# treangenlab/komb

Measured on AMD Instinct MI355X. Metric: peeled edges/sec (k-truss), higher is better.
Workload: dtype int32

## Files before the change

### komb_amd/csrc/common.h

```cpp
#pragma once

#include <hip/hip_runtime.h>

#include <chrono>
#include <cstddef>
#include <cstdint>
#include <cstdio>
#include <cstdlib>
#include <cstring>
#include <map>
#include <string>
#include <vector>

#include "komb_accel.h"

#include <roctracer/roctx.h>

namespace komb {

struct Range {
    explicit Range(const char *name) { (void)roctxRangePushA(name); }
    ~Range() { (void)roctxRangePop(); }
    void next(const char *name) { (void)roctxRangePop(); (void)roctxRangePushA(name); }
    Range(const Range &) = delete;
    Range &operator=(const Range &) = delete;
};

constexpr int kBlock = 256;
constexpr int kWave = 64;
constexpr int32_t kAlive = 0x7FFFFFFF;
constexpr int32_t kAliveMin = 0x40000000;

__device__ __forceinline__ uint32_t wave_sum(uint32_t v)
{
    for (int o = kWave / 2; o > 0; o >>= 1) v += (uint32_t)__shfl_xor((int32_t)v, o);
    return v;
}
__device__ __forceinline__ uint32_t wave_max(uint32_t v)
{
    for (int o = kWave / 2; o > 0; o >>= 1) { const uint32_t other = (uint32_t)__shfl_xor((int32_t)v, o); v = other > v ? other : v; }
    return v;
}

struct PeelCtrl {
    int32_t  mode;
    int32_t  level;
    int32_t  round;
    int32_t  done;
    uint32_t cur_light;
    uint32_t cur_heavy;
    int32_t  cur_sel;
    uint32_t remaining;
    int32_t  n_levels;
    int32_t  n_rounds;
    int32_t  n_scans;
    int32_t  max_level;
    uint32_t live_count;
    int32_t  live_sel;
    int32_t  live_mode;
    int32_t  seq;
    uint32_t tail_l[2];
    uint32_t tail_h[2];
    int32_t  next_min;
    uint32_t live_tail;
    int32_t  last_retire;
    uint32_t tail_limit;
    uint32_t pad1[7];
    int32_t  max_retire_gap;
};
static_assert(offsetof(PeelCtrl, seq) == 60 && offsetof(PeelCtrl, tail_l) == 64, "PeelCtrl: the entry state is one 64-byte line");
static_assert(sizeof(PeelCtrl) == 128, "PeelCtrl layout");

struct LocalCtrl {
    int32_t  done;
    int32_t  iters;
    uint32_t spare[3];
    uint32_t bad;
    int32_t  max_val;
    uint32_t levels;
    uint32_t evals;
    uint32_t n_light, n_heavy;
    uint32_t n_giant;
    uint32_t n_chunk;
    uint32_t pad0;
    unsigned long long key_sum;
};
static_assert(sizeof(LocalCtrl) == 64, "LocalCtrl layout");

enum FinishMode : int { FIN_LOCAL = 0, FIN_LDS = 1, FIN_NONE = 2 };

struct Timer {
    hipEvent_t a = nullptr, b = nullptr;
    bool init() { return hipEventCreate(&a) == hipSuccess && hipEventCreate(&b) == hipSuccess; }
    void start(hipStream_t s) { (void)hipEventRecord(a, s); }
    double stop(hipStream_t s)
    {
        (void)hipEventRecord(b, s);
        (void)hipEventSynchronize(b);
        float ms = 0.f;
        (void)hipEventElapsedTime(&ms, a, b);
        return (double)ms;
    }
    void destroy() { if (a) (void)hipEventDestroy(a); if (b) (void)hipEventDestroy(b); a = b = nullptr; }
};

struct EventSet {
    std::vector<hipEvent_t> v;
    EventSet() = default;
    EventSet(const EventSet &) = delete;
    EventSet &operator=(const EventSet &) = delete;
    hipError_t make(hipEvent_t *out, unsigned flags = 0)
    {
        hipEvent_t e = nullptr;
        const hipError_t rc = flags ? hipEventCreateWithFlags(&e, flags) : hipEventCreate(&e);
        if (rc == hipSuccess) { v.push_back(e); *out = e; }
        return rc;
    }
    ~EventSet() { for (hipEvent_t e : v) if (e) (void)hipEventDestroy(e); }
};

}

struct AllocHook {
    bool armed = false;
    int64_t requests = 0, fail_at = 0, trim_at = 0;
    int32_t fired = 0;
    enum Act { PASS, FAIL, TRIM };
    Act step()
    {
        ++requests;
        if (fail_at && requests == fail_at) { fail_at = 0; fired = 1; return FAIL; }
        if (trim_at && requests == trim_at) { trim_at = 0; return TRIM; }
        return PASS;
    }
};

struct Poison {
    bool on = false;
    uint32_t word = 0;
    hipStream_t stream = nullptr;
    AllocHook *hook = nullptr;
    hipError_t fill(void *p, size_t bytes) const
    {
        if (!on || !p || !bytes) return hipSuccess;
        const size_t words = bytes / 4, rest = bytes % 4;
        hipError_t e = hipSuccess;
        if (words) e = hipMemsetD32Async((hipDeviceptr_t)p, (int)word, words, stream);
        if (e == hipSuccess && rest) e = hipMemsetAsync((char *)p + 4 * words, (int)(word & 0xFFu), rest, stream);
        return e == hipSuccess ? hipStreamSynchronize(stream) : e;
    }
    hipError_t malloc(void **out, size_t bytes) const
    {
        if (hook && hook->armed && hook->step() == AllocHook::FAIL) return hipErrorOutOfMemory;
        void *q = nullptr;
        hipError_t e = hipMalloc(&q, bytes);
        if (e != hipSuccess) return e;
        e = fill(q, bytes);
        if (e != hipSuccess) { (void)hipFree(q); return e; }
        *out = q;
        return hipSuccess;
    }
};

struct DevPool {
    struct Block { void *p; size_t bytes; bool used; };
    std::vector<Block> blocks;
    size_t n_malloc = 0, n_trim = 0;
    double ms_malloc = 0.0;
    Poison poison;
    AllocHook hook;
    DevPool() { poison.hook = &hook; }
    DevPool(const DevPool &) = delete;
    DevPool &operator=(const DevPool &) = delete;
    hipError_t get(void **out, size_t bytes)
    {
        if (hook.armed) {
            const AllocHook::Act a = hook.step();
            if (a == AllocHook::FAIL) return hipErrorOutOfMemory;
            if (a == AllocHook::TRIM) { ++n_trim; trim(); }
        }
        if (bytes == 0) bytes = 16;
        int best = -1;
        for (int i = 0; i < (int)blocks.size(); ++i)
            if (!blocks[i].used && blocks[i].bytes >= bytes && blocks[i].bytes <= bytes + bytes / 4 + 4096 &&
                (best < 0 || blocks[i].bytes < blocks[best].bytes)) best = i;
        if (best >= 0) {
            if (poison.on) { const hipError_t e = poison.fill(blocks[best].p, blocks[best].bytes); if (e != hipSuccess) return e; }
            blocks[best].used = true; *out = blocks[best].p; return hipSuccess;
        }
        void *q = nullptr;
        ++n_malloc;
        const auto t0 = std::chrono::steady_clock::now();
        hipError_t e = hipMalloc(&q, bytes);
        ms_malloc += std::chrono::duration<double, std::milli>(std::chrono::steady_clock::now() - t0).count();
        if (e != hipSuccess) {
            ++n_trim;
            trim();
            e = hipMalloc(&q, bytes);
            if (e != hipSuccess) return e;
        }
        blocks.push_back({q, bytes, true});
        if (poison.on) { e = poison.fill(q, bytes); if (e != hipSuccess) { put(q); return e; } }
        *out = q;
        return hipSuccess;
// ... 512 lines not shown
```

### komb_amd/csrc/kcore.hip

```cpp
#include "peel_dev.h"
#include "core_tail.h"
#include "local_dev.h"
#include "shard_dev.h"

#include <cstdlib>

namespace komb {

namespace {

__global__ __launch_bounds__(kBlock) void k_core_init(const uint32_t *__restrict__ rowptr, int64_t nv,
                                                      int32_t *__restrict__ deg, int32_t *__restrict__ degw,
                                                      int32_t *__restrict__ core, uint32_t *__restrict__ init)
{
    uint32_t zeros = 0;
    int32_t lmin = 0x7FFFFFFF;
    for (int64_t v = (int64_t)blockIdx.x * kBlock + threadIdx.x; v < nv; v += (int64_t)gridDim.x * kBlock) {
        const int32_t d = (int32_t)(rowptr[v + 1] - rowptr[v]);
        deg[v] = d; degw[v] = d;
        if (d == 0) { core[v] = 0; ++zeros; }
        else { core[v] = alive_marker((uint32_t)d); lmin = min(lmin, d); }
    }
    block_add_min(zeros, lmin, &init[0], (int32_t *)&init[1]);
}
// ... 112 lines not shown
    const uint32_t *nbr;
    __device__ __forceinline__ void ids(uint32_t pos, uint32_t (&id)[1]) const { id[0] = nbr[pos]; }
};

__global__ void k_live_bits(const int32_t *__restrict__ gid, uint32_t n, unsigned long long *__restrict__ bits)
{
    for (uint32_t i = blockIdx.x * blockDim.x + threadIdx.x; i < n; i += gridDim.x * blockDim.x) {
        const uint32_t v = (uint32_t)gid[i];
        atomicOr(&bits[v >> 6], 1ull << (v & 63u));
    }
}

__global__ void k_collect_ctrl(PeelCtrl *c2, const PeelCtrl *from)
{
    if (threadIdx.x == 0) {
        PeelCtrl c{};
        c.mode = MODE_SCAN; c.round = 1; c.level = 0x3FFFFFFF; c.seq = 1;
        c.remaining = from->remaining;
        c.live_mode = from->live_mode; c.live_sel = from->live_sel; c.live_count = from->live_count;
        c.next_min = 0x7FFFFFFF;
        *c2 = c;
    }
}

__global__ void k_ctrl_pre(uint32_t *grp_done)
{
    for (int i = threadIdx.x; i < kInitOff; i += blockDim.x) grp_done[i] = 0u;
    if (threadIdx.x == 0) { grp_done[kInitOff] = 0u; grp_done[kInitOff + 1] = 0x7FFFFFFFu; grp_done[kInitOff + 2] = 0u; grp_done[kInitOff + 3] = 0u; }
}
__global__ void k_ctrl_init(PeelCtrl *ctrl, const uint32_t *grp_done, uint32_t units, uint32_t tail_limit)
{
    if (threadIdx.x == 0) {
        const uint32_t peeled = grp_done[kInitOff];
        const int32_t first = (int32_t)grp_done[kInitOff + 1];
        const uint32_t front = grp_done[kInitOff + 2];
        PeelCtrl c{};
        c.mode = MODE_SCAN; c.round = 1; c.seq = 1;
        c.last_retire = 1;
        c.remaining = units - peeled;
        c.done = (c.remaining == 0) ? 1 : 0;
        c.level = c.remaining ? first : 0;
        c.n_levels = peeled ? 1 : 0;
        c.next_min = 0x7FFFFFFF;
        c.tail_limit = tail_limit;
        if (front) {
            c.mode = MODE_PROCESS; c.cur_light = front; c.cur_heavy = 0; c.cur_sel = 0;
            c.remaining -= front;
            c.n_levels += 1; c.max_level = first;
        }
        *ctrl = c;
    }
}

}

void peel_ctrl_pre(hipStream_t s, uint32_t *d_grp_done) { k_ctrl_pre<<<1, 128, 0, s>>>(d_grp_done); }
void peel_collect_ctrl(hipStream_t s, PeelCtrl *d_collect, const PeelCtrl *d_from) { k_collect_ctrl<<<1, 64, 0, s>>>(d_collect, d_from); }

void peel_ctrl_init(hipStream_t s, PeelCtrl *d_ctrl, uint32_t *d_grp_done, uint32_t units, uint32_t tail_limit)
{
    k_ctrl_init<<<1, 64, 0, s>>>(d_ctrl, d_grp_done, units, tail_limit);
}

int peel_grid(int64_t units)
{
    int64_t g = (units + kPeelBlock - 1) / kPeelBlock;
    if (g < 1) g = 1;
    if (g > 256 * kPeelPerCu) g = 256 * kPeelPerCu;
    return (int)g;
}

int core_run(komb_ctx *ctx, int rank, int world, komb_allreduce_fn fn, void *user, bool sharded)
{
    if (ctx->nv < 0) KOMB_FAIL(ctx, KOMB_ERR_STATE, "komb_core_run: no graph loaded");
    const int64_t nv = ctx->nv;
    hipStream_t s = ctx->stream;
    ctx->core_done = false;
    if (!ctx->d_deg) {
        const size_t bytes = (size_t)(nv > 0 ? nv : 1) * sizeof(int32_t);
        KOMB_HIP(ctx, dev_malloc_pair(ctx, &ctx->d_deg, bytes, &ctx->d_core, bytes));
    }
    komb_stats &stt = ctx->stats;
    stt.core_levels = stt.core_subrounds = stt.core_launches = 0;
    stt.max_coreness = 0; stt.ms_core = 0.0;
    stt.core_local_units = 0; stt.core_local_sweeps = 0; stt.core_local_items = 0; stt.ms_core_local = 0.0;
    if (ctx_flag(ctx, "SHARD_ENGINE")) sharded = true;
    stt.shard_exchanges = 0; stt.ms_exchange = 0.0; stt.exchange_words = 0;
    stt.engine_flags = sharded ? KOMB_ENGINE_SHARD_PEEL : 0;
    if (nv == 0) { ctx->core_done = true; return KOMB_OK; }

    Range r_all("komb_core_run");
    DevBufs bufs(ctx);
    const size_t heavy_cap = (size_t)(2 * ctx->ne) / 32 + 64;
    int32_t *d_degw = nullptr; PeelCtrl *d_ctrl = nullptr; uint32_t *d_grp = nullptr;
    CoreTailBufs T{};
    PeelQueues Q{nullptr, {nullptr, nullptr}, {nullptr, nullptr}, {nullptr, nullptr}, 0};
    KOMB_HIP(ctx, bufs.alloc(&d_degw, (size_t)nv));
    for (int i = 0; i < 2; ++i) {
        KOMB_HIP(ctx, bufs.alloc(&Q.light[i], (size_t)nv));
        KOMB_HIP(ctx, bufs.alloc(&Q.heavy[i], heavy_cap));
        KOMB_HIP(ctx, bufs.alloc(&Q.live[i], (size_t)nv / 2 + 64));
    }
    KOMB_HIP(ctx, bufs.alloc(&Q.code, (size_t)nv));
    KOMB_HIP(ctx, bufs.alloc(&d_ctrl, 1));
    KOMB_HIP(ctx, bufs.alloc(&d_grp, (size_t)kInitOff + 4));
    const FinishMode fin = finish_mode(ctx, FIN_LOCAL);
    uint32_t tail_limit = 0;
    const size_t live_words = ((size_t)nv + 63) / 64;
    unsigned long long *d_livebits = nullptr;
    if (fin == FIN_LDS) {
        tail_limit = kCoreTailV;
        if (const char *tl = ctx_opt(ctx, "CORE_TAIL")) tail_limit = (uint32_t)strtoul(tl, nullptr, 10);
        if (tail_limit > kCoreTailV) tail_limit = kCoreTailV;
        if (tail_limit) {
            KOMB_HIP(ctx, bufs.alloc(&T.livebits, live_words));
            KOMB_HIP(ctx, bufs.alloc(&T.vnum, (size_t)nv));
            KOMB_HIP(ctx, bufs.alloc(&T.cnt, 4));
            KOMB_HIP(ctx, bufs.alloc(&T.vlist, (size_t)kCoreTailV));
            KOMB_HIP(ctx, bufs.alloc(&T.rows, (size_t)kCoreTailV * kCoreTailWords));
        }
    } else if (fin == FIN_LOCAL) {
        tail_limit = local_limit(ctx, (uint64_t)nv, 16);
        if (tail_limit) KOMB_HIP(ctx, bufs.alloc(&d_livebits, live_words));
    }

    int64_t g = (nv + kBlock - 1) / kBlock;
    const int grid_init = (int)(g > 1024 ? 1024 : g);
    const int grid = peel_grid(nv);
    CoreProblem P{(uint32_t)nv, ctx->d_o_rowptr, ctx->d_o_col, d_degw, ctx->d_core};
    ctx->timer.start(s);
    peel_ctrl_pre(s, d_grp);
    k_core_init<<<grid_init, kBlock, 0, s>>>(ctx->d_o_rowptr, nv, ctx->d_deg, d_degw, ctx->d_core, d_grp + kInitOff);
    peel_ctrl_init(s, d_ctrl, d_grp, (uint32_t)nv, tail_limit);
    auto run_tail = [&](const int32_t *list, uint32_t n_in) -> int {
        KOMB_HIP(ctx, hipMemsetAsync(T.livebits, 0, live_words * sizeof(unsigned long long), s));
        KOMB_HIP(ctx, hipMemsetAsync(T.cnt, 0, 4 * sizeof(uint32_t), s));
        KOMB_HIP(ctx, hipMemsetAsync(T.rows, 0, (size_t)kCoreTailV * kCoreTailWords * sizeof(unsigned long long), s));
        int64_t gm = ((int64_t)n_in + kBlock - 1) / kBlock;
        k_ctail_mark<<<(int)(gm < 1 ? 1 : (gm > 1024 ? 1024 : gm)), kBlock, 0, s>>>(list, n_in, ctx->d_core, T);
        k_ctail_rows<<<dim3(kCoreTailV, 8), kBlock, 0, s>>>(ctx->d_o_rowptr, ctx->d_o_col, T);
        k_core_tail<false><<<1, 1024, 0, s>>>(d_ctrl, T, d_degw, ctx->d_core, nullptr);
        KOMB_HIP(ctx, d2h(ctx, &ctx->h_ctrl[0], d_ctrl, sizeof(PeelCtrl)));
        return KOMB_OK;
    };
    auto run_local = [&]() -> int {
        const PeelCtrl hc = ctx->h_ctrl[0];
        Range r_local("core: local finish");
        EventSet evs;
        hipEvent_t ev[2] = {nullptr, nullptr};
        for (auto &e : ev) KOMB_HIP(ctx, evs.make(&e));
        (void)hipEventRecord(ev[0], s);
        KOMB_HIP(ctx, hipMemsetAsync(d_livebits, 0, live_words * sizeof(unsigned long long), s));
        LocalStats ls;
        const int rc = local_finish(ctx, bufs, hc, d_ctrl, (uint32_t)nv, ctx->d_core, d_degw, Q.live[hc.live_sel],
            (uint32_t)kWave * CoreLocal::kU, sizeof(uint32_t), local_item_limit(ctx, std::max<uint64_t>(kCoreLocalItems, (uint64_t)ctx->ne / 3)), 0u, false, 0, ctx->d_core,
            [&](const LocalGraph &lg, const int32_t *num, void *items, PeelCtrl *d_cctrl, int32_t launch) {
                CoreCollect C{(uint32_t)nv, ctx->d_o_rowptr, ctx->d_o_col, ctx->d_core, d_livebits, num, lg.off, lg.cur, (uint32_t *)items};
                k_peel_step<CoreCollect><<<grid, kPeelBlock, 0, s>>>(d_cctrl, d_grp, Q, C, launch);
            },
            [&](const LocalGraph &lg, void *items, uint64_t total, LocalCtrl *d_lctrl, uint32_t *d_cnt, int *launches) -> int {
                return local_fixpoint(ctx, d_lctrl, d_cnt, lg, CoreLocal{(const uint32_t *)items}, total, launches);
            },
            &ls,
            [&](const LocalGraph &lg) { k_live_bits<<<(int)((lg.n + 255) / 256 > 1024 ? 1024 : (lg.n + 255) / 256), 256, 0, s>>>(lg.gid, lg.n, d_livebits); });
        (void)hipEventRecord(ev[1], s);
        (void)hipEventSynchronize(ev[1]);
        float ms = 0.f;
        (void)hipEventElapsedTime(&ms, ev[0], ev[1]);
        KOMB_TRY(rc);
        if (ls.refused) { ctx->h_ctrl[0].done = 0; ctx->h_ctrl[0].tail_limit = ls.new_limit; return KOMB_OK; }
        stt.core_local_units = (int32_t)ls.units; stt.core_local_sweeps = ls.sweeps; stt.core_local_items = (int64_t)ls.items;
        stt.ms_core_local = (double)ms;
        PeelCtrl done = hc;
        done.done = 1; done.remaining = 0;
        done.n_levels += (int32_t)ls.levels;
        done.max_level = ls.max_val > done.max_level ? ls.max_val : done.max_level;
        ctx->h_ctrl[0] = done;
        return KOMB_OK;
    };
    int launches = 0, st = KOMB_OK;
    if (sharded) {
        uint32_t iw[2] = {0u, 0u};
        KOMB_HIP(ctx, d2h(ctx, iw, d_grp + kInitOff, sizeof(iw)));
        ShardCore SP{(uint32_t)nv, ctx->d_o_rowptr, ctx->d_o_col, d_degw, ctx->d_core, 0u, 0u};
        shard_bounds((uint64_t)nv, rank, world, &SP.lo, &SP.hi);
        ShardStats ss;
        st = shard_peel(ctx, bufs, SP, d_degw, (uint32_t)nv, iw[0], (int32_t)iw[1], rank, world, fn, user, Q, d_ctrl,
                        [&](int32_t launch) { k_peel_step<ShardCore><<<grid, kPeelBlock, 0, s>>>(d_ctrl, d_grp, Q, SP, launch); },
                        fin == FIN_LOCAL ? tail_limit : 0u, [&]() -> int { return run_local(); }, &ss);
        stt.shard_exchanges = (int32_t)ss.exchanges; stt.ms_exchange = ss.ms_exchange; stt.exchange_words = ss.words;
        launches = ss.launches;
        PeelCtrl fc{};
        fc.done = st == KOMB_OK ? 1 : 2; fc.n_levels = ss.levels; fc.n_rounds = ss.rounds; fc.n_scans = ss.scans; fc.max_level = ss.max_level;
        ctx->h_ctrl[0] = fc;
    } else if (tail_limit && (uint64_t)nv <= tail_limit) {
        st = d2h(ctx, &ctx->h_ctrl[0], d_ctrl, sizeof(PeelCtrl)) == hipSuccess ? KOMB_OK : KOMB_ERR_DEVICE;
        if (st == KOMB_OK && !ctx->h_ctrl[0].done) st = (fin == FIN_LOCAL) ? run_local() : run_tail(nullptr, (uint32_t)nv);
    } else {
        ctx->h_ctrl[0].done = 0;
    }
    for (int guard = 0; st == KOMB_OK && ctx->h_ctrl[0].done != 1 && ctx->h_ctrl[0].done != 2 && guard < 64; ++guard) {
        if (ctx->h_ctrl[0].done == 3) {
            const PeelCtrl &c = ctx->h_ctrl[0];
            if (fin == FIN_LOCAL) st = run_local();
            else st = c.live_mode ? run_tail(Q.live[c.live_sel], c.live_count) : run_tail(nullptr, (uint32_t)nv);
            continue;
        }
        int batch = 0;
        st = drive_peel(ctx, d_ctrl, nv, [&](int32_t launch) {
            k_peel_step<CoreProblem><<<grid, kPeelBlock, 0, s>>>(d_ctrl, d_grp, Q, P, launch);
        }, &batch);
        launches += batch;
    }
    stt.ms_core = ctx->timer.stop(s);
#ifdef KOMB_STEP_TIMERS
    {
        const PeelCtrl &c = ctx->h_ctrl[0];
        const double n = c.pad1[6] ? (double)c.pad1[6] : 1.0;
        fprintf(stderr, "komb core step timers (block 0, %u small multi-workgroup PROCESS steps), us per step: ctrl %.2f queue+slice %.2f items %.2f flush %.2f barrier %.2f ticket %.2f\n",
                c.pad1[6], c.pad1[0] / n / 100.0, c.pad1[1] / n / 100.0, c.pad1[2] / n / 100.0, c.pad1[3] / n / 100.0, c.pad1[4] / n / 100.0, c.pad1[5] / n / 100.0);
    }
#endif
    KOMB_TRY(st);
    if (ctx->h_ctrl[0].done != 1) KOMB_FAIL(ctx, KOMB_ERR_DEVICE, "k-core peel ended in an inconsistent state");
    if (stt.core_local_units) stt.engine_flags |= KOMB_ENGINE_LOCAL_FINISH;
    else if (fin == FIN_LDS && tail_limit) stt.engine_flags |= KOMB_ENGINE_LDS_TAIL;
    stt.core_levels = ctx->h_ctrl[0].n_levels;
    stt.core_subrounds = ctx->h_ctrl[0].n_rounds;
    stt.core_launches = launches;
    stt.max_coreness = ctx->h_ctrl[0].max_level;
    ctx->core_done = true;
    return KOMB_OK;
}

}
```

### komb_amd/csrc/ktruss.hip

```cpp
#include "peel_dev.h"
#include "truss_tail.h"
#include "local_dev.h"
#include "shard_dev.h"

#include <algorithm>
#include <cstdlib>
#include <cstring>

#include "truss_line.h"
#include "truss_tri.h"
#include "truss_wedge.h"
#include "truss_index.h"
#include "truss_gather.h"

namespace komb {

namespace {

struct TrussProblem {
    static constexpr bool kChain = false;
    static constexpr bool kSingleStep = false;
    uint32_t units;
    const uint2 *off2;
    const int2 *inc;
    int32_t *sup;
    int32_t *stamp;
    uint8_t *st8;
    static constexpr int32_t kRetireEvery = komb::kRetireEvery;
    int32_t retire_every;
#ifdef KOMB_DEBUG_SWITCHES
    int ablate;
#endif

    __device__ __forceinline__ void retire(const CtrlView &cv, uint32_t block, uint32_t nblocks) const
    {
        const uint32_t n16 = (units + 15u) / 16u;
        uint4 *v = reinterpret_cast<uint4 *>(st8);
        for (uint32_t i = block * (uint32_t)kPeelBlock + threadIdx.x; i < n16; i += nblocks * (uint32_t)kPeelBlock) {
            uint4 q = v[i];
            uint32_t *w = &q.x;
            bool changed = false;
#pragma unroll
            for (int k = 0; k < 4; ++k) {
                uint32_t out = w[k];
#pragma unroll
                for (int b = 0; b < 4; ++b) {
                    const uint32_t c = (w[k] >> (8 * b)) & 0xFFu;
                    if (c > ST_GONE && state_rel(c, cv.round) == REL_GONE) out = (out & ~(0xFFu << (8 * b))) | ((uint32_t)ST_GONE << (8 * b));
                }
                changed |= out != w[k];
                w[k] = out;
            }
            if (changed) v[i] = q;
        }
    }

    __device__ __forceinline__ const int32_t *scan_marker() const { return stamp; }
    __device__ __forceinline__ const uint8_t *scan_state() const { return st8; }
    __device__ __forceinline__ const int32_t *scan_key() const { return sup; }
    __device__ __forceinline__ void mark_scanned(uint32_t e, const CtrlView &cv) const { stamp[e] = cv.round; st8[e] = state_of_round(cv.round); }
    __device__ __forceinline__ void slice(uint32_t e, uint32_t &b, uint32_t &len) const
    {
        const uint2 o = off2[e];
        b = o.x;
        len = o.y;
    }
    struct Loaded { int32_t me, x, y; uint32_t cx, cy; };
    __device__ __forceinline__ Loaded item_load(int32_t me, uint32_t pos, const CtrlView &) const
    {
        Loaded ld;
#ifdef KOMB_DEBUG_SWITCHES
        if (ablate & 6) {
            int2 p = make_int2((int)(((uint32_t)me * 2654435761u) % units), (int)(((uint32_t)me * 40503u + pos) % units));
            if (!(ablate & 4)) { const unsigned long long pq = __builtin_nontemporal_load(reinterpret_cast<const unsigned long long *>(inc) + pos); p = make_int2((int)(uint32_t)pq, (int)(uint32_t)(pq >> 32)); }
            ld.me = me; ld.x = p.x; ld.y = p.y;
            ld.cx = (ablate & 2) ? 0u : st8[p.x]; ld.cy = (ablate & 2) ? 0u : st8[p.y];
            return ld;
        }
#endif
        const unsigned long long pq = __builtin_nontemporal_load(reinterpret_cast<const unsigned long long *>(inc) + pos);
        const int2 p = make_int2((int)(uint32_t)pq, (int)(uint32_t)(pq >> 32));
        ld.me = me; ld.x = p.x; ld.y = p.y;
        ld.cx = st8[p.x]; ld.cy = st8[p.y];
        return ld;
    }
    __device__ __forceinline__ void item_apply(const Loaded &ld, const CtrlView &cv, int32_t &t0, int32_t &t1, uint32_t &c0, uint32_t &c1) const
    {
        const int32_t r = cv.round, L = cv.level;
        const int rx = state_rel(ld.cx, r), ry = state_rel(ld.cy, r);
        if (rx == REL_GONE || ry == REL_GONE) return;
        const bool xin = (rx == REL_NOW), yin = (ry == REL_NOW);
        bool decx = !xin && (!yin || ld.me < ld.y);
        bool decy = !yin && (!xin || ld.me < ld.x);
#ifdef KOMB_DEBUG_SWITCHES
        if (ablate & 1) { decx = false; decy = false; }
#endif
        if (decx && atomicSub(&sup[ld.x], 1) == L + 1) {
            c0 = ld.cx == ST_ALIVE_HEAVY ? marker_chunks(stamp[ld.x]) : 0u;
            stamp[ld.x] = r + 1; st8[ld.x] = state_of_round(r + 1); t0 = ld.x;
        }
        if (decy && atomicSub(&sup[ld.y], 1) == L + 1) {
            c1 = ld.cy == ST_ALIVE_HEAVY ? marker_chunks(stamp[ld.y]) : 0u;
            stamp[ld.y] = r + 1; st8[ld.y] = state_of_round(r + 1); t1 = ld.y;
        }
    }
};

struct ShardTruss {
    static constexpr bool kChain = false;
    static constexpr bool kSingleStep = true;
    uint32_t units;
    const uint2 *off2;
    const int2 *inc;
    int32_t *sup;
    int32_t *stamp;
    uint32_t lo, hi;

    __device__ __forceinline__ const int32_t *scan_marker() const { return stamp; }
    __device__ __forceinline__ const int32_t *scan_key() const { return sup; }
    __device__ __forceinline__ void mark_scanned(uint32_t e, const CtrlView &cv) const { stamp[e] = cv.round; }
    __device__ __forceinline__ void slice(uint32_t e, uint32_t &b, uint32_t &len) const
    {
        const uint2 o = off2[e];
        b = o.x;
        len = o.y;
    }
    __device__ __forceinline__ bool mine(int32_t e) const { return (uint32_t)e - lo < hi - lo; }
    struct Loaded { int32_t me, x, y, sx, sy; };
    __device__ __forceinline__ Loaded item_load(int32_t me, uint32_t pos, const CtrlView &) const
    {
        Loaded ld;
        const int2 p = inc[pos];
        ld.me = me; ld.x = p.x; ld.y = p.y;
        ld.sx = stamp[p.x]; ld.sy = stamp[p.y];
        return ld;
    }
    __device__ __forceinline__ void item_apply(const Loaded &ld, const CtrlView &cv, int32_t &t0, int32_t &t1, uint32_t &, uint32_t &) const
    {
        const int32_t r = cv.round, L = cv.level;
        if (ld.sx < r || ld.sy < r) return;
        const bool xin = (ld.sx == r), yin = (ld.sy == r);
        const bool decx = !xin && (!yin || ld.me < ld.y) && mine(ld.x);
        const bool decy = !yin && (!xin || ld.me < ld.x) && mine(ld.y);
        if (decx && atomicSub(&sup[ld.x], 1) == L + 1) { stamp[ld.x] = r + 1; t0 = ld.x; }
        if (decy && atomicSub(&sup[ld.y], 1) == L + 1) { stamp[ld.y] = r + 1; t1 = ld.y; }
    }
};

struct TrussCollect {
    static constexpr bool kChain = false;
    static constexpr bool kSingleStep = false;
    uint32_t units;
    const uint2 *off2;
    const int2 *inc;
    const int32_t *stamp;
    const int32_t *num;
    const uint32_t *coff;
    uint32_t *cur;
    uint2 *cpair;

    __device__ __forceinline__ const int32_t *scan_marker() const { return stamp; }
    __device__ __forceinline__ const int32_t *scan_key() const { return nullptr; }
    __device__ __forceinline__ void mark_scanned(uint32_t, const CtrlView &) const {}
    __device__ __forceinline__ void slice(uint32_t e, uint32_t &b, uint32_t &len) const
    {
        const uint2 o = off2[e];
        b = o.x;
        len = o.y;
    }
    struct Loaded { int32_t me, x, y, sx, sy; };
    __device__ __forceinline__ Loaded item_load(int32_t me, uint32_t pos, const CtrlView &) const
    {
        Loaded ld;
        const int2 p = inc[pos];
        ld.me = me; ld.x = p.x; ld.y = p.y;
        ld.sx = stamp[p.x]; ld.sy = stamp[p.y];
        return ld;
    }
    __device__ __forceinline__ void item_apply(const Loaded &ld, const CtrlView &, int32_t &, int32_t &, uint32_t &, uint32_t &) const
    {
        if (!marker_alive(ld.sx) || !marker_alive(ld.sy)) return;
        const uint32_t id = (uint32_t)num[ld.me];
        const uint32_t b0 = coff[id], k = local_slot(id, cur);
        if (k < coff[id + 1] - b0) cpair[b0 + k] = make_uint2((uint32_t)num[ld.x], (uint32_t)num[ld.y]);
    }
};

constexpr uint64_t kTrussLocalItems = 32ull << 20;
constexpr uint32_t kTrussLocalDensity = 160;
struct TrussLocal {
    static constexpr int kU = 8;
#ifndef KOMB_TRUSS_GROUPS
#define KOMB_TRUSS_GROUPS 8
#endif
    static constexpr int kGroups = KOMB_TRUSS_GROUPS;
    static constexpr int kN = 2;
    const uint2 *cpair;
    __device__ __forceinline__ void ids(uint32_t pos, uint32_t (&id)[2]) const
    {
        const uint2 p = cpair[pos];
        id[0] = p.x; id[1] = p.y;
    }
};

}

void truss_free(komb_ctx *ctx)
{
    communities_drop(ctx);
    community_hierarchy_drop(ctx);
    biconnected_drop(ctx);
    structural_drop(ctx);
    nucleus_drop(ctx);
    max_clique_drop(ctx);
    clique_census_drop(ctx);
    maximal_cliques_drop(ctx);
    if (ctx->t_own_edges) { ctx->pool.put(ctx->d_t_eu); ctx->pool.put(ctx->d_t_ev); }
    ctx->pool.put(ctx->d_t_truss);
    ctx->pool.put(ctx->d_t_sup);
    ctx->pool.put(ctx->d_t_slice);
    ctx->d_t_eu = ctx->d_t_ev = ctx->d_t_truss = ctx->d_t_sup = nullptr;
    ctx->d_t_slice = nullptr;
    ctx->t_sup_ready = false;
    ctx->t_own_edges = false;
    ctx->t_ne = -1; ctx->truss_done = false;
}

int truss_edges_canonical(komb_ctx *ctx)
{
    if (ctx->t_own_edges || ctx->t_ne <= 0) return KOMB_OK;
    if (!ctx->d_ceu) {
        int32_t *eu = nullptr, *ev = nullptr;
        hipError_t e = ctx->pool.get((void **)&eu, (size_t)ctx->ne * sizeof(int32_t));
        if (e == hipSuccess) e = ctx->pool.get((void **)&ev, (size_t)ctx->ne * sizeof(int32_t));
        const int rc = e == hipSuccess ? edge_list(ctx, ctx->d_o_rowptr, ctx->d_o_col, ctx->nv, nullptr, eu, ev) : KOMB_ERR_NOMEM;
        if (rc != KOMB_OK) {
            ctx->pool.put(eu); ctx->pool.put(ev);
            if (e != hipSuccess) KOMB_FAIL(ctx, KOMB_ERR_NOMEM, "komb_truss_fetch: no memory for the canonical edge list (%s)", hipGetErrorString(e));
            return rc;
        }
        ctx->d_ceu = eu; ctx->d_cev = ev;
    }
    ctx->d_t_eu = ctx->d_ceu; ctx->d_t_ev = ctx->d_cev;
    return KOMB_OK;
}

int truss_support_canonical(komb_ctx *ctx)
{
    if (ctx->t_sup_ready) return KOMB_OK;
    if (!ctx->truss_done || !ctx->d_t_slice || !ctx->prep.valid || ctx->prep.ne != ctx->t_ne)
        KOMB_FAIL(ctx, KOMB_ERR_STATE, "komb_truss_fetch_support: no k-truss result to take the supports from");
    hipStream_t s = ctx->stream;
    const int64_t m = ctx->t_ne;
    if (!ctx->d_t_sup) KOMB_HIP(ctx, ctx->pool.get((void **)&ctx->d_t_sup, (size_t)m * sizeof(int32_t)));
#ifndef KOMB_TEST_SKIP_SLICE_ZERO
    if (ctx->t_k_lo) KOMB_HIP(ctx, hipMemsetAsync(ctx->d_t_sup, 0, (size_t)ctx->t_k_lo * sizeof(int32_t), s));
    if (ctx->t_k_hi < (uint32_t)m) KOMB_HIP(ctx, hipMemsetAsync(ctx->d_t_sup + ctx->t_k_hi, 0, ((size_t)m - ctx->t_k_hi) * sizeof(int32_t), s));
#endif
    k_scatter_len<<<grid_for(m), kBlock, 0, s>>>(ctx->d_t_slice, ctx->prep.e2k, m, ctx->t_k_lo, ctx->t_k_hi, ctx->d_t_sup);
    KOMB_HIP(ctx, hipStreamSynchronize(s));
    ctx->t_sup_ready = true;
    return KOMB_OK;
}

namespace {
int truss_run_body(komb_ctx *ctx, const uint8_t *vmask_host, int rank, int world, komb_allreduce_fn fn, void *user)
{
    if (world < 1 || rank < 0 || rank >= world || (world > 1 && !fn))
        KOMB_FAIL(ctx, KOMB_ERR_ARG, "komb_truss_run_sharded: bad rank %d / world %d / callback", rank, world);
    if (ctx->nv < 0) KOMB_FAIL(ctx, KOMB_ERR_STATE, "komb_truss_run: no graph loaded");
    truss_free(ctx);
    hipStream_t s = ctx->stream;
    komb_stats &st = ctx->stats;
    st.triangles = 0; st.truss_levels = st.truss_subrounds = st.truss_launches = 0;
    st.max_trussness = 0; st.ms_support = st.ms_peel = st.ms_orient = st.ms_tri_count = st.ms_tri_fill = st.ms_gather = st.ms_allreduce = st.ms_compact = 0.0;
    st.truss_scans = 0; st.ms_prepare = 0.0; st.truss_prepared = 0; st.ms_prep_vertex = st.ms_prep_edges = st.ms_prep_rows = 0.0;
    auto empty_result = [&]() -> int {
        void *q[4] = {nullptr, nullptr, nullptr, nullptr};
        hipError_t e = hipSuccess;
        for (int i = 0; i < 4 && e == hipSuccess; ++i) e = ctx->pool.get(&q[i], 4);
        if (e != hipSuccess) {
            for (void *p : q) ctx->pool.put(p);
            KOMB_HIP(ctx, e);
        }
        ctx->d_t_eu = (int32_t *)q[0]; ctx->d_t_ev = (int32_t *)q[1]; ctx->d_t_truss = (int32_t *)q[2]; ctx->d_t_sup = (int32_t *)q[3];
        ctx->t_own_edges = true; ctx->t_ne = 0; ctx->truss_done = true; ctx->t_sup_ready = true;
        return KOMB_OK;
    };
    if (ctx->nv == 0 || ctx->ne == 0) return empty_result();
    Range r_all("komb_truss_run");
    DevBufs bufs(ctx);

    Range phase("truss: preparation");
    InducedCsr sub;
    TrussPrep sub_prep;
    struct SubGuard { komb_ctx *c; InducedCsr *g; TrussPrep *p; ~SubGuard() { prep_free(c, p); induced_free(c, g); } } sub_guard{ctx, &sub, &sub_prep};
    TrussPrep *tp = &ctx->prep;
    if (vmask_host) {
        ctx->timer.start(s);
        KOMB_TRY(induce_csr(ctx, vmask_host, &sub));
        st.ms_orient = ctx->timer.stop(s);
        if (sub.ns == 0) return empty_result();
        KOMB_TRY(prep_build(ctx, sub.rowptr, sub.col, sub.nv, sub.ns, &sub_prep));
        st.ms_prepare = sub_prep.ms; st.truss_prepared = 1;
        st.ms_prep_vertex = sub_prep.ms_part[0]; st.ms_prep_edges = sub_prep.ms_part[1]; st.ms_prep_rows = sub_prep.ms_part[2];
        tp = &sub_prep;
    } else if (!ctx->prep.valid) {
        KOMB_TRY(prep_ensure(ctx));
        st.ms_prepare = ctx->prep.ms; st.truss_prepared = 1;
        st.ms_prep_vertex = ctx->prep.ms_part[0]; st.ms_prep_edges = ctx->prep.ms_part[1]; st.ms_prep_rows = ctx->prep.ms_part[2];
    }
    const int64_t nv = tp->nv;
    const int64_t m = tp->ne;
    const uint32_t *d_orow = tp->orow;
    const int32_t *d_ocol = tp->ocol;
    const uint4 *d_line = tp->vline;
    const uint2 *d_wtasks = (const uint2 *)tp->wtasks;
    const int64_t n_wtasks = tp->n_wtasks;
    const int gw = grid_for(n_wtasks, kTriWaves);
    phase.next("truss: triangles + incidence index");

    const int ge = grid_for(m);
    const int tri_tv = (int)std::max<int64_t>(1, std::min<int64_t>(kTriV, nv / (256 * KOMB_TRI_EU * kTriWaves * 4)));
    const int64_t ntasks = (nv + tri_tv - 1) / tri_tv;
    const int gt = grid_for(ntasks, kTriWaves);
    uint32_t *d_own = nullptr, *d_other = nullptr, *d_cnt = nullptr, *d_off = nullptr;
    uint2 *d_off2 = nullptr;
    KOMB_HIP(ctx, bufs.alloc(&d_own, 2 * ((size_t)m + 1)));
    d_other = d_own + ((size_t)m + 1);
    KOMB_HIP(ctx, bufs.alloc(&d_cnt, (size_t)m + 1));
    KOMB_HIP(ctx, bufs.alloc(&d_off2, (size_t)m + 4));
    unsigned long long *d_mom = nullptr;
    KOMB_HIP(ctx, bufs.alloc(&d_mom, 12));
    KOMB_HIP(ctx, hipMemsetAsync(d_mom, 0, 12 * sizeof(unsigned long long), s));
// ... 36 lines not shown
    st.ms_sort = 0.0; st.tri_records = 0; st.ms_compact = 0.0; st.ms_tri_count = 0.0; st.ms_tri_fill = 0.0; st.stream_retries = 0;
    st.index_layout = layout;
    auto zero_counts = [&]() -> hipError_t { return hipMemsetAsync(d_own, 0, 2 * ((size_t)m + 1) * sizeof(uint32_t), s); };
    if (!(world == 1 && layout == IDX_STREAM)) KOMB_HIP(ctx, zero_counts());
    bool have_counts = false;
    if (world > 1) {
        const int64_t task_lo = n_wtasks * rank / world, task_hi = n_wtasks * (rank + 1) / world;
        ctx->timer.start(s);
        k_wedges<TRI_COUNT><<<gw, kBlock, 0, s>>>(d_orow, d_ocol, d_line, d_wtasks, task_lo, task_hi, d_own, d_other, nullptr, nullptr, 0ull, nullptr, no_stream, nullptr, ablate);
        st.ms_tri_count = ctx->timer.stop(s);
        k_sum_counts<<<ge, kBlock, 0, s>>>(d_own, d_other, nullptr, m + 1, d_cnt, d_mom + 5);
        ctx->timer.start(s);
        KOMB_HIP(ctx, hipStreamSynchronize(s));
        if (fn(user, d_cnt, (int64_t)m + 1) != 0)
            KOMB_FAIL(ctx, KOMB_ERR_DEVICE, "komb_truss_run_sharded: all-reduce callback failed");
        st.ms_allreduce = ctx->timer.stop(s);
        KOMB_HIP(ctx, hipMemsetAsync(d_mom + 5, 0, sizeof(unsigned long long), s));
        k_total_u32<<<ge, kBlock, 0, s>>>(d_cnt, m + 1, d_mom + 5);
        have_counts = true;
        if (layout != IDX_TWO_PASS) {
            KOMB_HIP(ctx, bufs.alloc(&d_cnt_ref, (size_t)m + 1));
            KOMB_HIP(ctx, hipMemcpyAsync(d_cnt_ref, d_cnt, ((size_t)m + 1) * sizeof(uint32_t), hipMemcpyDeviceToDevice, s));
            KOMB_HIP(ctx, zero_counts());
        }
    }

    if (layout == IDX_STREAM) {
        const unsigned long long bound = (unsigned long long)tp->own_bound;
        const int gws = std::min(gw, 256 * KOMB_WEDGE_EU);
        const unsigned long long slack = (unsigned long long)gws * kTriWaves * kRecChunk + kRecChunk;
        const unsigned long long own_slack = (unsigned long long)gws * kTriWaves * kOwnChunk + kOwnChunk;
        const unsigned long long t_bound = bound / 2;
        const unsigned long long own_full = bound + bound / 8 + own_slack, rec_full = 3 * t_bound + (3 * t_bound) / 14 + slack;
        unsigned long long own_cap = std::min(own_full, 4ull * (unsigned long long)m + own_slack);
        unsigned long long rec_cap = std::min(rec_full, 2ull * (unsigned long long)m + slack);
        bool fixed_caps = false;
        if (const char *oc = ctx_opt(ctx, "OWN_DENSE_CAP")) { own_cap = strtoull(oc, nullptr, 10) + 1; rec_cap = rec_full; fixed_caps = true; }
        if (ctx_flag(ctx, "NO_OWN_DENSE")) { own_cap = 1; rec_cap = rec_full; fixed_caps = true; }
        if (const char *rc = ctx_opt(ctx, "REC_CAP")) { rec_cap = strtoull(rc, nullptr, 10) + 1; fixed_caps = true; }
        if (ctx_flag(ctx, "FULL_CAPS")) { own_cap = own_full; rec_cap = rec_full; }
        if (!fixed_caps && ctx->cap_hint.nv == nv && ctx->cap_hint.m == m) {
            own_cap = std::min(own_full, std::max(own_cap, ctx->cap_hint.own_cap));
            rec_cap = std::min(rec_full, std::max(rec_cap, ctx->cap_hint.rec_cap));
        }
        const uint32_t sentinel = geom.sentinel_base();
        uint32_t *d_key = nullptr; int2 *d_val = nullptr;
        unsigned long long n_claimed = 0;
        bool ok = false;
        st.ms_tri_fill = 0.0;
        for (int attempt = 0; attempt < 2; ++attempt) {
            size_t free_b = 0, total_b = 0;
            (void)hipMemGetInfo(&free_b, &total_b);
            const unsigned long long budget = (unsigned long long)((free_b + ctx->pool.unused_bytes()) * 0.7);
            if (own_cap * sizeof(int2) > budget / 2) own_cap = budget / 2 / sizeof(int2);
            if (rec_cap * 12ull > budget / 2) rec_cap = budget / 2 / 12ull;
            if (rec_cap > 0xFFFFFFF0ull) rec_cap = 0xFFFFFFF0ull;
            ok = bufs.alloc(&d_key, (size_t)rec_cap) == hipSuccess && bufs.alloc(&d_val, (size_t)rec_cap) == hipSuccess &&
                 bufs.alloc(&d_owndense, (size_t)own_cap) == hipSuccess &&
                 (d_ownoff || bufs.alloc(&d_ownoff, (size_t)m + 1) == hipSuccess) && (d_dcur || bufs.alloc(&d_dcur, 4) == hipSuccess);
            uint2 *d_scratch = nullptr;
            if (ok && !ctx_flag(ctx, "NO_REC_SCRATCH") && bufs.alloc(&d_scratch, (size_t)gws * kTriWaves * kScratchRec) != hipSuccess) { (void)hipGetLastError(); d_scratch = nullptr; }
            if (!ok) { (void)hipGetLastError(); break; }
            KOMB_HIP(ctx, hipMemsetAsync(d_dcur, 0, 4 * sizeof(unsigned long long), s));
            const TriStream ts{d_key, d_val, d_dcur + 2, rec_cap, sentinel, geom.nb - 1u, kChunkBits};
            ctx->timer.start(s);
            k_wedges<TRI_SINGLE><<<gws, kBlock, 0, s>>>(d_orow, d_ocol, d_line, d_wtasks, 0, n_wtasks, d_own, d_other, d_owndense, d_dcur, own_cap, d_ownoff, ts, d_scratch, ablate);
            st.ms_tri_fill += ctx->timer.stop(s);
            unsigned long long dc[4] = {0, 0, 0, 0};
            KOMB_HIP(ctx, d2h(ctx, dc, d_dcur, sizeof(dc)));
            n_claimed = dc[2];
            bufs.release(d_scratch);
            if (ctx_flag(ctx, "TRI_DEBUG"))
                fprintf(stderr, "komb triangles: stream build (attempt %d): %llu record positions claimed of %llu, dense own-role region %llu entries claimed of %llu, %llu task ranges overflowed their record buffer\n",
                        attempt, dc[2], rec_cap, dc[0], own_cap, dc[1]);
            if (n_claimed <= rec_cap) {
                if (!fixed_caps) { ctx->cap_hint.nv = nv; ctx->cap_hint.m = m; ctx->cap_hint.own_cap = own_cap; ctx->cap_hint.rec_cap = rec_cap; }
                break;
            }
            ok = false;
            if (attempt == 1 || fixed_caps) break;
            bufs.release(d_key); bufs.release(d_val); bufs.release(d_owndense);
            d_key = nullptr; d_val = nullptr; d_owndense = nullptr;
            own_cap = std::min(own_full, std::max(own_cap, dc[0] + own_slack));
            rec_cap = std::min(rec_full, n_claimed + slack);
            st.stream_retries += 1;
        }
        uint32_t *d_skey = nullptr;
        if (ok) {
            uint32_t *d_key2 = nullptr; unsigned long long *d_val2 = nullptr;
            ok = bufs.alloc(&d_key2, (size_t)n_claimed + 1) == hipSuccess && bufs.alloc(&d_val2, (size_t)n_claimed + 1) == hipSuccess;
            if (ok) {
                ctx->timer.start(s);
                unsigned long long *sv = nullptr;
                if (geom.nb_bits > 0) KOMB_TRY(prim_sort_pairs_u32_u64(ctx, d_key, d_key2, (unsigned long long *)d_val, d_val2, (int64_t)n_claimed, kChunkBits, kChunkBits + geom.nb_bits, &d_skey, &sv));
                else { d_skey = d_key; sv = (unsigned long long *)d_val; }
                st.ms_sort = ctx->timer.stop(s);
                d_recval = (int2 *)sv;
                if (d_skey == d_key) { bufs.release(d_key2); bufs.release(d_val2); } else { bufs.release(d_key); bufs.release(d_val); }
                d_reckey = d_skey;
                KOMB_HIP(ctx, bufs.alloc(&d_toff, (size_t)n_bins + 2));
                KOMB_HIP(ctx, bufs.alloc(&d_bintot, (size_t)n_bins + 2));
                KOMB_HIP(ctx, bufs.alloc(&d_grp, (size_t)kInitOff + 4));
                if (!whole_peel_finish && !shard_peel_on && !ctx_flag(ctx, "NO_FIRST_QUEUE")) KOMB_HIP(ctx, bufs.alloc(&d_light0, (size_t)m));
                ctx->timer.start(s);
                peel_ctrl_pre(s, d_grp);
                KOMB_HIP(ctx, hipMemsetAsync(d_mom + 5, 0, sizeof(unsigned long long), s));
                k_bin_offsets<<<grid_for(n_bins + 1), kBlock, 0, s>>>(d_skey, (int64_t)n_claimed, geom, d_toff);
                k_bin_count<<<grid_for(n_bins, 1, 256 * 8), kBlock, 0, s>>>(d_skey, d_toff, geom, d_own, m, d_cnt, d_bintot, d_mom + 5, (int32_t *)(d_grp + kInitOff + 1));
                st.ms_compact = ctx->timer.stop(s);
                st.tri_records = (int64_t)n_claimed;
            } else (void)hipGetLastError();
        }
        if (!ok) {
            bufs.release(d_key); bufs.release(d_val); bufs.release(d_owndense); bufs.release(d_ownoff); bufs.release(d_dcur);
            bufs.release(d_grp); bufs.release(d_light0); d_grp = nullptr; d_light0 = nullptr;
            d_owndense = nullptr; d_ownoff = nullptr; d_dcur = nullptr;
            KOMB_HIP(ctx, zero_counts());
            KOMB_HIP(ctx, hipMemsetAsync(d_mom + 5, 0, sizeof(unsigned long long), s));
            st.ms_tri_fill = 0.0;
            layout = IDX_TWO_PASS;
        }
    }
    if (layout != IDX_TWO_PASS && d_cnt_ref) {
        k_count_mismatch<<<ge, kBlock, 0, s>>>(d_cnt, d_cnt_ref, m + 1, d_mom + 8);
    }
    if (layout == IDX_TWO_PASS) {
        if (d_cnt_ref) {
            KOMB_HIP(ctx, hipMemcpyAsync(d_cnt, d_cnt_ref, ((size_t)m + 1) * sizeof(uint32_t), hipMemcpyDeviceToDevice, s));
            KOMB_HIP(ctx, hipMemsetAsync(d_mom + 5, 0, sizeof(unsigned long long), s));
            k_total_u32<<<ge, kBlock, 0, s>>>(d_cnt, m + 1, d_mom + 5);
        } else if (!have_counts) {
            ctx->timer.start(s);
            k_triangles<TRI_COUNT><<<gt, kBlock, 0, s>>>(d_orow, d_ocol, nv, 0, ntasks, d_own, d_other, nullptr, nullptr, ablate, tri_tv);
            st.ms_tri_count = ctx->timer.stop(s);
            k_sum_counts<<<ge, kBlock, 0, s>>>(d_own, d_other, nullptr, m + 1, d_cnt, d_mom + 5);
        }
    }
    st.index_layout = layout;
    {
        unsigned long long mom[9];
        KOMB_HIP(ctx, d2h(ctx, mom, d_mom, sizeof(mom)));
        st.triangles = (int64_t)(mom[5] / 3);
        bufs.release(d_mom);
        if (mom[8] != 0)
            KOMB_FAIL(ctx, KOMB_ERR_DEVICE, "komb_truss_run_sharded: %llu edges whose all-reduced support differs from the support of the index build", mom[8]);
        if (mom[5] > 0xFFFFFFF0ull)
            KOMB_FAIL(ctx, KOMB_ERR_LIMIT, "graph has %llu triangles; the incidence index is limited to 2^32-16 entries (3 per triangle)",
                      mom[5] / 3);
    }
    bufs.release(d_cnt_ref);
    uint32_t total = 0;
    const uint32_t sum_supports = (uint32_t)st.triangles * 3u;
    int2 *d_inc = nullptr;
    int32_t *d_sup = nullptr, *d_stamp = nullptr, *d_truss = nullptr;
    uint8_t *d_st8 = nullptr;
    bool peel_inited = false;
    if (layout == IDX_STREAM) {
        KOMB_TRY(prim_exclusive_sum_u32(ctx, d_bintot, d_bintot, n_bins + 1));
        total = sum_supports;
        KOMB_HIP(ctx, bufs.alloc(&d_inc, (size_t)total));
        KOMB_HIP(ctx, bufs.alloc(&d_sup, (size_t)m));
        KOMB_HIP(ctx, bufs.alloc(&d_stamp, (size_t)m));
        KOMB_HIP(ctx, bufs.alloc(&d_st8, (size_t)m + 16));
        KOMB_HIP(ctx, bufs.alloc(&d_truss, (size_t)m));
        ctx->timer.start(s);
        k_bin_finish<<<grid_for(n_bins, 1, 256 * kFinPerCu), kFinBlock, 0, s>>>(d_reckey, d_recval, d_toff, geom, d_own, d_cnt, d_bintot, d_owndense, d_ownoff, d_inc, m,
                                                                      d_off2, d_sup, d_stamp, d_st8, d_grp + kInitOff, d_light0);
        st.ms_compact += ctx->timer.stop(s);
        peel_inited = true;
        bufs.release(d_toff); bufs.release(d_bintot); bufs.release((void *)d_recval); bufs.release(d_reckey);
        bufs.release(d_owndense); bufs.release(d_ownoff); bufs.release(d_dcur);
    } else {
        KOMB_HIP(ctx, bufs.alloc(&d_off, (size_t)m + 1));
        KOMB_TRY(prim_exclusive_sum_u32(ctx, d_cnt, d_off, m + 1));
        KOMB_HIP(ctx, d2h(ctx, &total, d_off + m, sizeof(uint32_t)));
        KOMB_HIP(ctx, bufs.alloc(&d_inc, (size_t)total));
        ctx->timer.start(s);
        KOMB_HIP(ctx, zero_counts());
        k_back_cursors<<<ge, kBlock, 0, s>>>(d_off, m, d_other);
        k_triangles<TRI_SINGLE><<<gt, kBlock, 0, s>>>(d_orow, d_ocol, nv, 0, ntasks, d_own, d_other, d_off, d_inc, ablate, tri_tv);
        st.ms_tri_fill = ctx->timer.stop(s);
    }
    st.ms_support = st.ms_tri_count + st.ms_tri_fill + st.ms_sort + st.ms_compact;
    bufs.release(d_cnt); bufs.release(d_own);

    phase.next("truss: peel");
    PeelCtrl *d_ctrl = nullptr;
    PeelQueues Q{nullptr, {nullptr, nullptr}, {nullptr, nullptr}, {nullptr, nullptr}, 0};
    const size_t heavy_cap = (size_t)total / 32 + 64;
    if (!peel_inited) {
        KOMB_HIP(ctx, bufs.alloc(&d_sup, (size_t)m));
        KOMB_HIP(ctx, bufs.alloc(&d_stamp, (size_t)m));
        KOMB_HIP(ctx, bufs.alloc(&d_st8, (size_t)m + 16));
        KOMB_HIP(ctx, bufs.alloc(&d_truss, (size_t)m));
        KOMB_HIP(ctx, bufs.alloc(&d_grp, (size_t)kInitOff + 4));
    }
    for (int i = 0; i < 2; ++i) {
        if (i == 0 && d_light0) Q.light[0] = d_light0;
        else KOMB_HIP(ctx, bufs.alloc(&Q.light[i], (size_t)m));
        KOMB_HIP(ctx, bufs.alloc(&Q.heavy[i], heavy_cap));
        KOMB_HIP(ctx, bufs.alloc(&Q.live[i], (size_t)m / 2 + 64));
    }
    KOMB_HIP(ctx, bufs.alloc(&d_ctrl, 1));
    KOMB_HIP(ctx, bufs.alloc(&Q.code, (size_t)m));
    KOMB_HIP(ctx, bufs.alloc(&Q.rlevel, (size_t)m + 2));
    KOMB_HIP(ctx, hipMemsetAsync(Q.rlevel, 0, 2 * sizeof(int32_t), s));
    int32_t retire_every = kRetireEvery;
    if (const char *e = ctx_opt(ctx, "RETIRE_EVERY")) retire_every = std::max(1, std::min((int)kRetireEvery, atoi(e)));
#ifdef KOMB_DEBUG_SWITCHES
    TrussProblem P{(uint32_t)m, d_off2, d_inc, d_sup, d_stamp, d_st8, retire_every, getenv("KOMB_PEEL_ABLATE") ? atoi(getenv("KOMB_PEEL_ABLATE")) : 0};
#else
    TrussProblem P{(uint32_t)m, d_off2, d_inc, d_sup, d_stamp, d_st8, retire_every};
#endif
    TailBufs T{};
    if (fin == FIN_LDS && tail_limit) {
        KOMB_HIP(ctx, bufs.alloc(&T.vmap, (size_t)nv));
        KOMB_HIP(ctx, bufs.alloc(&T.cnt, 64));
        KOMB_HIP(ctx, bufs.alloc(&T.vlist, (size_t)kTailMaxV));
        KOMB_HIP(ctx, bufs.alloc(&T.rows, (size_t)kTailMaxV * kTailRowWords));
        KOMB_HIP(ctx, bufs.alloc(&T.pair, (size_t)tail_limit));
        KOMB_HIP(ctx, bufs.alloc(&T.sup, (size_t)tail_limit));
        KOMB_HIP(ctx, bufs.alloc(&T.gid, (size_t)tail_limit));
        KOMB_HIP(ctx, bufs.alloc(&T.gid_by_rank, (size_t)tail_limit));
        KOMB_HIP(ctx, bufs.alloc(&T.pair_by_rank, (size_t)tail_limit));
        KOMB_HIP(ctx, bufs.alloc(&T.truss_by_rank, (size_t)tail_limit));
        KOMB_HIP(ctx, bufs.alloc(&T.spill[0], (size_t)tail_limit));
        KOMB_HIP(ctx, bufs.alloc(&T.spill[1], (size_t)tail_limit));
        T.max_edges = tail_limit;
    }
    auto run_tail = [&](const int32_t *list, uint32_t n_in) -> int {
        KOMB_HIP(ctx, hipMemsetAsync(T.vmap, 0, (size_t)nv * sizeof(int32_t), s));
        KOMB_HIP(ctx, hipMemsetAsync(T.cnt, 0, 64 * sizeof(uint32_t), s));
        KOMB_HIP(ctx, hipMemsetAsync(T.rows, 0, (size_t)kTailMaxV * kTailRowWords * sizeof(unsigned long long), s));
        const int g = grid_for(n_in, kBlock, 256);
        const bool dbg = ctx_flag(ctx, "TAIL_DEBUG");
        hipEvent_t ev[3] = {nullptr, nullptr, nullptr};
        for (auto &e : ev) (void)hipEventCreate(&e);
        (void)hipEventRecord(ev[0], s);
        k_tail_mark<<<g, kBlock, 0, s>>>(list, n_in, d_sup, d_stamp, d_osrc, d_ocol, T);
        k_tail_number<<<1, kTailMaxV, 0, s>>>(T);
        k_tail_rows<<<g, kBlock, 0, s>>>(list, n_in, d_sup, d_stamp, d_osrc, d_ocol, T);
        (void)hipEventRecord(ev[1], s);
        k_truss_tail<<<1, 1024, 0, s>>>(d_ctrl, T, d_truss);
        (void)hipEventRecord(ev[2], s);
        KOMB_HIP(ctx, d2h(ctx, &ctx->h_ctrl[0], d_ctrl, sizeof(PeelCtrl)));
        ++st.truss_tail_runs;
        float m0 = 0, m1 = 0, m2 = 0;
        (void)hipEventElapsedTime(&m0, ctx->timer.a, ev[0]); (void)hipEventElapsedTime(&m1, ev[0], ev[1]); (void)hipEventElapsedTime(&m2, ev[1], ev[2]);
        for (auto &e : ev) (void)hipEventDestroy(e);
        st.ms_tail += (double)m1 + (double)m2;
        if (dbg) {
            uint32_t h[16];
            KOMB_HIP(ctx, d2h(ctx, h, T.cnt, sizeof(h)));
            fprintf(stderr, "komb tail: %u vertices, %u edges, %s; general engine before it %.1f us, setup %.1f us, tail kernel %.1f us\n",
                    h[0], h[1], ctx->h_ctrl[0].done == 1 ? "done" : "refused", m0 * 1000.f, m1 * 1000.f, m2 * 1000.f);
#ifdef KOMB_TAIL_TIMERS
            fprintf(stderr, "komb tail: us in kernel: load %.1f ranks %.1f supports %.1f scan %.1f mark %.1f triangles %.1f retire %.1f results %.1f\n",
                    h[14] / 100.0, h[15] / 100.0, h[8] / 100.0, h[9] / 100.0, h[10] / 100.0, h[11] / 100.0, h[12] / 100.0, h[13] / 100.0);
#endif
        }
        return KOMB_OK;
    };
    const int gp = peel_grid(m);
    auto run_local = [&]() -> int {
        const PeelCtrl hc = ctx->h_ctrl[0];
        EventSet evs;
        hipEvent_t ev[2] = {nullptr, nullptr};
        for (auto &e : ev) KOMB_HIP(ctx, evs.make(&e));
        (void)hipEventRecord(ev[0], s);
        LocalStats ls;
        const int lrc = local_finish(ctx, bufs, hc, d_ctrl, (uint32_t)m, d_stamp, d_sup, Q.live[hc.live_sel],
            (uint32_t)kWave * TrussLocal::kU, sizeof(uint2), local_item_limit(ctx, kTrussLocalItems), local_density_limit(ctx, kTrussLocalDensity), true, 2, d_truss,
            [&](const LocalGraph &lg, const int32_t *num, void *items, PeelCtrl *d_cctrl, int32_t launch) {
                TrussCollect C{(uint32_t)m, d_off2, d_inc, d_stamp, num, lg.off, lg.cur, (uint2 *)items};
                PeelQueues Qc = Q;
                Qc.rlevel = nullptr;
                k_peel_step<TrussCollect><<<gp, kPeelBlock, 0, s>>>(d_cctrl, d_grp, Qc, C, launch);
            },
            [&](const LocalGraph &lg, void *items, uint64_t total_items, LocalCtrl *d_lctrl, uint32_t *d_cnt, int *nl) -> int {
                return local_fixpoint(ctx, d_lctrl, d_cnt, lg, TrussLocal{(const uint2 *)items}, total_items, nl);
            },
            &ls, [](const LocalGraph &) {});
        (void)hipEventRecord(ev[1], s);
        (void)hipEventSynchronize(ev[1]);
        float ms = 0.f;
        (void)hipEventElapsedTime(&ms, ev[0], ev[1]);
        KOMB_TRY(lrc);
        if (ls.refused) { ctx->h_ctrl[0].done = 0; ctx->h_ctrl[0].tail_limit = ls.new_limit; return KOMB_OK; }
        st.truss_local_units = (int32_t)ls.units; st.truss_local_sweeps = ls.sweeps; st.truss_local_items = (int64_t)ls.items;
        st.ms_truss_local = (double)ms;
        PeelCtrl fin_c = hc;
        fin_c.done = 1; fin_c.remaining = 0;
        fin_c.n_levels += (int32_t)ls.levels;
        fin_c.max_level = ls.max_val > fin_c.max_level ? ls.max_val : fin_c.max_level;
        ctx->h_ctrl[0] = fin_c;
        return KOMB_OK;
    };
    ctx->timer.start(s);
    if (!peel_inited) {
        peel_ctrl_pre(s, d_grp);
        k_peel_init<<<grid_for(m, kBlock, 1024), kBlock, 0, s>>>(m, d_off, d_off2, d_sup, d_stamp, d_st8, d_grp + kInitOff);
    }
    peel_ctrl_init(s, d_ctrl, d_grp, (uint32_t)m, tail_limit);
    int launches = 0, rc = KOMB_OK;
    st.truss_tail_runs = 0; st.ms_tail = 0.0;
    st.truss_local_units = 0; st.truss_local_sweeps = 0; st.truss_local_items = 0; st.ms_truss_local = 0.0;
    st.shard_exchanges = 0; st.ms_exchange = 0.0; st.exchange_words = 0;
    if (shard_peel_on) {
        uint32_t iw[2] = {0u, 0u};
        KOMB_HIP(ctx, d2h(ctx, iw, d_grp + kInitOff, sizeof(iw)));
        ShardTruss SP{(uint32_t)m, d_off2, d_inc, d_sup, d_stamp, 0u, 0u};
        shard_bounds((uint64_t)m, rank, world, &SP.lo, &SP.hi);
        ShardStats ss;
        rc = shard_peel(ctx, bufs, SP, d_sup, (uint32_t)m, iw[0], (int32_t)iw[1], rank, world, fn, user, Q, d_ctrl,
                        [&](int32_t launch) { k_peel_step<ShardTruss><<<gp, kPeelBlock, 0, s>>>(d_ctrl, d_grp, Q, SP, launch); },
                        fin == FIN_LOCAL ? tail_limit : 0u, [&]() -> int { return run_local(); }, &ss);
        st.shard_exchanges = (int32_t)ss.exchanges; st.ms_exchange = ss.ms_exchange; st.exchange_words = ss.words;
        launches = ss.launches;
        PeelCtrl fc{};
        fc.done = rc == KOMB_OK ? 1 : 2; fc.n_levels = ss.levels; fc.n_rounds = ss.rounds; fc.n_scans = ss.scans; fc.max_level = ss.max_level;
        ctx->h_ctrl[0] = fc;
    } else if (whole_peel_finish) {
        rc = d2h(ctx, &ctx->h_ctrl[0], d_ctrl, sizeof(PeelCtrl)) == hipSuccess ? KOMB_OK : KOMB_ERR_DEVICE;
        if (rc == KOMB_OK && !ctx->h_ctrl[0].done) rc = (fin == FIN_LOCAL) ? run_local() : run_tail(nullptr, (uint32_t)m);
    } else {
        ctx->h_ctrl[0].done = 0;
    }
    for (int guard = 0; rc == KOMB_OK && ctx->h_ctrl[0].done != 1 && ctx->h_ctrl[0].done != 2 && guard < 64; ++guard) {
        if (ctx->h_ctrl[0].done == 3) {
            const PeelCtrl &c = ctx->h_ctrl[0];
            if (fin == FIN_LOCAL) rc = run_local();
            else rc = c.live_mode ? run_tail(Q.live[c.live_sel], c.live_count) : run_tail(nullptr, (uint32_t)m);
            continue;
        }
        int batch = 0;
        rc = drive_peel(ctx, d_ctrl, m, [&](int32_t launch) {
            k_peel_step<TrussProblem><<<gp, kPeelBlock, 0, s>>>(d_ctrl, d_grp, Q, P, launch);
        }, &batch);
        launches += batch;
    }
    st.ms_peel = ctx->timer.stop(s);
    KOMB_TRY(rc);
#ifdef KOMB_STEP_TIMERS
    {
        const PeelCtrl &c = ctx->h_ctrl[0];
        const double n = c.pad1[6] ? (double)c.pad1[6] : 1.0;
        fprintf(stderr, "komb step timers (block 0, %u small multi-workgroup PROCESS steps), us per step: ctrl %.2f queue+slice %.2f items %.2f flush %.2f barrier %.2f ticket %.2f\n",
                c.pad1[6], c.pad1[0] / n / 100.0, c.pad1[1] / n / 100.0, c.pad1[2] / n / 100.0, c.pad1[3] / n / 100.0, c.pad1[4] / n / 100.0, c.pad1[5] / n / 100.0);
    }
#endif
    if (ctx->h_ctrl[0].done != 1) KOMB_FAIL(ctx, KOMB_ERR_DEVICE, "k-truss peel ended in an inconsistent state");
    if (ctx->h_ctrl[0].max_retire_gap > retire_every)
        KOMB_FAIL(ctx, KOMB_ERR_DEVICE, "k-truss peel: %d sub-rounds passed without a RETIRE step (period %d): edge state codes may have wrapped",
                  ctx->h_ctrl[0].max_retire_gap, retire_every);
    st.engine_flags = (layout == IDX_TWO_PASS ? KOMB_ENGINE_TWO_PASS : 0) | (shard_peel_on ? KOMB_ENGINE_SHARD_PEEL : 0) |
                      (st.truss_local_units ? KOMB_ENGINE_LOCAL_FINISH : 0) | (st.truss_tail_runs ? KOMB_ENGINE_LDS_TAIL : 0);
    st.truss_levels = ctx->h_ctrl[0].n_levels;
    st.truss_subrounds = ctx->h_ctrl[0].n_rounds;
    st.truss_launches = launches;
    st.truss_scans = ctx->h_ctrl[0].n_scans;
    st.max_trussness = ctx->h_ctrl[0].max_level + 2;
    for (int i = 0; i < 2; ++i) { bufs.release(Q.light[i]); bufs.release(Q.heavy[i]); bufs.release(Q.live[i]); }
    bufs.release(Q.code);
    bufs.release(d_sup); bufs.release(d_inc);

    phase.next("truss: canonical gather");
    ctx->timer.start(s);
    KOMB_HIP(ctx, ctx->pool.get((void **)&ctx->d_t_truss, (size_t)m * sizeof(int32_t)));
    uint32_t k_lo = 0, k_hi = (uint32_t)m;
    if (!vmask_host) {
        ctx->d_t_eu = ctx->d_ceu; ctx->d_t_ev = ctx->d_cev;
        ctx->t_own_edges = false;
        if (ctx->slice_world > 1) {
            shard_bounds((uint64_t)m, ctx->slice_rank, ctx->slice_world, &k_lo, &k_hi);
#ifndef KOMB_TEST_SKIP_SLICE_ZERO
            if (k_lo) KOMB_HIP(ctx, hipMemsetAsync(ctx->d_t_truss, 0, (size_t)k_lo * sizeof(int32_t), s));
            if (k_hi < (uint32_t)m) KOMB_HIP(ctx, hipMemsetAsync(ctx->d_t_truss + k_hi, 0, ((size_t)m - k_hi) * sizeof(int32_t), s));
#endif
        }
    } else {
        ctx->t_own_edges = true;
        KOMB_HIP(ctx, ctx->pool.get((void **)&ctx->d_t_eu, (size_t)m * sizeof(int32_t)));
        KOMB_HIP(ctx, ctx->pool.get((void **)&ctx->d_t_ev, (size_t)m * sizeof(int32_t)));
        KOMB_TRY(edge_list(ctx, sub.rowptr, sub.col, sub.nv, sub.vold, ctx->d_t_eu, ctx->d_t_ev));
    }
    ctx->t_k_lo = k_lo; ctx->t_k_hi = k_hi;
    k_truss_results<<<grid_for(m), kBlock, 0, s>>>(d_stamp, Q.rlevel, d_truss, tp->e2k, m, k_lo, k_hi, ctx->d_t_truss);
    ctx->d_t_slice = d_off2;
    bufs.detach(d_off2);
    ctx->t_sup_ready = false;
    if (vmask_host) {
        KOMB_HIP(ctx, ctx->pool.get((void **)&ctx->d_t_sup, (size_t)m * sizeof(int32_t)));
        k_scatter_len<<<grid_for(m), kBlock, 0, s>>>(ctx->d_t_slice, tp->e2k, m, 0u, (uint32_t)m, ctx->d_t_sup);
        ctx->t_sup_ready = true;
    }
    st.ms_gather = ctx->timer.stop(s);
    if (ctx_flag(ctx, "POOL_DEBUG")) {
        size_t held = 0;
        for (const auto &b : ctx->pool.blocks) held += b.bytes;
        fprintf(stderr, "komb pool: %zu blocks, %.2f GB held, %zu hipMalloc calls so far (%.1f ms inside them), %zu trims\n", ctx->pool.blocks.size(), held / 1e9, ctx->pool.n_malloc, ctx->pool.ms_malloc, ctx->pool.n_trim);
    }
    if (vmask_host) KOMB_HIP(ctx, hipStreamSynchronize(s));
    ctx->t_ne = m;
    ctx->truss_done = true;
    return KOMB_OK;
}
}

int truss_run(komb_ctx *ctx, const uint8_t *vmask_host, int rank, int world, komb_allreduce_fn fn, void *user)
{
    const int rc = truss_run_body(ctx, vmask_host, rank, world, fn, user);
    if (rc != KOMB_OK && !ctx->truss_done) truss_free(ctx);
    return rc;
}

}
```

### komb_amd/csrc/local_dev.h

```cpp
#pragma once

#include "peel_dev.h"

namespace komb {

constexpr int kLocBlock = 512;
constexpr int kLocWaves = kLocBlock / kWave;
constexpr int kLocHB = 4096;
constexpr int kLocBins = kLocHB / kLocBlock;
constexpr int kCntWays = 8;
constexpr int kCntWords = (5 * kCntWays + 5) * 32;
constexpr int kCntTimerWords = 6 * 12 * 2;
constexpr int kHvU = 8;
constexpr uint32_t kKeyBins = 4096;
constexpr uint32_t kMedMax = 2048;
constexpr int kGiantWin = 8;
constexpr uint32_t kGiantChunk = 8192;
constexpr int kLocBatch = 6;


struct LocalGraph {
    uint32_t n, nh;
    uint32_t *off;
    int32_t *val;
    int32_t *mark[2];
    int32_t *gid;
    uint32_t *len;
    uint32_t *cur;
    uint4 *giant;
    uint32_t ng;
    uint4 *gchunk;
    uint32_t nchunk;
    unsigned long long *gacc;
    uint32_t *gwin;
    int4 *gnote;
    uint32_t *khist;
    uint32_t *list;
    uint32_t flags;
};
constexpr uint32_t kLocUseList = 1u, kLocDeferNotify = 2u;
constexpr uint32_t kLocDeferChunks = 256;

constexpr int kNumBlock = 1024;
static __global__ __launch_bounds__(kNumBlock) void k_local_number(const int32_t *__restrict__ list, uint32_t n_in, uint32_t n_live,
                                                         const int32_t *__restrict__ marker, const int32_t *__restrict__ key,
                                                         uint32_t light_max, int32_t *__restrict__ num, LocalGraph g, LocalCtrl *ctrl)
{
    __shared__ uint32_t sh_cnt[kNumBlock / kWave][2];
    __shared__ uint32_t sh_base[2];
    __shared__ uint32_t sh_kh[kKeyBins];
    __shared__ unsigned long long sh_ks;
    unsigned long long ks = 0ull;
    if (threadIdx.x == 0) sh_ks = 0ull;
    for (uint32_t i = threadIdx.x; i < kKeyBins; i += kNumBlock) sh_kh[i] = 0u;
    const int lane = lane_id(), w = (int)(threadIdx.x >> 6);
    for (uint32_t i0 = blockIdx.x * kNumBlock; i0 < n_in; i0 += gridDim.x * kNumBlock) {
        const uint32_t i = i0 + threadIdx.x;
        int32_t u = -1, k = 0;
        if (i < n_in) {
            u = list ? list[i] : (int32_t)i;
            if (!marker_alive(marker[u])) u = -1; else k = key[u];
        }
        const bool heavy = u >= 0 && (uint32_t)k > light_max, light = u >= 0 && !heavy;
        const uint64_t mh = __ballot(heavy), ml = __ballot(light);
        __syncthreads();
        if (lane == 0) { sh_cnt[w][0] = (uint32_t)__popcll(mh); sh_cnt[w][1] = (uint32_t)__popcll(ml); }
        __syncthreads();
        uint32_t bh = 0, bl = 0, th = 0, tl = 0;
#pragma unroll
        for (int x = 0; x < kNumBlock / kWave; ++x) {
            const uint32_t a = sh_cnt[x][0], b = sh_cnt[x][1];
            if (x < w) { bh += a; bl += b; }
            th += a; tl += b;
        }
        if (threadIdx.x == 0) {
            sh_base[0] = th ? atomicAdd(&ctrl->n_heavy, th) : 0u;
            sh_base[1] = tl ? atomicAdd(&ctrl->n_light, tl) : 0u;
        }
        __syncthreads();
        if (u < 0) continue;
        ks += (unsigned long long)(uint32_t)k;
        const uint32_t id = heavy ? sh_base[0] + bh + (uint32_t)__popcll(mh & lanemask_lt())
                                  : n_live - 1u - (sh_base[1] + bl + (uint32_t)__popcll(ml & lanemask_lt()));
        if (id >= n_live) { atomicAdd(&ctrl->bad, 1u); continue; }
        num[u] = (int32_t)id;
        g.gid[id] = u; g.len[id] = (uint32_t)k; g.val[id] = k; g.mark[1][id] = 1; g.mark[0][id] = 0; g.cur[id] = 0u;
        atomicAdd(&sh_kh[min((uint32_t)k, kKeyBins - 1u)], 1u);
        if ((uint32_t)k > kMedMax) {
            const uint32_t nch = ((uint32_t)k + kGiantChunk - 1u) / kGiantChunk;
            g.giant[atomicAdd(&ctrl->n_giant, 1u)] = make_uint4(id, atomicAdd(&ctrl->n_chunk, nch), nch, 0u);
        }
    }
    for (int o = 32; o > 0; o >>= 1) ks += __shfl_xor(ks, o);
    if (lane == 0 && ks) atomicAdd(&sh_ks, ks);
    __syncthreads();
    for (uint32_t i = threadIdx.x; i < kKeyBins; i += kNumBlock) if (sh_kh[i]) atomicAdd(&g.khist[i], sh_kh[i]);
    if (threadIdx.x == 0 && sh_ks) atomicAdd(&ctrl->key_sum, sh_ks);
}

static __global__ __launch_bounds__(kBlock) void k_local_chunks(LocalGraph g)
{
    for (uint32_t gi = blockIdx.x; gi < g.ng; gi += gridDim.x) {
        const uint4 u = g.giant[gi];
        for (uint32_t j = threadIdx.x; j < u.z; j += kBlock) g.gchunk[u.y + j] = make_uint4(u.x, gi, j, u.z);
        if (threadIdx.x == 0) { g.gacc[gi] = 0ull; g.gnote[gi] = make_int4(0, 0, 0, 0); }
        if (threadIdx.x < (uint32_t)kGiantWin) g.gwin[gi * kGiantWin + threadIdx.x] = 0u;
    }
}

static __global__ __launch_bounds__(kBlock) void k_local_clamp(LocalGraph g, int32_t K)
{
    for (uint32_t id = blockIdx.x * kBlock + threadIdx.x; id < g.n; id += gridDim.x * kBlock)
        if (g.val[id] > K) g.val[id] = K;
}

__device__ __forceinline__ uint32_t local_slot(uint32_t id, uint32_t *cur)
{
    const int lane = lane_id();
    uint64_t todo = __ballot(true);
    uint32_t pos = 0;
    while (todo) {
        const int leader = __ffsll((long long)todo) - 1;
        const uint32_t lid = (uint32_t)__shfl((int)id, leader);
        const uint64_t grp = __ballot(id == lid) & todo;
        uint32_t base = 0;
        if (lane == leader) base = atomicAdd(&cur[lid], (uint32_t)__popcll(grp));
        base = (uint32_t)__shfl((int)base, leader);
        if ((grp >> lane) & 1ull) pos = base + (uint32_t)__popcll(grp & lanemask_lt());
        todo &= ~grp;
    }
    return pos;
}

static __global__ __launch_bounds__(kBlock) void k_local_check(LocalGraph g, LocalCtrl *ctrl)
{
    uint32_t bad = 0;
    for (uint32_t id = blockIdx.x * kBlock + threadIdx.x; id < g.n; id += gridDim.x * kBlock)
        bad += (g.cur[id] != g.off[id + 1] - g.off[id]) ? 1u : 0u;
    bad = wave_sum(bad);
    if (lane_id() == 0 && bad) atomicAdd(&ctrl->bad, bad);
    if (blockIdx.x == 0 && threadIdx.x == 0 && (ctrl->n_heavy != g.nh || ctrl->n_heavy + ctrl->n_light != g.n)) atomicAdd(&ctrl->bad, 1u);
}

constexpr int kListBlock = 1024;
static __global__ __launch_bounds__(kListBlock) void k_local_list(const LocalCtrl *ctrl, uint32_t *cnt, LocalGraph g, int32_t k)
{
    if (ctrl->done) return;
    __shared__ uint32_t sh_n[kListBlock / kWave];
    __shared__ uint32_t sh_base;
    const int32_t *mark_cur = g.mark[k & 1];
    const int lane = lane_id(), w = (int)(threadIdx.x >> 6);
    uint32_t *tail = cnt + (5 * kCntWays + 3 + (k & 1)) * 32;
    const uint32_t nlight = g.n - g.nh;
    for (uint32_t i0 = blockIdx.x * kListBlock; i0 < nlight; i0 += gridDim.x * kListBlock) {
        const uint32_t i = i0 + threadIdx.x;
        const bool m = i < nlight && mark_cur[g.nh + i] == k;
        const uint64_t bm = __ballot(m);
        __syncthreads();
        if (lane == 0) sh_n[w] = (uint32_t)__popcll(bm);
        __syncthreads();
        uint32_t before = 0, total = 0;
#pragma unroll
        for (int x = 0; x < kListBlock / kWave; ++x) { const uint32_t c = sh_n[x]; if (x < w) before += c; total += c; }
        if (threadIdx.x == 0) sh_base = total ? atomicAdd(tail, total) : 0u;
        __syncthreads();
        if (m) g.list[sh_base + before + (uint32_t)__popcll(bm & lanemask_lt())] = g.nh + i;
    }
}

template <class P>
__device__ __forceinline__ int32_t local_value(const P &p, uint32_t pos, const int32_t *val)
{
    uint32_t id[P::kN];
    p.ids(pos, id);
    int32_t v = val[id[0]];
#pragma unroll
    for (int i = 1; i < P::kN; ++i) v = min(v, val[id[i]]);
    return v;
}
template <class P>
struct LocalNotify {
    uint32_t id[P::kN];
    bool hit[P::kN];
    __device__ __forceinline__ void load(const P &p, uint32_t pos, const int32_t *val, const int32_t *mark_cur, int32_t h, int32_t a, int32_t k, bool active, bool all)
    {
#pragma unroll
        for (int i = 0; i < P::kN; ++i) hit[i] = false;
        if (!active) return;
        p.ids(pos, id);
        int32_t v[P::kN];
#pragma unroll
        for (int i = 0; i < P::kN; ++i) v[i] = val[id[i]];
#pragma unroll
        for (int i = 0; i < P::kN; ++i) hit[i] = v[i] > h && (all || v[i] <= a || mark_cur[id[i]] == k);
    }
    __device__ __forceinline__ void load_known(const P &p, uint32_t pos, int32_t v0, const int32_t *mark_cur, int32_t h, int32_t a, int32_t k, bool active, bool all)
    {
        static_assert(P::kN == 1, "one unit per item");
        hit[0] = false;
        if (!active || v0 <= h) return;
        p.ids(pos, id);
        hit[0] = all || v0 <= a || mark_cur[id[0]] == k;
    }
    __device__ __forceinline__ void store(int32_t *mark_next, int32_t k) const
    {
#pragma unroll
        for (int i = 0; i < P::kN; ++i) if (hit[i]) mark_next[id[i]] = k + 1;
    }
};

template <class P>
__global__ __launch_bounds__(kLocBlock) void k_local_step(LocalCtrl *ctrl, uint32_t *cnt, LocalGraph g, P p, int32_t k, uint32_t full_thr)
{
    constexpr int kU = P::kU;
// ... 390 lines not shown
    if (lane == 0 && (k == 1 || k == 4 || k == 8 || k == 12 || k == 16 || k == 20)) {
        const int slot = k == 1 ? 0 : k / 4;
        unsigned long long *tm = reinterpret_cast<unsigned long long *>(cnt + kCntWords) + slot * 12;
        for (int i = 0; i < 9; ++i) atomicAdd(&tm[i], tmv[i]);
        atomicMax(&tm[9], wall_clock64() - tstart);
        atomicAdd(&tm[10], 1ull);
    }
#endif
    __syncthreads();
    if (lane == 0) { sh_end[w][0] = n_changed; sh_end[w][1] = n_evals; }
    __syncthreads();
    if (tid == 0) {
        uint32_t c = 0, e = 0;
        for (int i = 0; i < kLocWaves; ++i) { c += sh_end[i][0]; e += sh_end[i][1]; }
        uint32_t *mine = cnt + ((k & 3) * kCntWays + (blockIdx.x % kCntWays)) * 32;
        if (c) atomicAdd(mine, c);
        if (e) atomicAdd(cnt + (4 * kCntWays + (blockIdx.x % kCntWays)) * 32, e);
    }
}

template <class P>
__global__ __launch_bounds__(kLocBlock) void k_local_giant_notify(const LocalCtrl *ctrl, LocalGraph g, P p, int32_t k)
{
    if (ctrl->done) return;
    const int32_t *mark_cur = g.mark[k & 1];
    int32_t *mark_next = g.mark[(k + 1) & 1];
    for (uint32_t c = blockIdx.x; c < g.nchunk; c += gridDim.x) {
        const uint4 ch = g.gchunk[c];
        const int4 nt4 = g.gnote[ch.y];
        if (nt4.w != k) continue;
        const uint32_t beg = g.off[ch.x], len = g.off[ch.x + 1] - beg;
        const uint32_t c_end = min(len, (ch.z + 1u) * kGiantChunk);
        for (uint32_t j0 = ch.z * kGiantChunk + threadIdx.x; j0 < c_end; j0 += kHvU * kLocBlock) {
            LocalNotify<P> nt[kHvU];
#pragma unroll
            for (int x = 0; x < kHvU; ++x) { const uint32_t j = j0 + (uint32_t)x * kLocBlock; nt[x].load(p, beg + j, g.val, mark_cur, nt4.x, nt4.y, k, j < c_end, nt4.z != 0); }
#pragma unroll
            for (int x = 0; x < kHvU; ++x) nt[x].store(mark_next, k);
        }
    }
}

constexpr uint32_t kFinWords = 2048;
static __global__ __launch_bounds__(kBlock) void k_local_finish(LocalGraph g, int32_t add, int32_t *__restrict__ out,
                                                         uint32_t *present, LocalCtrl *ctrl)
{
    __shared__ uint32_t sh_bits[kFinWords];
    for (uint32_t i = threadIdx.x; i < kFinWords; i += kBlock) sh_bits[i] = 0u;
    __syncthreads();
    int32_t mx = 0;
    for (uint32_t id = blockIdx.x * kBlock + threadIdx.x; id < g.n; id += gridDim.x * kBlock) {
        const int32_t v = g.val[id];
        out[g.gid[id]] = v + add;
        mx = max(mx, v);
        const uint32_t wd = (uint32_t)v >> 5, bit = 1u << ((uint32_t)v & 31u);
        if (wd < kFinWords) { if (!(sh_bits[wd] & bit)) atomicOr(&sh_bits[wd], bit); }
        else atomicOr(&present[wd], bit);
    }
    __shared__ int32_t sh_mx;
    if (threadIdx.x == 0) sh_mx = 0;
    __syncthreads();
    for (uint32_t i = threadIdx.x; i < kFinWords; i += kBlock) if (sh_bits[i]) atomicOr(&present[i], sh_bits[i]);
    for (int o = 32; o > 0; o >>= 1) mx = max(mx, __shfl_xor(mx, o));
    if (lane_id() == 0 && mx) atomicMax(&sh_mx, mx);
    __syncthreads();
    if (threadIdx.x == 0 && sh_mx) atomicMax(&ctrl->max_val, sh_mx);
}
static __global__ __launch_bounds__(kBlock) void k_local_levels(const uint32_t *__restrict__ present, uint32_t words, const uint32_t *__restrict__ cnt, LocalCtrl *ctrl)
{
    if (blockIdx.x == 0 && threadIdx.x == 0) { uint32_t e = 0; for (int i = 0; i < kCntWays; ++i) e += cnt[(4 * kCntWays + i) * 32]; ctrl->evals = e; }
    uint32_t c = 0;
    for (uint32_t i = blockIdx.x * kBlock + threadIdx.x; i < words; i += gridDim.x * kBlock) c += (uint32_t)__popc(present[i]);
    c = wave_sum(c);
    if (lane_id() == 0 && c) atomicAdd(&ctrl->levels, c);
}

template <class P>
int local_fixpoint(komb_ctx *ctx, LocalCtrl *d_ctrl, uint32_t *d_cnt, const LocalGraph &g, const P &p, uint64_t total_items, int *launches_out)
{
    hipStream_t s = ctx->stream;
    const int grid = 512;
    const uint32_t nlight_all = g.n - g.nh;
    const int list_grid = (int)std::min<uint32_t>(256u, (nlight_all + kListBlock - 1) / kListBlock ? (nlight_all + kListBlock - 1) / kListBlock : 1u);
    EventSet evs;
    hipEvent_t ev[2] = {nullptr, nullptr};
    KOMB_HIP(ctx, evs.make(&ev[0], hipEventDisableTiming));
    KOMB_HIP(ctx, evs.make(&ev[1], hipEventDisableTiming));
    LocalCtrl *h = ctx->h_local;
    const uint64_t max_launches = total_items + (uint64_t)g.n + 64u;
    int launches = 0, slot = 0, status = KOMB_OK;
    bool have_prev = false, finished = false, stuck = false;
    int32_t k = 0, seen_iters = -1;
    uint32_t full_thr = g.n / 8u + 1u;
#ifdef KOMB_DEBUG_SWITCHES
    if (const char *e = getenv("KOMB_LOCAL_FULL")) { const long d = atol(e); full_thr = d > 0 ? g.n / (uint32_t)d + 1u : 0xFFFFFFFFu; }
#endif
    const char *dbg_env = ctx_opt(ctx, "LOCAL_DEBUG");
    const bool per_sweep = dbg_env && atoi(dbg_env) >= 2;
    std::vector<hipEvent_t> sw;
    if (per_sweep) { sw.resize(1); if (evs.make(&sw[0]) == hipSuccess) (void)hipEventRecord(sw[0], s); }
    while (!finished && (uint64_t)launches < max_launches && k < 0x3FFFFFF0) {
        for (int i = 0; i < kLocBatch; ++i) {
            ++k;
            if (g.flags & kLocUseList) k_local_list<<<list_grid, kListBlock, 0, s>>>(d_ctrl, d_cnt, g, k);
            k_local_step<P><<<grid, kLocBlock, 0, s>>>(d_ctrl, d_cnt, g, p, k, full_thr); ++launches;
            if (g.nchunk && (g.flags & kLocDeferNotify)) k_local_giant_notify<P><<<(int)std::min<uint32_t>(g.nchunk, 1024u), kLocBlock, 0, s>>>(d_ctrl, g, p, k);
            if (per_sweep && sw.size() < 600) { hipEvent_t e2 = nullptr; if (evs.make(&e2) == hipSuccess) { (void)hipEventRecord(e2, s); sw.push_back(e2); } }
        }
        if (hipMemcpyAsync(&h[slot], d_ctrl, sizeof(LocalCtrl), hipMemcpyDeviceToHost, s) != hipSuccess ||
            hipEventRecord(ev[slot], s) != hipSuccess) { status = KOMB_ERR_DEVICE; break; }
        if (have_prev) {
            if (hipEventSynchronize(ev[slot ^ 1]) != hipSuccess) { status = KOMB_ERR_DEVICE; break; }
            if (h[slot ^ 1].done) finished = true;
            else if ((int32_t)h[slot ^ 1].spare[0] == seen_iters) { stuck = true; finished = true; }
            seen_iters = (int32_t)h[slot ^ 1].spare[0];
        }
        have_prev = true;
        slot ^= 1;
    }
    hipError_t e = hipStreamSynchronize(s);
    if (per_sweep) {
        fprintf(stderr, "komb local sweeps (us):");
        for (size_t i = 1; i < sw.size(); ++i) { float ms = 0.f; (void)hipEventElapsedTime(&ms, sw[i - 1], sw[i]); fprintf(stderr, " %.0f", ms * 1e3f); }
        fprintf(stderr, "\n");
    }
    if (launches_out) *launches_out = launches;
    if (status != KOMB_OK || e != hipSuccess)
        KOMB_FAIL(ctx, KOMB_ERR_DEVICE, "local fixed point: HIP failure (%s)", hipGetErrorString(e));
    if (stuck) KOMB_FAIL(ctx, KOMB_ERR_DEVICE, "local fixed point: the sweeps make no progress (sweep %d)", (int)seen_iters);
    return KOMB_OK;
}

static __global__ __launch_bounds__(kBlock) void k_local_zero(uint32_t *a, uint32_t na, uint32_t *b, uint32_t nb, uint32_t *c, uint32_t nc,
                                                       uint32_t *d, uint32_t nd, uint32_t *e, uint32_t ne)
{
    const uint32_t t = blockIdx.x * kBlock + threadIdx.x, step = gridDim.x * kBlock;
    for (uint32_t i = t; i < na; i += step) a[i] = 0u;
    for (uint32_t i = t; i < nb; i += step) b[i] = 0u;
    for (uint32_t i = t; i < nc; i += step) c[i] = 0u;
    for (uint32_t i = t; i < nd; i += step) d[i] = 0u;
    for (uint32_t i = t; i < ne; i += step) e[i] = 0u;
}

struct LocalStats {
    uint32_t units = 0, heavy = 0, levels = 0;
    int32_t max_val = 0;
    int sweeps = 0, launches = 0;
    uint64_t items = 0, evals = 0;
    bool refused = false;
    uint32_t new_limit = 0;
};

template <class LaunchCollect, class RunFix, class AfterNumber>
int local_finish(komb_ctx *ctx, DevBufs &bufs, const PeelCtrl &hc, PeelCtrl *d_ctrl, uint32_t units, const int32_t *marker,
                 const int32_t *key, const int32_t *live_list, uint32_t light_max, size_t item_bytes, uint64_t item_limit, uint32_t max_density, bool use_list, int32_t add, int32_t *out,
                 LaunchCollect &&launch_collect, RunFix &&run_fix, LocalStats *ls, AfterNumber &&after_number)
{
    hipStream_t s = ctx->stream;
    const uint32_t n = hc.remaining;
    if (n == 0) KOMB_FAIL(ctx, KOMB_ERR_STATE, "local finish: nothing left to hand over");
    const bool dbg = ctx_opt(ctx, "LOCAL_DEBUG") != nullptr;
    EventSet evs;
    hipEvent_t ev[5] = {nullptr, nullptr, nullptr, nullptr, nullptr};
    if (dbg) for (auto &e : ev) (void)evs.make(&e);
    auto stamp = [&](int i) { if (dbg) (void)hipEventRecord(ev[i], s); };
    stamp(0);
    const int32_t *list = hc.live_mode ? live_list : nullptr;
    const uint32_t n_in = hc.live_mode ? hc.live_count : units;
    LocalGraph g{};
    int32_t *d_num = nullptr;
    LocalCtrl *d_lctrl = nullptr;
    PeelCtrl *d_cctrl = nullptr;
    uint32_t *d_present = nullptr;
    const size_t present_words = ((size_t)units >> 5) + 2 > kFinWords ? ((size_t)units >> 5) + 2 : (size_t)kFinWords;
    KOMB_HIP(ctx, bufs.alloc(&d_num, (size_t)units));
    KOMB_HIP(ctx, bufs.alloc(&g.off, (size_t)n + 1));
    KOMB_HIP(ctx, bufs.alloc(&g.len, (size_t)n + 1));
    KOMB_HIP(ctx, bufs.alloc(&g.val, (size_t)n));
    KOMB_HIP(ctx, bufs.alloc(&g.mark[0], (size_t)n));
    KOMB_HIP(ctx, bufs.alloc(&g.mark[1], (size_t)n));
    KOMB_HIP(ctx, bufs.alloc(&g.gid, (size_t)n));
    KOMB_HIP(ctx, bufs.alloc(&g.cur, (size_t)n));
    KOMB_HIP(ctx, bufs.alloc(&g.list, (size_t)n));
    KOMB_HIP(ctx, bufs.alloc(&g.giant, (size_t)n));
    KOMB_HIP(ctx, bufs.alloc(&g.khist, (size_t)kKeyBins));
    KOMB_HIP(ctx, bufs.alloc(&d_lctrl, 1));
    uint32_t *d_cnt = nullptr;
    KOMB_HIP(ctx, bufs.alloc(&d_cnt, (size_t)kCntWords + kCntTimerWords));
    KOMB_HIP(ctx, bufs.alloc(&d_cctrl, 1));
    KOMB_HIP(ctx, bufs.alloc(&d_present, present_words));
    static_assert(sizeof(LocalCtrl) % sizeof(uint32_t) == 0, "LocalCtrl is zeroed word by word");
    if (present_words > 0xFFFFFFFFull) KOMB_FAIL(ctx, KOMB_ERR_LIMIT, "local finish: %zu presence words", present_words);
    k_local_zero<<<64, kBlock, 0, s>>>(g.khist, kKeyBins, d_cnt, (uint32_t)(kCntWords + kCntTimerWords), (uint32_t *)d_lctrl, (uint32_t)(sizeof(LocalCtrl) / sizeof(uint32_t)),
                                       g.len + n, 1u, d_present, (uint32_t)present_words);
    void *d_items = nullptr;
    auto release_all = [&]() {
        bufs.release(d_items); bufs.release(d_num); bufs.release(g.off); bufs.release(g.len); bufs.release(g.val);
        bufs.release(g.mark[0]); bufs.release(g.mark[1]); bufs.release(g.gid); bufs.release(g.list); bufs.release(g.giant); bufs.release(g.gchunk); bufs.release(g.gacc); bufs.release(g.gwin); bufs.release(g.gnote);
        bufs.release(g.khist); bufs.release(g.cur); bufs.release(d_lctrl); bufs.release(d_cnt); bufs.release(d_cctrl); bufs.release(d_present);
    };
    g.n = n; g.nh = 0; g.ng = 0; g.nchunk = 0;
    int64_t gb = ((int64_t)n_in + kNumBlock - 1) / kNumBlock;
    k_local_number<<<(int)(gb < 1 ? 1 : (gb > 1024 ? 1024 : gb)), kNumBlock, 0, s>>>(list, n_in, n, marker, key, light_max, d_num, g, d_lctrl);
    LocalCtrl hl{};
    std::vector<uint32_t> kh(kKeyBins);
    if (ctx->h_stage && sizeof(LocalCtrl) + kKeyBins * sizeof(uint32_t) <= kStageBytes) {
        char *st8 = (char *)ctx->h_stage;
        KOMB_HIP(ctx, hipMemcpyAsync(st8, d_lctrl, sizeof(LocalCtrl), hipMemcpyDeviceToHost, s));
        KOMB_HIP(ctx, hipMemcpyAsync(st8 + sizeof(LocalCtrl), g.khist, kKeyBins * sizeof(uint32_t), hipMemcpyDeviceToHost, s));
        KOMB_HIP(ctx, hipStreamSynchronize(s));
        memcpy(&hl, st8, sizeof(LocalCtrl));
        memcpy(kh.data(), st8 + sizeof(LocalCtrl), kKeyBins * sizeof(uint32_t));
    } else {
        KOMB_HIP(ctx, d2h(ctx, &hl, d_lctrl, sizeof(LocalCtrl)));
        KOMB_HIP(ctx, d2h(ctx, kh.data(), g.khist, kKeyBins * sizeof(uint32_t)));
    }
    if (hl.bad || hl.n_heavy + hl.n_light != n)
        KOMB_FAIL(ctx, KOMB_ERR_DEVICE, "local finish: %u live units numbered, the peel counted %u", hl.n_heavy + hl.n_light, n);
    const bool too_dense = max_density && hl.key_sum > (unsigned long long)max_density * n;
    if (hl.key_sum > item_limit || hl.key_sum >= 0xFFFFFFFFull || too_dense) {
        const uint64_t lim = item_limit < 0xFFFFFFFFull ? item_limit : 0xFFFFFFFFull;
        uint64_t nl = (uint64_t)((double)n * ((double)lim / (double)hl.key_sum) * 0.5);
        if (nl >= n) nl = n / 2;
        if (too_dense) nl = 0;
        const uint32_t patch[2] = {(uint32_t)nl, 0u};
        KOMB_HIP(ctx, hipMemcpy(&d_ctrl->tail_limit, &patch[0], sizeof(uint32_t), hipMemcpyHostToDevice));
        KOMB_HIP(ctx, hipMemcpy(&d_ctrl->done, &patch[1], sizeof(uint32_t), hipMemcpyHostToDevice));
        if (dbg) fprintf(stderr, "komb local finish: refused %u units with %llu items (limit %llu); next offer at <= %u units\n", n, (unsigned long long)hl.key_sum, (unsigned long long)item_limit, (uint32_t)nl);
        if (ls) { ls->refused = true; ls->new_limit = (uint32_t)nl; }
        release_all();
        return KOMB_OK;
    }
    KOMB_TRY(prim_exclusive_sum_u32(ctx, g.len, g.off, (int64_t)n + 1));
    const uint32_t total = (uint32_t)hl.key_sum;
    g.nh = hl.n_heavy;
    g.ng = hl.n_giant;
    g.nchunk = hl.n_chunk;
    uint32_t defer_chunks = kLocDeferChunks;
    if (const char *e = ctx_opt(ctx, "LOCAL_DEFER_CHUNKS")) defer_chunks = (uint32_t)strtoul(e, nullptr, 10);
    g.flags = (use_list ? kLocUseList : 0u) | (g.nchunk >= defer_chunks && g.nchunk > 0 ? kLocDeferNotify : 0u);
#ifdef KOMB_DEBUG_SWITCHES
    if (const char *e = getenv("KOMB_LOCAL_MODE")) g.flags = (uint32_t)atoi(e);
#endif
    if (g.ng) {
        KOMB_HIP(ctx, bufs.alloc(&g.gchunk, (size_t)g.nchunk));
        KOMB_HIP(ctx, bufs.alloc(&g.gacc, (size_t)g.ng));
        KOMB_HIP(ctx, bufs.alloc(&g.gwin, (size_t)g.ng * kGiantWin));
        KOMB_HIP(ctx, bufs.alloc(&g.gnote, (size_t)g.ng));
        k_local_chunks<<<(int)(g.ng > 1024u ? 1024u : g.ng), kBlock, 0, s>>>(g);
    }
    int32_t K = 0x7FFFFFFF;
    {
        uint64_t ge = 0;
        for (int32_t k = (int32_t)kKeyBins - 1; k >= 0; --k) {
            ge += kh[(size_t)k];
            if (ge >= (uint64_t)k) { if (k < (int32_t)kKeyBins - 1) K = k; break; }
        }
    }
    stamp(1);
    after_number(g);
    KOMB_HIP(ctx, bufs.alloc((unsigned char **)&d_items, (size_t)total * item_bytes));

    peel_collect_ctrl(s, d_cctrl, d_ctrl);
    PeelCtrl hcc{};
    int32_t cl = 1;
    for (int guard = 0; guard < 16 && hcc.done == 0; ++guard) {
        for (int i = 0; i < 3; ++i) launch_collect(g, d_num, d_items, d_cctrl, cl++);
        KOMB_HIP(ctx, d2h(ctx, &hcc, d_cctrl, sizeof(PeelCtrl)));
        cl = hcc.seq;
    }
    if (hcc.done != 1) KOMB_FAIL(ctx, KOMB_ERR_DEVICE, "local finish: collect pass did not complete (state %d)", hcc.done);
    int64_t gn = ((int64_t)n + kBlock - 1) / kBlock;
    const int grid_n = (int)(gn > 1024 ? 1024 : gn);
    k_local_check<<<grid_n, kBlock, 0, s>>>(g, d_lctrl);
    if (K != 0x7FFFFFFF) k_local_clamp<<<grid_n, kBlock, 0, s>>>(g, K);
    stamp(2);

    int launches = 0;
    KOMB_TRY(run_fix(g, d_items, (uint64_t)total, d_lctrl, d_cnt, &launches));
    stamp(3);
    k_local_finish<<<grid_n, kBlock, 0, s>>>(g, add, out, d_present, d_lctrl);
    k_local_levels<<<(int)(present_words / kBlock + 1 > 256 ? 256 : present_words / kBlock + 1), kBlock, 0, s>>>(d_present, (uint32_t)present_words, d_cnt, d_lctrl);
    stamp(4);
    KOMB_HIP(ctx, d2h(ctx, &hl, d_lctrl, sizeof(LocalCtrl)));
    if (dbg) {
        float t[4] = {0, 0, 0, 0};
        for (int i = 0; i < 4; ++i) (void)hipEventElapsedTime(&t[i], ev[i], ev[i + 1]);
        fprintf(stderr, "komb local finish: %u units (%u heavy, %u of them long; bound %d), %u items; number+scan %.1f us, collect %.1f us, %d sweeps (%d launches, %u evaluations) %.1f us, scatter %.1f us\n",
                n, g.nh, g.ng, K == 0x7FFFFFFF ? -1 : K, total, t[0] * 1e3f, t[1] * 1e3f, hl.iters, launches, hl.evals, t[2] * 1e3f, t[3] * 1e3f);
    }
#ifdef KOMB_LOCAL_TIMERS
    {
        unsigned long long tm[72];
        KOMB_HIP(ctx, d2h(ctx, tm, d_cnt + kCntWords, sizeof(tm)));
        for (int sw = 0; sw < 6; ++sw) {
            const unsigned long long *t = tm + sw * 12;
            const double nwv = t[10] ? (double)t[10] : 1.0;
            fprintf(stderr, "komb local timers, sweep %d (%llu waves), us per wave: hscan %.1f medium %.1f workgroup %.1f setup %.1f load+count %.1f search %.1f notify %.1f; "
                            "batches/wave %.2f groups/wave %.2f; slowest wave %.1f us\n",
                    sw == 0 ? 1 : sw * 4, t[10], t[0] / nwv / 100.0, t[1] / nwv / 100.0, t[2] / nwv / 100.0, t[3] / nwv / 100.0, t[4] / nwv / 100.0, t[5] / nwv / 100.0,
                    t[6] / nwv / 100.0, t[7] / nwv, t[8] / nwv, t[9] / 100.0);
        }
    }
#endif
    if (hl.bad) KOMB_FAIL(ctx, KOMB_ERR_DEVICE, "local finish: %u consistency failures in the compact index", hl.bad);
    if (!hl.done) KOMB_FAIL(ctx, KOMB_ERR_DEVICE, "local finish: launch budget exhausted before the fixed point");
    if (ls) {
        ls->units = n; ls->heavy = g.nh; ls->levels = hl.levels; ls->max_val = hl.max_val;
        ls->sweeps = hl.iters; ls->launches = launches; ls->items = total; ls->evals = hl.evals;
    }
    release_all();
    return KOMB_OK;
}

}
```

### komb_amd/csrc/peel_dev.h

```cpp
#pragma once

#include "common.h"

namespace komb {

enum : int32_t { MODE_SCAN = 0, MODE_PROCESS = 1, MODE_RETIRE = 2 };

#ifndef KOMB_PEEL_BLOCK
#define KOMB_PEEL_BLOCK 1024
#endif
#ifndef KOMB_PEEL_PER_CU
#define KOMB_PEEL_PER_CU 1
#endif
constexpr int kPeelBlock = KOMB_PEEL_BLOCK;
constexpr int kPeelPerCu = KOMB_PEEL_PER_CU;
constexpr int kPeelWaves = kPeelBlock / kWave;
constexpr int kLight = 64;
constexpr int kChunk = 128;
constexpr int kScanU = 4;
constexpr int kItemU = 2;
constexpr int kChainBudget = 16;
constexpr int kStage = 192;
constexpr int kGroup = 32;
constexpr int kMaxGroups = 64;
constexpr int kInitOff = 2 * (kMaxGroups + 1);

struct CtrlView {
    int32_t mode, level, round, done, cur_sel;
    uint32_t cur_light, cur_heavy, remaining;
    uint32_t live_count;
    int32_t live_sel, live_mode;
    uint32_t tail_limit;
};

__device__ __forceinline__ int32_t alive_marker(uint32_t len)
{
    return kAlive - (int32_t)(len <= (uint32_t)kLight ? 0u : (len + kChunk - 1) / kChunk);
}
__device__ __forceinline__ bool marker_alive(int32_t m) { return m >= kAliveMin; }
__device__ __forceinline__ uint32_t marker_chunks(int32_t m) { return (uint32_t)(kAlive - m); }

enum : uint32_t { ST_ALIVE_LIGHT = 0, ST_ALIVE_HEAVY = 1, ST_GONE = 2, ST_ROUND0 = 3 };
enum : int { REL_GONE = 0, REL_NOW = 1, REL_LATER = 2 };
constexpr uint32_t kStateWindow = 253;
constexpr int32_t kRetireEvery = 120;
static_assert(2 * kRetireEvery + 2 < (int32_t)kStateWindow, "state codes must not wrap between two RETIRE steps, even if one were late by a whole period");
__device__ __forceinline__ uint8_t state_of_round(int32_t q) { return (uint8_t)(ST_ROUND0 + (uint32_t)q % kStateWindow); }
__device__ __forceinline__ uint8_t state_of_stamp(int32_t stamp)
{
    if (stamp >= kAliveMin) return (uint8_t)(stamp == kAlive ? ST_ALIVE_LIGHT : ST_ALIVE_HEAVY);
    return stamp == 0 ? (uint8_t)ST_GONE : state_of_round(stamp);
}
__device__ __forceinline__ int32_t marker_of_state(uint32_t c)
{
    return c == ST_ALIVE_LIGHT ? kAlive : (c == ST_ALIVE_HEAVY ? kAlive - 1 : 0);
}
__device__ __forceinline__ int state_rel(uint32_t c, int32_t r)
{
    if (c < ST_GONE) return REL_LATER;
    if (c == ST_GONE) return REL_GONE;
    uint32_t d = c - ST_ROUND0 + kStateWindow - (uint32_t)r % kStateWindow;
    d = d >= kStateWindow ? d - kStateWindow : d;
    return d == 0 ? REL_NOW : (d == 1 ? REL_LATER : REL_GONE);
}

__device__ __forceinline__ int lane_id() { return (int)(threadIdx.x & 63); }
__device__ __forceinline__ uint64_t lanemask_lt() { return (1ull << lane_id()) - 1ull; }

__device__ __forceinline__ uint32_t coherent_load(uint32_t *p) { return atomicAdd(p, 0u); }
__device__ __forceinline__ int32_t coherent_load(int32_t *p) { return atomicAdd(p, 0); }

__device__ __forceinline__ int32_t wave_min(int32_t v)
{
    for (int o = 32; o > 0; o >>= 1) v = min(v, __shfl_xor(v, o));
    return v;
}
__device__ __forceinline__ uint32_t wave_incl_scan(uint32_t v)
{
    const int lane = lane_id();
    for (int o = 1; o < kWave; o <<= 1) {
        const uint32_t t = (uint32_t)__shfl_up((int)v, o);
        if (lane >= o) v += t;
    }
    return v;
}

__device__ __forceinline__ void block_add_u64(unsigned long long v, unsigned long long *dst)
{
    __shared__ unsigned long long sh_blk64[16];
    for (int o = 32; o > 0; o >>= 1) v += __shfl_xor(v, o);
    const int w = (int)(threadIdx.x >> 6), nw = (int)((blockDim.x + 63) >> 6);
    __syncthreads();
    if (lane_id() == 0) sh_blk64[w] = v;
    __syncthreads();
    if (threadIdx.x == 0) { unsigned long long t = 0; for (int i = 0; i < nw; ++i) t += sh_blk64[i]; if (t) atomicAdd(dst, t); }
}
__device__ __forceinline__ void block_add_min(uint32_t add, int32_t mn, uint32_t *dst_add, int32_t *dst_min)
{
    __shared__ uint32_t sh_blk_a[16];
    __shared__ int32_t sh_blk_m[16];
    add = wave_sum(add);
    mn = wave_min(mn);
    const int w = (int)(threadIdx.x >> 6), nw = (int)((blockDim.x + 63) >> 6);
    __syncthreads();
    if (lane_id() == 0) { sh_blk_a[w] = add; sh_blk_m[w] = mn; }
    __syncthreads();
    if (threadIdx.x == 0) {
        uint32_t a = 0; int32_t m = 0x7FFFFFFF;
        for (int i = 0; i < nw; ++i) { a += sh_blk_a[i]; m = min(m, sh_blk_m[i]); }
        if (a) atomicAdd(dst_add, a);
        if (m != 0x7FFFFFFF) atomicMin(dst_min, m);
    }
}

enum : uint8_t { SC_NONE = 0, SC_LIGHT = 1, SC_HEAVY = 2, SC_SURVIVOR = 4 };

struct PeelQueues {
    uint8_t *code;
    int32_t *light[2];
    int2 *heavy[2];
    int32_t *live[2];
    int scalar_scan;
    int32_t *rlevel = nullptr;
};


__device__ __forceinline__ void wave_write_ordered(bool pred, int32_t val, int32_t *q, uint32_t base, uint32_t &run)
{
    const uint64_t m = __ballot(pred);
    if (pred) q[base + run + (uint32_t)__popcll(m & lanemask_lt())] = val;
    run += (uint32_t)__popcll(m);
}

__device__ __forceinline__ void wave_write_chunks(bool pred, int32_t unit, uint32_t nchunks, int2 *q, uint32_t base, uint32_t &run)
{
    uint64_t m = __ballot(pred);
    const int lane = lane_id();
    while (m) {
        const int src = __ffsll((long long)m) - 1;
        m &= m - 1;
        const int32_t u = __shfl(unit, src);
        const uint32_t n = (uint32_t)__shfl((int)nchunks, src);
        for (uint32_t c = (uint32_t)lane; c < n; c += kWave) q[base + run + c] = make_int2(u, (int)c);
        run += n;
    }
}

constexpr int kStageH = 64;
struct WaveStage {
    int32_t *buf;
    int2 *hbuf;
    uint32_t n, hn;
};
__device__ __forceinline__ void stage_flush(WaveStage &st, int32_t *ql, uint32_t *tail_l, int2 *qh, uint32_t *tail_h)
{
    if (st.n == 0 && st.hn == 0) return;
    const int lane = lane_id();
    __builtin_amdgcn_wave_barrier();
    const int2 mine = (uint32_t)lane < st.hn ? st.hbuf[lane] : make_int2(0, 0);
    const uint32_t incl = wave_incl_scan((uint32_t)mine.y);
    const uint32_t total_h = (uint32_t)__shfl((int)incl, kWave - 1);
    uint32_t r = 0;
    if (lane == 0 && st.n) r = atomicAdd(tail_l, st.n);
    else if (lane == 1 && total_h) r = atomicAdd(tail_h, total_h);
    const uint32_t base_l = (uint32_t)__shfl((int)r, 0), base_h = (uint32_t)__shfl((int)r, 1);
    for (uint32_t i = (uint32_t)lane; i < st.n; i += kWave) ql[base_l + i] = st.buf[i];
    const uint32_t excl = incl - (uint32_t)mine.y;
    for (uint32_t k = 0; k < st.hn; ++k) {
        const int32_t u = __shfl(mine.x, (int)k);
        const uint32_t n = (uint32_t)__shfl(mine.y, (int)k);
        const uint32_t o = base_h + (uint32_t)__shfl((int)excl, (int)k);
        for (uint32_t c = (uint32_t)lane; c < n; c += kWave) qh[o + c] = make_int2(u, (int)c);
    }
    __builtin_amdgcn_wave_barrier();
    st.n = 0; st.hn = 0;
}
__device__ __forceinline__ void stage_push(WaveStage &st, bool is_light, bool is_heavy, int32_t unit, uint32_t nchunks,
                                           int32_t *ql, uint32_t *tail_l, int2 *qh, uint32_t *tail_h)
{
    const uint64_t ml = __ballot(is_light), mh = __ballot(is_heavy);
    if ((ml | mh) == 0) return;
    const uint32_t cl = (uint32_t)__popcll(ml), ch = (uint32_t)__popcll(mh);
    if (st.n + cl > (uint32_t)kStage || st.hn + ch > (uint32_t)kStageH) stage_flush(st, ql, tail_l, qh, tail_h);
    if (is_light) st.buf[st.n + (uint32_t)__popcll(ml & lanemask_lt())] = unit;
    if (is_heavy) st.hbuf[st.hn + (uint32_t)__popcll(mh & lanemask_lt())] = make_int2(unit, (int)nchunks);
    st.n += cl; st.hn += ch;
}

constexpr uint32_t kSmallScan = 16384;
#ifndef KOMB_SMALL_LIGHT
#define KOMB_SMALL_LIGHT 64
#endif
#ifndef KOMB_SMALL_HEAVY
#define KOMB_SMALL_HEAVY 4
#endif
constexpr uint32_t kSmallLight = KOMB_SMALL_LIGHT;
constexpr uint32_t kSmallHeavy = KOMB_SMALL_HEAVY;
constexpr uint32_t kMaxInKernelSteps = 8192;

__device__ __forceinline__ uint32_t plan_step(const CtrlView &cv, uint32_t grid, uint32_t &bsz)
{
    bsz = kWave;
    const uint64_t grid_waves = (uint64_t)grid * kPeelWaves;
    while (bsz > 2 && (uint64_t)cv.cur_light < grid_waves * (bsz / 2)) bsz >>= 1;
    if (cv.mode & MODE_RETIRE) return grid;
    if (cv.mode == MODE_SCAN) return (cv.live_mode != 0 && cv.live_count <= kSmallScan) ? 1u : grid;
    if (cv.cur_light <= kSmallLight && cv.cur_heavy <= kSmallHeavy) {
        bsz = 4;
        while (bsz < (uint32_t)kWave && bsz * kPeelWaves < cv.cur_light) bsz <<= 1;
        return 1u;
    }
    const uint64_t wave_jobs = ((uint64_t)cv.cur_light + bsz - 1) / bsz + (uint64_t)cv.cur_heavy;
    const uint64_t need = (wave_jobs + kPeelWaves - 1) / kPeelWaves;
    return (uint32_t)(need < 1 ? 1 : (need > grid ? grid : need));
}

__device__ __forceinline__ void finalize_step(PeelCtrl *ctrl, const CtrlView &cv, uint32_t units, CtrlView *out, uint32_t acc, int32_t launch,
                                              int32_t *rlevel, int32_t retire_every)
{
    const int lane = lane_id();
    if (lane == 0) { (void)atomicExch(&ctrl->seq, launch + 1); asm volatile("s_waitcnt vmcnt(0)" ::: "memory"); }
    __builtin_amdgcn_wave_barrier();
    if (cv.mode & MODE_RETIRE) {
        if (lane == 0) { ctrl->mode = cv.mode & ~MODE_RETIRE; ctrl->last_retire = cv.round; *out = cv; out->mode = cv.mode & ~MODE_RETIRE; }
        return;
    }
    const bool scan = cv.mode == MODE_SCAN;
    const int sel = cv.cur_sel;
    const bool emitted = scan && (cv.live_mode != 0 || cv.remaining <= units / 2);
    const int next_q = scan ? sel : (sel ^ 1);
    uint32_t v = 0;
    if (lane == 1) v = coherent_load(&ctrl->tail_l[next_q]);
    else if (lane == 2) v = coherent_load(&ctrl->tail_h[next_q]);
    else if (lane == 3) v = (uint32_t)atomicExch(&ctrl->next_min, 0x7FFFFFFF);
    else if (lane == 4) v = emitted ? atomicExch(&ctrl->live_tail, 0u) : 0u;
    else if (lane == 5) { if (!scan) atomicExch(&ctrl->tail_l[sel], 0u); }
    else if (lane == 6) { if (!scan) atomicExch(&ctrl->tail_h[sel], 0u); }
    else if (lane == 7) atomicAdd(scan ? &ctrl->n_scans : &ctrl->n_rounds, 1);
    const uint32_t cur_l = (uint32_t)__shfl((int)v, 1), cur_h = (uint32_t)__shfl((int)v, 2);
    const int32_t nmin = __shfl((int)v, 3);
    const uint32_t live_n = (uint32_t)__shfl((int)v, 4);
    if (lane != 0) return;
    if (!scan && rlevel) rlevel[cv.round] = cv.level;
    int32_t mode = cv.mode, level = cv.level, round = cv.round, done = 0, nsel = sel;
    int32_t live_sel = cv.live_sel, live_mode = cv.live_mode;
    uint32_t live_count = cv.live_count;
    const uint32_t remaining = cv.remaining - acc;
    if (scan) {
        if (emitted) { live_count = live_n; live_sel ^= 1; live_mode = 1; }
        if (acc > 0) { atomicAdd(&ctrl->n_levels, 1); ctrl->max_level = level; }
        if (cur_l + cur_h > 0) mode = MODE_PROCESS;
        else if (remaining == 0) done = 1;
        else if (acc > 0) level += 1;
        else if (nmin == 0x7FFFFFFF) done = 2;
        else level = nmin;
    } else {
        nsel = sel ^ 1; round += 1;
        const bool retire = retire_every > 0 && round % retire_every == 0;
        if (cur_l + cur_h == 0) {
            if (remaining == 0) done = 1;
            else {
                level += 1; mode = MODE_SCAN;
                if (remaining <= cv.tail_limit) done = 3;
            }
        }
#ifdef KOMB_TEST_OLD_RETIRE_RULE
        if (retire && !done) mode |= MODE_RETIRE;
#else
        if (retire && done != 1 && done != 2) mode |= MODE_RETIRE;
#endif
        if (retire_every > 0) {
            const int32_t gap = round - ctrl->last_retire;
            if (gap > ctrl->max_retire_gap) ctrl->max_retire_gap = gap;
        }
    }
    ctrl->mode = mode; ctrl->level = level; ctrl->round = round; ctrl->done = done;
    ctrl->cur_sel = nsel; ctrl->cur_light = cur_l; ctrl->cur_heavy = cur_h; ctrl->remaining = remaining;
    ctrl->live_count = live_count; ctrl->live_sel = live_sel; ctrl->live_mode = live_mode;
    out->mode = mode; out->level = level; out->round = round; out->done = done;
    out->cur_sel = nsel; out->cur_light = cur_l; out->cur_heavy = cur_h; out->remaining = remaining;
    out->live_count = live_count; out->live_sel = live_sel; out->live_mode = live_mode;
    out->tail_limit = cv.tail_limit;
}

template <class P, class = void> struct PeelRetire { static constexpr int32_t every = 0; };
template <class P> struct PeelRetire<P, decltype((void)P::kRetireEvery)> { static constexpr int32_t every = P::kRetireEvery; };
template <class P> __host__ __device__ constexpr int32_t peel_retire_every() { return PeelRetire<P>::every; }

template <class P>
__global__ __launch_bounds__(kPeelBlock, (kPeelBlock / 64) * kPeelPerCu / 4) void k_peel_step(PeelCtrl *ctrl, uint32_t *grp_done, PeelQueues Q, P p, int32_t launch)
{
    int32_t retire_every = 0;
    if constexpr (peel_retire_every<P>() > 0) retire_every = p.retire_every;
    __shared__ CtrlView sh_cv;
    __shared__ uint32_t sh_w[kPeelWaves][4];
    __shared__ uint32_t sh_base[3];
    __shared__ uint32_t sh_acc;
    __shared__ int32_t sh_min[kPeelWaves];
    __shared__ uint32_t sh_end[kPeelWaves][kWave];
    __shared__ uint32_t sh_beg[kPeelWaves][kWave];
    __shared__ int32_t sh_unit[kPeelWaves][kWave];
    __shared__ int32_t sh_stage[kPeelWaves][kStage];
    __shared__ int2 sh_stage_h[kPeelWaves][kStageH];

#ifdef KOMB_STEP_TIMERS
    unsigned long long tk[8] = {(unsigned long long)wall_clock64(), 0, 0, 0, 0, 0, 0, 0};
#define KOMB_TK(i) do { if (blockIdx.x == 0 && threadIdx.x == 0) tk[i] = wall_clock64(); } while (0)
#else
#define KOMB_TK(i) do { } while (0)
#endif
    __shared__ int32_t sh_raw[16];
    if (threadIdx.x < 16) sh_raw[threadIdx.x] = reinterpret_cast<const int32_t *>(ctrl)[threadIdx.x];
    __syncthreads();
    if (threadIdx.x == 0) {
        const PeelCtrl *c = reinterpret_cast<const PeelCtrl *>(sh_raw);
        sh_cv.mode = c->mode; sh_cv.level = c->level; sh_cv.round = c->round; sh_cv.done = c->done;
        sh_cv.cur_sel = c->cur_sel; sh_cv.cur_light = c->cur_light; sh_cv.cur_heavy = c->cur_heavy;
        sh_cv.remaining = c->remaining; sh_cv.live_count = c->live_count;
        sh_cv.live_sel = c->live_sel; sh_cv.live_mode = c->live_mode;
        sh_cv.tail_limit = ctrl->tail_limit;
        if (c->seq != launch) sh_cv.done = 1;
    }
    __syncthreads();
    CtrlView cv = sh_cv;
    if (cv.done) return;
    KOMB_TK(1);
    const int lane = lane_id();
    const int w = (int)(threadIdx.x >> 6);

    for (uint32_t chained = 0;; ++chained) {
    uint32_t bsz;
    const uint32_t nblk = plan_step(cv, gridDim.x, bsz);
    if (blockIdx.x >= nblk) return;
    const int L = cv.level;
    const int sel = cv.cur_sel;

    if (cv.mode & MODE_RETIRE) {
        if constexpr (peel_retire_every<P>() > 0) p.retire(cv, blockIdx.x, nblk);
        if (threadIdx.x == 0) sh_acc = 0;
    } else if (cv.mode == MODE_SCAN) {
        const bool from_list = cv.live_mode != 0;
        const bool emit = from_list || cv.remaining <= p.units / 2;
        const uint32_t n_in = from_list ? cv.live_count : p.units;
        const int32_t *live_in = Q.live[cv.live_sel];
        int32_t *live_out = Q.live[cv.live_sel ^ 1];
        const bool vec = !from_list && !Q.scalar_scan;
        const int32_t *s_marker = p.scan_marker(), *s_key = p.scan_key();
        constexpr bool byte_marker = peel_retire_every<P>() > 0;
        const uint8_t *s_state = nullptr;
        if constexpr (byte_marker) s_state = p.scan_state();
        uint32_t n_light = 0, n_chunks = 0, n_hits = 0, n_surv = 0;
        int32_t lmin = 0x7FFFFFFF;
        const uint64_t tile = (uint64_t)kPeelBlock * kScanU;
        auto index_of = [&](uint64_t tb, int k) -> uint64_t {
            return vec ? tb + ((uint64_t)w * kWave + (uint64_t)lane) * kScanU + (uint64_t)k
                       : tb + (uint64_t)k * kPeelBlock + (uint64_t)w * kWave + (uint64_t)lane;
        };
        int4 nm4 = make_int4(0, 0, 0, 0), nk4 = make_int4(0, 0, 0, 0);
        auto fetch = [&](uint64_t tb) {
            const uint64_t i0 = index_of(tb, 0);
            if (vec && tb < n_in && i0 + kScanU <= n_in) {
                if constexpr (byte_marker) nm4.x = (int32_t)*reinterpret_cast<const uint32_t *>(s_state + i0);
                else nm4 = *reinterpret_cast<const int4 *>(s_marker + i0);
                if (s_key) nk4 = *reinterpret_cast<const int4 *>(s_key + i0);
            }
        };
        fetch((uint64_t)blockIdx.x * tile);
        for (uint64_t tb = (uint64_t)blockIdx.x * tile; tb < n_in; tb += (uint64_t)nblk * tile) {
            uint8_t code[kScanU];
            int32_t mk[kScanU], ky[kScanU];
            const uint64_t i0 = index_of(tb, 0);
            const bool whole = vec && i0 + kScanU <= n_in;
            if (whole) {
                static_assert(kScanU == 4, "the dense sweep loads int4");
                if constexpr (byte_marker) {
#pragma unroll
                    for (int k = 0; k < kScanU; ++k) mk[k] = marker_of_state(((uint32_t)nm4.x >> (8 * k)) & 0xFFu);
                } else { mk[0] = nm4.x; mk[1] = nm4.y; mk[2] = nm4.z; mk[3] = nm4.w; }
                ky[0] = nk4.x; ky[1] = nk4.y; ky[2] = nk4.z; ky[3] = nk4.w;
            }
            fetch(tb + (uint64_t)nblk * tile);
#pragma unroll
            for (int k = 0; k < kScanU; ++k) {
                const uint64_t idx = index_of(tb, k);
                code[k] = SC_NONE;
                if (idx < n_in) {
                    if (!whole) {
                        const uint32_t u = from_list ? (uint32_t)live_in[idx] : (uint32_t)idx;
                        if constexpr (byte_marker) mk[k] = marker_of_state(s_state[u]);
                        else mk[k] = s_marker[u];
                        ky[k] = s_key ? s_key[u] : 0;
                    }
                    const bool live = marker_alive(mk[k]);
                    uint32_t nch = marker_chunks(mk[k]);
                    if (live && ky[k] <= L) {
                        if constexpr (byte_marker) if (nch) {
                            const uint32_t u = from_list ? (uint32_t)live_in[idx] : (uint32_t)idx;
                            uint32_t b, len; p.slice(u, b, len); nch = (len + kChunk - 1) / kChunk;
                        }
                        if (nch == 0) code[k] = SC_LIGHT;
                        else { n_chunks += nch; code[k] = SC_HEAVY; }
                    } else if (live) { lmin = min(lmin, ky[k]); code[k] = SC_SURVIVOR; }
                }
            }
            if (whole) *reinterpret_cast<uchar4 *>(Q.code + i0) = make_uchar4(code[0], code[1], code[2], code[3]);
#pragma unroll
            for (int k = 0; k < kScanU; ++k) {
                const uint64_t idx = index_of(tb, k);
                if (!whole && idx < n_in) Q.code[idx] = code[k];
                n_light += code[k] == SC_LIGHT ? 1u : 0u;
                n_hits += (code[k] == SC_LIGHT || code[k] == SC_HEAVY) ? 1u : 0u;
                n_surv += (emit && code[k] == SC_SURVIVOR) ? 1u : 0u;
            }
        }
        n_light = wave_sum(n_light); n_hits = wave_sum(n_hits); n_surv = wave_sum(n_surv);
        n_chunks = wave_sum(n_chunks);
        lmin = wave_min(lmin);
        if (lane == 0) { sh_w[w][0] = n_light; sh_w[w][1] = n_chunks; sh_w[w][2] = n_hits; sh_w[w][3] = n_surv; sh_min[w] = lmin; }
        __syncthreads();
        if (threadIdx.x == 0) {
            uint32_t tl = 0, th = 0, ts = 0, hits = 0;
            int32_t bmin = 0x7FFFFFFF;
            for (int i = 0; i < kPeelWaves; ++i) {
                const uint32_t a = sh_w[i][0], b = sh_w[i][1], c = sh_w[i][3];
                sh_w[i][0] = tl; sh_w[i][1] = th; sh_w[i][3] = ts;
                tl += a; th += b; ts += c; hits += sh_w[i][2];
                bmin = min(bmin, sh_min[i]);
            }
            sh_base[0] = tl ? atomicAdd(&ctrl->tail_l[sel], tl) : 0u;
            sh_base[1] = th ? atomicAdd(&ctrl->tail_h[sel], th) : 0u;
            sh_base[2] = ts ? atomicAdd(&ctrl->live_tail, ts) : 0u;
            sh_acc = hits;
            if (bmin != 0x7FFFFFFF) atomicMin(&ctrl->next_min, bmin);
        }
        __syncthreads();
        const uint32_t base_l = sh_base[0] + sh_w[w][0], base_h = sh_base[1] + sh_w[w][1], base_s = sh_base[2] + sh_w[w][3];
        uint32_t run_l = 0, run_h = 0, run_s = 0;
        auto index_b = [&](uint64_t tb, int k) -> uint64_t {
            return vec ? tb + (uint64_t)w * (kWave * kScanU) + (uint64_t)k * kWave + (uint64_t)lane : index_of(tb, k);
        };
        for (uint64_t tb = (uint64_t)blockIdx.x * tile; tb < n_in; tb += (uint64_t)nblk * tile) {
            uint8_t code[kScanU];
            uint32_t u[kScanU];
#pragma unroll
            for (int k = 0; k < kScanU; ++k) {
                const uint64_t idx = index_b(tb, k);
                code[k] = idx < n_in ? Q.code[idx] : (uint8_t)SC_NONE;
            }
#pragma unroll
            for (int k = 0; k < kScanU; ++k) {
                const uint64_t idx = index_b(tb, k);
                u[k] = 0;
                if (code[k] != SC_NONE) u[k] = from_list ? (uint32_t)live_in[idx] : (uint32_t)idx;
            }
#pragma unroll
            for (int k = 0; k < kScanU; ++k) {
                const bool light = code[k] == SC_LIGHT, heavy = code[k] == SC_HEAVY, surv = code[k] == SC_SURVIVOR;
                uint32_t nch = 0;
                if (heavy) { uint32_t b, len; p.slice(u[k], b, len); nch = (len + kChunk - 1) / kChunk; }
                if (code[k] != SC_NONE && !surv) p.mark_scanned(u[k], cv);
                wave_write_ordered(light, (int32_t)u[k], Q.light[sel], base_l, run_l);
                if (__ballot(heavy)) wave_write_chunks(heavy, (int32_t)u[k], nch, Q.heavy[sel], base_h, run_h);
                if (emit) wave_write_ordered(surv, (int32_t)u[k], live_out, base_s, run_s);
            }
        }
    } else {
        int32_t *qn_l = Q.light[sel ^ 1];
        int2 *qn_h = Q.heavy[sel ^ 1];
        uint32_t *tail_nl = &ctrl->tail_l[sel ^ 1], *tail_nh = &ctrl->tail_h[sel ^ 1];
        WaveStage st{sh_stage[w], sh_stage_h[w], 0u, 0u};
        uint32_t n_trig = 0;
        const uint64_t gw = (uint64_t)blockIdx.x * kPeelWaves + (uint64_t)w;
        const uint64_t nw = (uint64_t)nblk * kPeelWaves;

        auto push_trigger = [&](int32_t t, uint32_t nch) {
            const bool trig = t >= 0;
            const uint64_t m = __ballot(trig);
            if (m == 0) return;
            n_trig += (uint32_t)__popcll(m);
            const bool is_light = trig && nch == 0;
            const bool is_heavy = trig && nch != 0;
            stage_push(st, is_light, is_heavy, t, nch, qn_l, tail_nl, qn_h, tail_nh);
        };
        auto run_items = [&](const bool (&active)[kItemU], const int32_t (&unit)[kItemU], const uint32_t (&pos)[kItemU]) {
            typename P::Loaded ld[kItemU];
#pragma unroll
            for (int k = 0; k < kItemU; ++k)
                if (active[k]) ld[k] = p.item_load(unit[k], pos[k], cv);
            int32_t trg[2 * kItemU];
            uint32_t tch[2 * kItemU];
#pragma unroll
            for (int k = 0; k < kItemU; ++k) {
                trg[2 * k] = -1; trg[2 * k + 1] = -1;
                tch[2 * k] = 0; tch[2 * k + 1] = 0;
                if (active[k]) p.item_apply(ld[k], cv, trg[2 * k], trg[2 * k + 1], tch[2 * k], tch[2 * k + 1]);
            }
#pragma unroll
            for (int k = 0; k < 2 * kItemU; ++k) push_trigger(trg[k], tch[k]);
        };

        const uint64_t n_batches = ((uint64_t)cv.cur_light + bsz - 1) / bsz;
        uint32_t *s_end = sh_end[w], *s_beg = sh_beg[w];
        int32_t *s_unit = sh_unit[w];
        auto run_batch = [&](int32_t unit, uint32_t beg, uint32_t len) {
            const uint32_t incl = wave_incl_scan(len);
            const uint32_t total = (uint32_t)__shfl((int)incl, kWave - 1);
            __builtin_amdgcn_wave_barrier();
            s_end[lane] = incl; s_beg[lane] = beg; s_unit[lane] = unit;
            __builtin_amdgcn_wave_barrier();
            for (uint32_t it0 = 0; it0 < total; it0 += kWave * kItemU) {
                bool active[kItemU];
                int32_t me[kItemU];
                uint32_t pos[kItemU];
#pragma unroll
                for (int k = 0; k < kItemU; ++k) {
                    const uint32_t it = it0 + (uint32_t)(k * kWave + lane);
                    active[k] = it < total;
                    me[k] = -1; pos[k] = 0;
                    if (active[k]) {
                        int lo = 0;
#pragma unroll
                        for (int st = kWave / 2; st > 0; st >>= 1) lo += (s_end[lo + st - 1] <= it) ? st : 0;
                        const uint32_t first = lo ? s_end[lo - 1] : 0u;
                        me[k] = s_unit[lo];
                        pos[k] = s_beg[lo] + (it - first);
                    }
                }
                run_items(active, me, pos);
            }
            __builtin_amdgcn_wave_barrier();
        };
        const uint64_t n_jobs = n_batches + (uint64_t)cv.cur_heavy;
        for (uint64_t job = gw; job < n_jobs; job += nw) {
            if (job < n_batches) {
                const uint64_t idx = job * bsz + (uint64_t)lane;
                int32_t unit = -1;
                uint32_t beg = 0, len = 0;
                if ((uint32_t)lane < bsz && idx < cv.cur_light) { unit = Q.light[sel][idx]; p.slice((uint32_t)unit, beg, len); }
#ifdef KOMB_STEP_TIMERS
                if (blockIdx.x == 0 && threadIdx.x == 0 && tk[2] == 0) { asm volatile("s_waitcnt vmcnt(0)" ::: "memory"); tk[2] = wall_clock64(); }
#endif
                run_batch(unit, beg, len);
                continue;
            }
            const int2 ent = Q.heavy[sel][job - n_batches];
            uint32_t beg, len;
            p.slice((uint32_t)ent.x, beg, len);
#ifdef KOMB_STEP_TIMERS
            if (blockIdx.x == 0 && threadIdx.x == 0 && tk[2] == 0) { asm volatile("s_waitcnt vmcnt(0)" ::: "memory"); tk[2] = wall_clock64(); }
#endif
            const uint32_t c0 = (uint32_t)ent.y * kChunk;
            const uint32_t c1 = min(len, c0 + (uint32_t)kChunk);
            for (uint32_t it0 = c0; it0 < c1; it0 += kWave * kItemU) {
                bool active[kItemU];
                int32_t me[kItemU];
                uint32_t pos[kItemU];
#pragma unroll
                for (int k = 0; k < kItemU; ++k) {
                    const uint32_t it = it0 + (uint32_t)(k * kWave + lane);
                    active[k] = it < c1; me[k] = ent.x; pos[k] = beg + it;
                }
                run_items(active, me, pos);
            }
        }
        if (P::kChain) {
            for (int budget = kChainBudget; budget > 0 && st.n > 0; --budget) {
                const uint32_t take = st.n < (uint32_t)kWave ? st.n : (uint32_t)kWave;
                int32_t unit = -1;
                uint32_t beg = 0, len = 0;
                __builtin_amdgcn_wave_barrier();
                if ((uint32_t)lane < take) { unit = st.buf[st.n - take + (uint32_t)lane]; p.slice((uint32_t)unit, beg, len); }
                __builtin_amdgcn_wave_barrier();
                st.n -= take;
                run_batch(unit, beg, len);
            }
        }
        KOMB_TK(3);
        stage_flush(st, qn_l, tail_nl, qn_h, tail_nh);
#ifdef KOMB_STEP_TIMERS
        if (blockIdx.x == 0 && threadIdx.x == 0) { asm volatile("s_waitcnt vmcnt(0)" ::: "memory"); tk[4] = wall_clock64(); }
#endif
        if (lane == 0) sh_w[w][3] = n_trig;
        __syncthreads();
        if (threadIdx.x == 0) {
            uint32_t t = 0;
            for (int i = 0; i < kPeelWaves; ++i) t += sh_w[i][3];
            sh_acc = t;
        }
    }

    __syncthreads();
    KOMB_TK(5);
    if (nblk > 1) {
        if (threadIdx.x >= kWave) return;
        int last = 0;
        uint32_t total = 0;
        if (lane == 0) {
            asm volatile("s_waitcnt vmcnt(0)" ::: "memory");
            unsigned long long *tick = reinterpret_cast<unsigned long long *>(grp_done);
            const uint32_t grp = blockIdx.x / kGroup;
            const uint32_t ngrp = (nblk + kGroup - 1) / kGroup;
            const uint32_t grp_size = (grp == ngrp - 1) ? (nblk - grp * kGroup) : (uint32_t)kGroup;
            const uint32_t mine = sh_acc;
            const unsigned long long old = atomicAdd(&tick[grp], (1ull << 32) | mine);
            if ((uint32_t)(old >> 32) == grp_size - 1) {
                atomicExch(&tick[grp], 0ull);
                const uint32_t grp_acc = (uint32_t)old + mine;
                if (ngrp == 1) { last = 1; total = grp_acc; }
                else {
                    const unsigned long long old2 = atomicAdd(&tick[kMaxGroups], (1ull << 32) | grp_acc);
                    if ((uint32_t)(old2 >> 32) == ngrp - 1) {
                        atomicExch(&tick[kMaxGroups], 0ull);
                        last = 1; total = (uint32_t)old2 + grp_acc;
                    }
                }
            }
        }
#ifdef KOMB_STEP_TIMERS
        if (blockIdx.x == 0 && threadIdx.x == 0 && cv.mode == MODE_PROCESS && cv.cur_light + cv.cur_heavy < 16384 && tk[2] != 0) {
            tk[6] = wall_clock64();
            for (int i = 0; i < 6; ++i) atomicAdd(&ctrl->pad1[i], (uint32_t)(tk[i + 1] - tk[i]));
            atomicAdd(&ctrl->pad1[6], 1u);
        }
#endif
        last = __shfl(last, 0);
        total = (uint32_t)__shfl((int)total, 0);
        if (last) finalize_step(ctrl, cv, p.units, &sh_cv, total, launch, Q.rlevel, retire_every);
        return;
    }
    if (threadIdx.x < kWave) finalize_step(ctrl, cv, p.units, &sh_cv, sh_acc, launch, Q.rlevel, retire_every);
    if (P::kSingleStep) return;
    __syncthreads();
    cv = sh_cv;
    if (cv.done || chained >= kMaxInKernelSteps) return;
    uint32_t next_bsz;
    if (plan_step(cv, gridDim.x, next_bsz) != 1u) return;
    }
}

}
```

### komb_amd/csrc/truss_gather.h

```cpp
#pragma once

#include "peel_dev.h"

namespace komb {

namespace {

__global__ __launch_bounds__(kBlock) void k_truss_results(const int32_t *__restrict__ stamp, const int32_t *__restrict__ rlevel,
                                                         const int32_t *__restrict__ truss,
                                                         const uint32_t *__restrict__ e2k, int64_t m, uint32_t k_lo, uint32_t k_hi,
                                                         int32_t *__restrict__ tr_out)
{
    for (int64_t e = (int64_t)blockIdx.x * kBlock + threadIdx.x; e < m; e += (int64_t)gridDim.x * kBlock) {
        const int32_t s = stamp[e];
        const int32_t t = marker_alive(s) ? truss[e] : rlevel[s] + 2;
        const uint32_t k = e2k[e];
        if (k - k_lo < k_hi - k_lo) tr_out[k] = t;
    }
}

__global__ __launch_bounds__(kBlock) void k_scatter_len(const uint2 *__restrict__ off2, const uint32_t *__restrict__ e2k, int64_t m,
                                                       uint32_t k_lo, uint32_t k_hi, int32_t *__restrict__ out)
{
    for (int64_t e = (int64_t)blockIdx.x * kBlock + threadIdx.x; e < m; e += (int64_t)gridDim.x * kBlock) {
        const uint32_t k = e2k[e];
        if (k - k_lo < k_hi - k_lo) out[k] = (int32_t)off2[e].y;
    }
}

}

}
```

### komb_amd/csrc/truss_index.h

```cpp
#pragma once

#include "peel_dev.h"

namespace komb {

namespace {

constexpr int kBinBits = 11;
constexpr uint32_t kBinEdges = 1u << kBinBits;
#ifndef KOMB_CHUNK_BITS
#define KOMB_CHUNK_BITS 6
#endif
constexpr int kChunkBits = KOMB_CHUNK_BITS;
constexpr uint32_t kChunkMask = (1u << kChunkBits) - 1u;
struct BinGeom {
    int nb_bits;
    uint32_t nb;
    __host__ __device__ uint32_t bin_of(uint32_t e) const { return (e >> kChunkBits) & (nb - 1u); }
    __host__ __device__ uint32_t local_of(uint32_t e) const { return ((e >> (kChunkBits + nb_bits)) << kChunkBits) | (e & kChunkMask); }
    __host__ __device__ uint64_t edge_of(uint32_t b, uint32_t i) const
    {
        return ((((uint64_t)(i >> kChunkBits) << nb_bits) | b) << kChunkBits) | (i & kChunkMask);
    }
    __host__ __device__ uint32_t sentinel_base() const { return (uint32_t)(((uint64_t)kBinEdges >> kChunkBits) << (kChunkBits + nb_bits)); }
};
inline BinGeom bin_geom(int64_t m)
{
    BinGeom g{0, 1u};
    while (((int64_t)g.nb << kBinBits) < m) { ++g.nb_bits; g.nb <<= 1; }
    return g;
}

__global__ __launch_bounds__(kBlock) void k_bin_offsets(const uint32_t *__restrict__ key, int64_t n, BinGeom g, uint32_t *__restrict__ boff)
{
    for (int64_t b = (int64_t)blockIdx.x * kBlock + threadIdx.x; b <= (int64_t)g.nb; b += (int64_t)gridDim.x * kBlock) {
        int64_t lo = 0, hi = n;
        while (lo < hi) {
            const int64_t mid = lo + ((hi - lo) >> 1);
            if ((int64_t)g.bin_of(key[mid]) < b) lo = mid + 1; else hi = mid;
        }
        boff[b] = (uint32_t)lo;
    }
}

__global__ __launch_bounds__(kBlock) void k_count_mismatch(const uint32_t *__restrict__ a, const uint32_t *__restrict__ b, int64_t n,
                                                           unsigned long long *__restrict__ bad)
{
    unsigned long long t = 0;
    for (int64_t e = (int64_t)blockIdx.x * kBlock + threadIdx.x; e < n; e += (int64_t)gridDim.x * kBlock) t += a[e] != b[e] ? 1ull : 0ull;
    block_add_u64(t, bad);
}

constexpr int kCntU = 4;
constexpr int kCntE = (int)(kBinEdges / kBlock);
static_assert(kBlock % (1 << kChunkBits) == 0, "a thread's edges sit at one place in different chunks of the bin");
__global__ __launch_bounds__(kBlock, 8) void k_bin_count(const uint32_t *__restrict__ key, const uint32_t *__restrict__ boff, BinGeom g,
                                                      const uint32_t *__restrict__ own, int64_t m, uint32_t *__restrict__ sum,
                                                      uint32_t *__restrict__ bin_total, unsigned long long *__restrict__ total,
                                                      int32_t *__restrict__ min_pos)
{
    __shared__ uint32_t sh_cnt[kBinEdges];
    __shared__ uint32_t sh_part[kBlock / kWave];
    unsigned long long t = 0;
    int32_t lmin = 0x7FFFFFFF;
    uint32_t n0 = 0, n1 = 0;
    uint32_t kq[kCntU];
    auto first_keys = [&](uint32_t r0, uint32_t r1) {
#pragma unroll
        for (int u = 0; u < kCntU; ++u) {
            const uint64_t r = (uint64_t)r0 + threadIdx.x + (uint64_t)u * kBlock;
            kq[u] = r < r1 ? key[r] : 0xFFFFFFFFu;
        }
    };
    if (blockIdx.x < g.nb) { n0 = boff[blockIdx.x]; n1 = boff[blockIdx.x + 1]; first_keys(n0, n1); }
    for (uint32_t b = blockIdx.x; b < g.nb; b += gridDim.x) {
        const uint32_t r0 = n0, r1 = n1;
        const uint32_t bn = b + gridDim.x;
        const bool more = bn > b && bn < g.nb;
        if (more) { n0 = boff[bn]; n1 = boff[bn + 1]; }
        const uint64_t e_first = g.edge_of(b, threadIdx.x), e_step = (uint64_t)(kBlock >> kChunkBits) << (kChunkBits + g.nb_bits);
        uint32_t ow[kCntE];
#pragma unroll
        for (int u = 0; u < kCntE; ++u) {
            const uint64_t e = e_first + (uint64_t)u * e_step;
            ow[u] = e < (uint64_t)m ? own[e] : 0u;
        }
        for (uint32_t i = threadIdx.x; i < kBinEdges; i += kBlock) sh_cnt[i] = 0u;
        __syncthreads();
        for (uint64_t r = (uint64_t)r0 + threadIdx.x; r < r1; r += (uint64_t)kBlock * kCntU) {
            uint32_t k[kCntU];
            if (r < (uint64_t)r0 + kBlock) {
#pragma unroll
                for (int u = 0; u < kCntU; ++u) k[u] = kq[u];
            } else {
#pragma unroll
                for (int u = 0; u < kCntU; ++u) {
                    const uint64_t rr = r + (uint64_t)u * kBlock;
                    k[u] = rr < r1 ? key[rr] : 0xFFFFFFFFu;
                }
            }
#pragma unroll
            for (int u = 0; u < kCntU; ++u) {
                const uint64_t rr = r + (uint64_t)u * kBlock;
                if (rr < r1 && (int64_t)k[u] < m) atomicAdd(&sh_cnt[g.local_of(k[u])], 1u);
            }
        }
        __syncthreads();
#pragma unroll
        for (int u = 0; u < kCntE; ++u) asm volatile("" : "+v"(ow[u]));
        if (more) first_keys(n0, n1);
        uint32_t tb = 0;
#pragma unroll
        for (int u = 0; u < kCntE; ++u) {
            const uint32_t i = threadIdx.x + (uint32_t)u * kBlock;
            const uint64_t e = e_first + (uint64_t)u * e_step;
            if (e >= (uint64_t)m) continue;
            const uint32_t c = ow[u] + sh_cnt[i];
            sum[e] = c;
            tb += c;
            if (c) lmin = min(lmin, (int32_t)c);
        }
        tb = wave_sum(tb);
        if (lane_id() == 0) sh_part[threadIdx.x >> 6] = tb;
        __syncthreads();
        if (threadIdx.x == 0) {
            uint32_t all = 0;
            for (int i = 0; i < kBlock / kWave; ++i) all += sh_part[i];
            bin_total[b] = all;
            t += all;
        }
        __syncthreads();
    }
    if (blockIdx.x == 0 && threadIdx.x == 0) { sum[m] = 0u; bin_total[g.nb] = 0u; }
    if (threadIdx.x == 0 && t) atomicAdd(total, t);
    lmin = wave_min(lmin);
    if (lane_id() == 0 && lmin != 0x7FFFFFFF) atomicMin(min_pos, lmin);
}

constexpr int kFinBlock = 512;
#ifndef KOMB_FIN_PER_CU
#define KOMB_FIN_PER_CU 2
#endif
#ifndef KOMB_WIN_CAP
#define KOMB_WIN_CAP 7168
#endif
constexpr int kFinPerCu = KOMB_FIN_PER_CU;
constexpr uint32_t kWinCap = KOMB_WIN_CAP;
constexpr int kFinE = (int)(kBinEdges / kFinBlock);
constexpr int kFinU = 4;
static_assert((kWinCap * 8 + 2 * kBinEdges * 4 + 512) * kFinPerCu <= 160 * 1024, "the finishing workgroups of a CU: windows and tables are sized for gfx950's 160 KB of LDS");
static_assert(kWinCap * 8 >= (2 * kBinEdges + 4) * 4 + kBinEdges * 8, "the window buffer doubles as the table of the in-place copy");
static_assert(kFinE == 4 && kFinE <= (1 << kChunkBits), "a thread's edges are 4 consecutive ones of a chunk: their supports and own-role counts are one 16-byte vector each");
__global__ __launch_bounds__(kFinBlock, (kFinBlock / 64) * kFinPerCu / 4) void k_bin_finish(const uint32_t *__restrict__ key, const int2 *__restrict__ val,
                                                         const uint32_t *__restrict__ boff, BinGeom g,
                                                         const uint32_t *__restrict__ own, const uint32_t *__restrict__ cnt,
                                                         const uint32_t *__restrict__ bin_base,
                                                         const int2 *__restrict__ own_dense, const unsigned long long *__restrict__ ownoff,
                                                         int2 *__restrict__ dense, int64_t m,
                                                         uint2 *__restrict__ off2, int32_t *__restrict__ sup, int32_t *__restrict__ stamp, uint8_t *__restrict__ st8,
                                                         uint32_t *__restrict__ init, int32_t *__restrict__ light0)
{
    __shared__ uint32_t sh_off[kBinEdges + 4];
    __shared__ uint32_t sh_cur[kBinEdges];
    __shared__ uint32_t sh_wsum[kFinBlock / kWave];
    __shared__ int2 sh_win[kWinCap];
    __shared__ uint32_t sh_hsum[kFinBlock / kWave];
    __shared__ uint32_t sh_qbase;
    const int lane = lane_id(), w = (int)(threadIdx.x >> 6);
    uint32_t zeros = 0;
    const int32_t L1 = (int32_t)init[1];
    const bool queue_first = light0 != nullptr && L1 <= kLight;
    for (uint32_t b = blockIdx.x; b < g.nb; b += gridDim.x) {
        const uint64_t r0 = boff[b], r1 = boff[b + 1];
        const uint32_t base = bin_base[b];
        const uint32_t i0 = threadIdx.x * (uint32_t)kFinE;
        const uint64_t e0 = g.edge_of(b, i0);
        const uint32_t nin = e0 >= (uint64_t)m ? 0u : (uint32_t)min((uint64_t)kFinE, (uint64_t)m - e0);
        uint32_t c[kFinE], ow[kFinE];
        unsigned long long oo[kFinE];
        if (nin == (uint32_t)kFinE) {
            const uint4 v = *reinterpret_cast<const uint4 *>(cnt + e0);
            const uint4 q = *reinterpret_cast<const uint4 *>(own + e0);
            c[0] = v.x; c[1] = v.y; c[2] = v.z; c[3] = v.w;
            ow[0] = q.x; ow[1] = q.y; ow[2] = q.z; ow[3] = q.w;
        } else {
#pragma unroll
            for (int u = 0; u < kFinE; ++u) { const bool in = (uint32_t)u < nin; c[u] = in ? cnt[e0 + u] : 0u; ow[u] = in ? own[e0 + u] : 0u; }
        }
#pragma unroll
        for (int u = 0; u < kFinE; ++u) oo[u] = ow[u] ? ownoff[e0 + u] : 0ull;
        const uint32_t mine = c[0] + c[1] + c[2] + c[3];
        const uint32_t incl = wave_incl_scan(mine);
        uint32_t hits = 0;
#pragma unroll
        for (int u = 0; u < kFinE; ++u) hits += (queue_first && (int32_t)c[u] == L1) ? 1u : 0u;
        const uint32_t hincl = wave_incl_scan(hits);
        if (lane == kWave - 1) { sh_wsum[w] = incl; sh_hsum[w] = hincl; }
        __syncthreads();
        uint32_t before = 0, hbefore = 0, hall = 0;
#pragma unroll
        for (int i = 0; i < kFinBlock / kWave; ++i) { before += i < w ? sh_wsum[i] : 0u; hbefore += i < w ? sh_hsum[i] : 0u; hall += sh_hsum[i]; }
        if (threadIdx.x == 0 && hall) sh_qbase = atomicAdd(&init[2], hall);
        uint32_t o[kFinE + 1];
        o[0] = before + incl - mine;
#pragma unroll
        for (int u = 0; u < kFinE; ++u) o[u + 1] = o[u] + c[u];
#pragma unroll
        for (int u = 0; u < kFinE; ++u) { sh_off[i0 + u] = o[u]; sh_cur[i0 + u] = o[u]; }
        if (threadIdx.x == kFinBlock - 1) sh_off[kBinEdges] = o[kFinE];
        if (nin == (uint32_t)kFinE) {
            reinterpret_cast<uint4 *>(off2 + e0)[0] = make_uint4(base + o[0], c[0], base + o[1], c[1]);
            reinterpret_cast<uint4 *>(off2 + e0)[1] = make_uint4(base + o[2], c[2], base + o[3], c[3]);
            int4 sv, mv;
            int32_t *svp = &sv.x, *mvp = &mv.x;
#pragma unroll
            for (int u = 0; u < kFinE; ++u) {
                const bool first = queue_first && (int32_t)c[u] == L1;
                svp[u] = (int32_t)c[u];
                mvp[u] = first ? 1 : (c[u] ? alive_marker(c[u]) : 0);
                if (!c[u]) ++zeros;
            }
            *reinterpret_cast<int4 *>(sup + e0) = sv;
            *reinterpret_cast<int4 *>(stamp + e0) = mv;
            *reinterpret_cast<uchar4 *>(st8 + e0) = make_uchar4(state_of_stamp(mv.x), state_of_stamp(mv.y), state_of_stamp(mv.z), state_of_stamp(mv.w));
        } else {
#pragma unroll
            for (int u = 0; u < kFinE; ++u) if ((uint32_t)u < nin) {
                const uint64_t e = e0 + u;
                const bool first = queue_first && (int32_t)c[u] == L1;
                off2[e] = make_uint2(base + o[u], c[u]);
                sup[e] = (int32_t)c[u];
                stamp[e] = first ? 1 : (c[u] ? alive_marker(c[u]) : 0);
                st8[e] = state_of_stamp(stamp[e]);
                if (!c[u]) ++zeros;
            }
        }
        __syncthreads();
        if (hall) {
            uint32_t q = sh_qbase + hbefore + hincl - hits;
#pragma unroll
            for (int u = 0; u < kFinE; ++u) if (queue_first && (int32_t)c[u] == L1 && (uint32_t)u < nin) light0[q++] = (int32_t)(e0 + u);
        }
        const uint32_t W = sh_off[kBinEdges];
        const bool inwin = W <= kWinCap;
        for (uint64_t r = r0 + threadIdx.x; r < r1; r += (uint64_t)kFinBlock * kFinU) {
            uint32_t k[kFinU];
            int2 v[kFinU];
#pragma unroll
            for (int u = 0; u < kFinU; ++u) {
                const uint64_t rr = r + (uint64_t)u * kFinBlock;
                if (rr < r1) { k[u] = key[rr]; v[u] = val[rr]; }
            }
#pragma unroll
            for (int u = 0; u < kFinU; ++u) {
                const uint64_t rr = r + (uint64_t)u * kFinBlock;
                if (rr < r1 && (int64_t)k[u] < m) {
                    const uint32_t p = atomicAdd(&sh_cur[g.local_of(k[u])], 1u);
                    if (inwin) sh_win[p] = v[u]; else dense[base + p] = v[u];
                }
            }
        }
        if (inwin) {
            uint32_t most = 0;
#pragma unroll
            for (int u = 0; u < kFinE; ++u) most = max(most, ow[u]);
            for (uint32_t kk = 0; kk < most; ++kk) {
                int2 t[kFinE];
#pragma unroll
                for (int u = 0; u < kFinE; ++u) if (kk < ow[u]) t[u] = own_dense[oo[u] + kk];
#pragma unroll
                for (int u = 0; u < kFinE; ++u) if (kk < ow[u]) sh_win[o[u + 1] - ow[u] + kk] = t[u];
            }
        } else {
            uint32_t *tab_pre = reinterpret_cast<uint32_t *>(sh_win), *tab_dst = tab_pre + kBinEdges + 4;
            unsigned long long *tab_src = reinterpret_cast<unsigned long long *>(tab_dst + kBinEdges);
            const uint32_t mine_ow = ow[0] + ow[1] + ow[2] + ow[3];
            const uint32_t incl_ow = wave_incl_scan(mine_ow);
            __syncthreads();
            if (lane == kWave - 1) sh_wsum[w] = incl_ow;
            __syncthreads();
            uint32_t before_ow = 0, total_ow = 0;
#pragma unroll
            for (int i = 0; i < kFinBlock / kWave; ++i) { before_ow += i < w ? sh_wsum[i] : 0u; total_ow += sh_wsum[i]; }
            uint32_t run = before_ow + incl_ow - mine_ow;
#pragma unroll
            for (int u = 0; u < kFinE; ++u) {
                tab_pre[i0 + u] = run; tab_dst[i0 + u] = o[u + 1] - ow[u]; tab_src[i0 + u] = oo[u];
                run += ow[u];
            }
            if (threadIdx.x == kFinBlock - 1) tab_pre[kBinEdges] = run;
            __syncthreads();
            for (uint32_t x = threadIdx.x; x < total_ow; x += kFinBlock) {
                uint32_t lo = 0;
#pragma unroll
                for (uint32_t st = kBinEdges / 2; st > 0; st >>= 1) lo += (tab_pre[lo + st] <= x) ? st : 0u;
                const uint32_t kk = x - tab_pre[lo];
                dense[base + tab_dst[lo] + kk] = own_dense[tab_src[lo] + kk];
            }
        }
        __syncthreads();
        if (inwin) for (uint32_t j = threadIdx.x; j < W; j += kFinBlock) dense[base + j] = sh_win[j];
        __syncthreads();
    }
    block_add_min(zeros, 0x7FFFFFFF, &init[0], (int32_t *)&init[1]);
}

__global__ __launch_bounds__(kBlock) void k_peel_init(int64_t m, const uint32_t *__restrict__ off, uint2 *__restrict__ off2,
                                                      int32_t *__restrict__ sup, int32_t *__restrict__ stamp, uint8_t *__restrict__ st8,
                                                      uint32_t *__restrict__ init)
{
    uint32_t zeros = 0;
    int32_t lmin = 0x7FFFFFFF;
    for (int64_t e = (int64_t)blockIdx.x * kBlock + threadIdx.x; e < m; e += (int64_t)gridDim.x * kBlock) {
        const uint32_t b0 = off[e];
        const int32_t s0 = (int32_t)(off[e + 1] - b0);
        off2[e] = make_uint2(b0, (uint32_t)s0);
        sup[e] = s0;
        if (s0 == 0) { stamp[e] = 0; st8[e] = (uint8_t)ST_GONE; ++zeros; }
        else { const int32_t a = alive_marker((uint32_t)s0); stamp[e] = a; st8[e] = state_of_stamp(a); lmin = min(lmin, s0); }
    }
    block_add_min(zeros, lmin, &init[0], (int32_t *)&init[1]);
}

}

}
```

### komb_amd/csrc/truss_tail.h

```cpp
#pragma once

#include "peel_dev.h"

namespace komb {
namespace {

constexpr uint32_t kTailEdges = 32768;
constexpr uint32_t kTailMaxEdges = 65534;
constexpr uint32_t kTailMaxV = 1024;
constexpr uint32_t kTailRowWords = kTailMaxV / 64;
constexpr uint32_t kTailPoolWords = 40448;
constexpr uint32_t kTailPark = 128;
constexpr uint32_t kTailMinQueue = 512;
constexpr uint32_t kTFrontier = 0xFFFFu, kTDead = 0xFFFEu;

struct TailBufs {
    int32_t *vmap;
    uint32_t *cnt;
    int32_t *vlist;
    unsigned long long *rows;
    uint32_t *pair;
    int32_t *sup;
    int32_t *gid;
    int32_t *gid_by_rank;
    uint32_t *pair_by_rank;
    int32_t *truss_by_rank;
    uint32_t *spill[2];
    uint32_t max_edges;
};

__global__ __launch_bounds__(kBlock) void k_tail_mark(const int32_t *__restrict__ list, uint32_t n_in, const int32_t *__restrict__ sup,
                                                      const int32_t *__restrict__ stamp,
                                                      const int32_t *__restrict__ osrc, const int32_t *__restrict__ ocol, TailBufs T)
{
    __shared__ uint32_t seen[32];
    if (threadIdx.x < 32) seen[threadIdx.x] = 0u;
    __syncthreads();
    uint32_t live = 0;
    unsigned long long work = 0;
    for (uint32_t i = blockIdx.x * kBlock + threadIdx.x; i < n_in; i += gridDim.x * kBlock) {
        const int32_t e = list ? list[i] : (int32_t)i;
        if (!marker_alive(stamp[e])) continue;
        ++live;
        const uint32_t sv = (uint32_t)sup[e];
        work += sv;
        atomicOr(&seen[min(sv, 1023u) >> 5], 1u << (min(sv, 1023u) & 31u));
        const int32_t ab[2] = {osrc[e], ocol[e]};
        for (int k = 0; k < 2; ++k)
            if (atomicExch(&T.vmap[ab[k]], 1) == 0) {
                const uint32_t id = atomicAdd(&T.cnt[0], 1u);
                if (id < kTailMaxV) T.vlist[id] = ab[k];
            }
    }
    live = wave_sum(live);
    for (int o = 32; o > 0; o >>= 1) work += __shfl_xor(work, o);
    if (lane_id() == 0 && live) {
        atomicAdd(&T.cnt[1], live);
        atomicAdd(reinterpret_cast<unsigned long long *>(&T.cnt[4]), work);
    }
    __syncthreads();
    if (threadIdx.x < 32 && seen[threadIdx.x]) atomicOr(&T.cnt[16 + threadIdx.x], seen[threadIdx.x]);
}

constexpr unsigned long long kTailWorkPerLevel = 145000ull;
__global__ __launch_bounds__(kTailMaxV) void k_tail_number(TailBufs T)
{
    __shared__ int32_t ids[kTailMaxV];
    __shared__ uint32_t distinct;
    const uint32_t n = T.cnt[0], ne = T.cnt[1];
    if (threadIdx.x == 0) distinct = 0;
    __syncthreads();
    if (threadIdx.x < 32) atomicAdd(&distinct, (uint32_t)__popc(T.cnt[16 + threadIdx.x]));
    __syncthreads();
    const unsigned long long work = *reinterpret_cast<const unsigned long long *>(&T.cnt[4]);
    if (n > kTailMaxV || ne > kTailMaxEdges || ne > T.max_edges || ne == 0 || work > kTailWorkPerLevel * distinct) {
        if (threadIdx.x == 0) T.cnt[2] = 1u;
        return;
    }
    const uint32_t t = threadIdx.x;
    if (t < n) ids[t] = T.vlist[t];
    __syncthreads();
    if (t < n) {
        const int32_t mine = ids[t];
        uint32_t rank = 0;
        for (uint32_t j = 0; j < n; ++j) rank += ids[j] < mine ? 1u : 0u;
        T.vmap[mine] = (int32_t)rank + 1;
        T.vlist[rank] = mine;
    }
}

__global__ __launch_bounds__(kBlock) void k_tail_rows(const int32_t *__restrict__ list, uint32_t n_in, const int32_t *__restrict__ sup,
                                                      const int32_t *__restrict__ stamp,
                                                      const int32_t *__restrict__ osrc, const int32_t *__restrict__ ocol, TailBufs T)
{
    if (T.cnt[2]) return;
    for (uint32_t i0 = blockIdx.x * kBlock; i0 < n_in; i0 += gridDim.x * kBlock) {
        const uint32_t i = i0 + threadIdx.x;
        int32_t e = -1;
        int32_t st = 0;
        if (i < n_in) { e = list ? list[i] : (int32_t)i; st = stamp[e]; }
        const bool live = e >= 0 && marker_alive(st);
        const uint64_t m = __ballot(live);
        uint32_t base = 0;
        if (lane_id() == 0 && m) base = atomicAdd(&T.cnt[3], (uint32_t)__popcll(m));
        base = (uint32_t)__shfl((int)base, 0);
        if (!live) continue;
        const uint32_t u = (uint32_t)T.vmap[osrc[e]] - 1u, v = (uint32_t)T.vmap[ocol[e]] - 1u;
        atomicOr(&T.rows[(size_t)u * kTailRowWords + (v >> 6)], 1ull << (v & 63));
        atomicOr(&T.rows[(size_t)v * kTailRowWords + (u >> 6)], 1ull << (u & 63));
        const uint32_t j = base + (uint32_t)__popcll(m & lanemask_lt());
        T.pair[j] = (min(u, v) << 16) | max(u, v);
        T.sup[j] = sup[e];
        T.gid[j] = e;
    }
}

struct TailLds {
    unsigned long long *A;
    unsigned long long *U;
    uint16_t *pre;
    int32_t *base;
    uint32_t *S;
    uint32_t *park;
    uint32_t *q[2];
    uint32_t W, cap;
};

__device__ __forceinline__ uint32_t tail_tri(uint32_t u, uint32_t W)
{
    const uint32_t b = u >> 6;
    return 64u * (b * W - b * (b - 1) / 2) + (u - 64u * b) * (W - b);
}
__device__ __forceinline__ unsigned long long tail_upmask(uint32_t u, uint32_t j)
{
    const uint32_t ju = u >> 6;
    if (j > ju) return ~0ull;
    if (j < ju) return 0ull;
    return (u & 63) == 63 ? 0ull : (~0ull << ((u & 63) + 1));
}
__device__ __forceinline__ uint32_t tail_rank(const TailLds &t, uint32_t lo, uint32_t hi)
{
    const uint32_t w = tail_tri(lo, t.W) + (hi >> 6) - (lo >> 6);
    const unsigned long long bits = t.U[w] & ((1ull << (hi & 63)) - 1ull);
    return (uint32_t)t.base[lo] + (uint32_t)t.pre[w] + (uint32_t)__popcll(bits);
}
__device__ __forceinline__ uint32_t tail_sup(const TailLds &t, uint32_t r) { return (t.S[r >> 1] >> (16 * (r & 1))) & 0xFFFFu; }
__device__ __forceinline__ void tail_to_frontier(const TailLds &t, uint32_t r) { atomicOr(&t.S[r >> 1], 0xFFFFu << (16 * (r & 1))); }
__device__ __forceinline__ void tail_to_dead(const TailLds &t, uint32_t r) { atomicAnd(&t.S[r >> 1], ~(1u << (16 * (r & 1)))); }

__global__ __launch_bounds__(1024) void k_truss_tail(PeelCtrl *ctrl, TailBufs T, int32_t *__restrict__ truss)
{
    __shared__ __attribute__((aligned(16))) uint32_t pool[kTailPoolWords];
    __shared__ uint32_t sh_cnt[2];
    __shared__ int32_t sh_min;
    __shared__ int32_t sh_ok;
    const uint32_t tid = threadIdx.x;
    const int lane = lane_id();
#ifdef KOMB_TAIL_TIMERS
    unsigned long long tm[8] = {0, 0, 0, 0, 0, 0, 0, 0}, tlast = wall_clock64();
    auto tick = [&](int k) { const unsigned long long now = wall_clock64(); tm[k] += now - tlast; tlast = now; };
#else
    auto tick = [](int) {};
#endif
    const uint32_t n = T.cnt[0], E = T.cnt[1];
    TailLds t;
    t.W = (n + 63) / 64;
    const uint32_t tri = tail_tri(n, t.W);
    const uint32_t wA = n * t.W * 2, wU = tri * 2, wPre = (tri + 1) / 2, wBase = n, wS = (E + 1) / 2, wPark = 16 * kTailPark;
    const uint32_t used = wA + wU + wPre + wBase + wS + wPark;
    const bool ok = T.cnt[2] == 0 && T.cnt[3] == E && n <= kTailMaxV && used + 2 * kTailMinQueue <= kTailPoolWords;
    if (!ok) {
        if (tid == 0) { ctrl->tail_limit = ctrl->remaining / 2; ctrl->done = 0; }
        return;
    }
    t.A = reinterpret_cast<unsigned long long *>(pool);
    t.U = reinterpret_cast<unsigned long long *>(pool + wA);
    t.pre = reinterpret_cast<uint16_t *>(pool + wA + wU);
    t.base = reinterpret_cast<int32_t *>(pool + wA + wU + wPre);
    t.S = pool + wA + wU + wPre + wBase;
    t.park = t.S + wS;
    t.cap = (kTailPoolWords - used) / 2;
    t.q[0] = pool + used;
    t.q[1] = pool + used + t.cap;

    for (uint32_t w = tid; w < n * t.W; w += 1024) {
        const uint32_t u = w / t.W, j = w % t.W;
        const unsigned long long bits = T.rows[(size_t)u * kTailRowWords + j];
        t.A[w] = bits;
        if (j >= (u >> 6)) t.U[tail_tri(u, t.W) + j - (u >> 6)] = bits & tail_upmask(u, j);
    }
    for (uint32_t w = tid; w < wS; w += 1024) t.S[w] = 0u;
    if (tid == 0) { sh_cnt[0] = sh_cnt[1] = 0u; sh_ok = 1; }
    __syncthreads();
    tick(6);
    if (tid < n) {
        uint32_t run = 0;
        const uint32_t w0 = tail_tri(tid, t.W), nw = t.W - (tid >> 6);
        for (uint32_t j = 0; j < nw; ++j) {
            t.pre[w0 + j] = (uint16_t)run;
            run += (uint32_t)__popcll(t.U[w0 + j]);
        }
        t.base[tid] = (int32_t)run;
    }
    __syncthreads();
    if (tid < kWave) {
        uint32_t carry = 0;
        for (uint32_t c0 = 0; c0 < n; c0 += kWave) {
            const uint32_t i = c0 + (uint32_t)lane;
            const uint32_t v = i < n ? (uint32_t)t.base[i] : 0u;
            const uint32_t incl = wave_incl_scan(v);
            if (i < n) t.base[i] = (int32_t)(carry + incl - v);
            carry += (uint32_t)__shfl((int)incl, kWave - 1);
        }
        if (lane == 0 && carry != E) sh_ok = 0;
    }
    __syncthreads();
    if (!sh_ok) {
        if (tid == 0) { ctrl->tail_limit = 0; ctrl->done = 0; }
        return;
    }
    tick(7);
    for (uint32_t j = tid; j < E; j += 1024) {
        const uint32_t code = T.pair[j], lo = code >> 16, hi = code & 0xFFFFu;
        const uint32_t r = tail_rank(t, lo, hi);
        atomicOr(&t.S[r >> 1], ((uint32_t)T.sup[j] & 0xFFFFu) << (16 * (r & 1)));
        T.gid_by_rank[r] = T.gid[j];
        T.pair_by_rank[r] = code;
    }
    __syncthreads();

    auto q_get = [&](int sel, uint32_t i) -> uint32_t {
        const uint32_t *q = sel ? t.q[1] : t.q[0];
        uint32_t *sp = sel ? T.spill[1] : T.spill[0];
        return i < t.cap ? q[i] : __hip_atomic_load(&sp[i - t.cap], __ATOMIC_RELAXED, __HIP_MEMORY_SCOPE_AGENT);
    };
    auto q_push = [&](int sel, uint32_t code) {
        uint32_t *q = sel ? t.q[1] : t.q[0];
        uint32_t *sp = sel ? T.spill[1] : T.spill[0];
        const uint32_t slot = atomicAdd(&sh_cnt[sel], 1u);
        if (slot < t.cap) q[slot] = code;
        else __hip_atomic_store(&sp[slot - t.cap], code, __ATOMIC_RELAXED, __HIP_MEMORY_SCOPE_AGENT);
    };
    tick(0);
    int32_t L = ctrl->level;
    uint32_t alive = E, rounds = 0, levels = 0;
    int32_t max_level = ctrl->max_level;
    int sel = 0;
    int32_t state = 1;
    const uint32_t gl = (uint32_t)lane & 15u;
    uint32_t *park = t.park + (tid >> 6) * kTailPark;
    while (alive > 0) {
        if (tid == 0) { sh_cnt[sel] = 0u; sh_cnt[sel ^ 1] = 0u; sh_min = 0x7FFFFFFF; }
        __syncthreads();
        int32_t lmin = 0x7FFFFFFF;
        for (uint32_t w = tid; w < wS; w += 1024) {
            const uint32_t two = t.S[w];
            const uint32_t s0 = two & 0xFFFFu, s1 = two >> 16;
            if (s0 < kTDead) lmin = min(lmin, (int32_t)s0);
            if (s1 < kTDead && 2 * w + 1 < E) lmin = min(lmin, (int32_t)s1);
        }
        lmin = wave_min(lmin);
        if (lane == 0 && lmin != 0x7FFFFFFF) atomicMin(&sh_min, lmin);
        __syncthreads();
        if (sh_min == 0x7FFFFFFF) { state = 2; break; }
        L = max(L, sh_min);
        for (uint32_t w = tid; w < wS; w += 1024) {
            const uint32_t two = t.S[w];
#pragma unroll
            for (uint32_t h = 0; h < 2; ++h) {
                const uint32_t s = (two >> (16 * h)) & 0xFFFFu, r = 2 * w + h;
                if (s < kTDead && r < E && (int32_t)s <= L) {
                    q_push(sel, __hip_atomic_load(&T.pair_by_rank[r], __ATOMIC_RELAXED, __HIP_MEMORY_SCOPE_AGENT));
                    tail_to_frontier(t, r);
                    T.truss_by_rank[r] = L + 2;
                }
            }
        }
        __syncthreads();
        uint32_t ncur = sh_cnt[sel];
        tick(1);
        ++levels; max_level = L;
        while (ncur > 0) {
            uint32_t npark = 0;
            auto handle = [&](bool valid, uint32_t item) {
                const uint32_t u = item & 1023u, v = (item >> 10) & 1023u, x = item >> 20;
                const uint32_t code = (u << 16) | v;
                const uint32_t k1 = (min(u, x) << 16) | max(u, x), k2 = (min(v, x) << 16) | max(v, x);
                bool t1 = false, t2 = false;
                if (valid) {
                    const uint32_t r1 = tail_rank(t, k1 >> 16, k1 & 0xFFFFu), r2 = tail_rank(t, k2 >> 16, k2 & 0xFFFFu);
                    const uint32_t s1 = tail_sup(t, r1), s2 = tail_sup(t, r2);
                    const bool f1 = s1 == kTFrontier, f2 = s2 == kTFrontier;
                    if (!f1 && (!f2 || code < k2)) {
                        const uint32_t sh = 16 * (r1 & 1);
                        t1 = (int32_t)((atomicSub(&t.S[r1 >> 1], 1u << sh) >> sh) & 0xFFFFu) == L + 1;
                    }
                    if (!f2 && (!f1 || code < k1)) {
                        const uint32_t sh = 16 * (r2 & 1);
                        t2 = (int32_t)((atomicSub(&t.S[r2 >> 1], 1u << sh) >> sh) & 0xFFFFu) == L + 1;
                    }
                }
                if (t1) q_push(sel ^ 1, k1);
                if (t2) q_push(sel ^ 1, k2);
            };
            for (uint32_t i0 = (tid >> 6) * 4; i0 < ncur; i0 += 64) {
                const uint32_t i = i0 + ((uint32_t)lane >> 4);
                uint32_t u = 0, v = 0;
                unsigned long long bits = 0ull;
                if (i < ncur) {
                    const uint32_t code = q_get(sel, i);
                    u = code >> 16; v = code & 0xFFFFu;
                    if (gl < t.W) bits = t.A[u * t.W + gl] & t.A[v * t.W + gl];
                }
                const uint32_t uv = u | (v << 10);
                while (true) {
                    const bool has = bits != 0ull;
                    const uint64_t m = __ballot(has);
                    if (m == 0) break;
                    if (has) {
                        const uint32_t x = gl * 64 + (uint32_t)__ffsll((long long)bits) - 1u;
                        bits &= bits - 1ull;
                        park[npark + (uint32_t)__popcll(m & lanemask_lt())] = uv | (x << 20);
                    }
                    npark += (uint32_t)__popcll(m);
                    __builtin_amdgcn_wave_barrier();
                    if (npark >= (uint32_t)kWave) {
                        npark -= kWave;
                        const uint32_t item = park[npark + (uint32_t)lane];
                        __builtin_amdgcn_wave_barrier();
                        handle(true, item);
                    }
                }
            }
            __builtin_amdgcn_wave_barrier();
            if (npark) handle((uint32_t)lane < npark, park[(uint32_t)lane < npark ? lane : 0]);
            __syncthreads();
            tick(3);
            const uint32_t nnext = sh_cnt[sel ^ 1];
            if (tid == 0) sh_cnt[sel] = 0u;
            for (uint32_t i = tid; i < ncur; i += 1024) {
                const uint32_t code = q_get(sel, i);
                const uint32_t u = code >> 16, v = code & 0xFFFFu;
                tail_to_dead(t, tail_rank(t, u, v));
                atomicAnd(&t.A[u * t.W + (v >> 6)], ~(1ull << (v & 63)));
                atomicAnd(&t.A[v * t.W + (u >> 6)], ~(1ull << (u & 63)));
            }
            for (uint32_t i = tid; i < nnext; i += 1024) {
                const uint32_t code = q_get(sel ^ 1, i);
                const uint32_t r = tail_rank(t, code >> 16, code & 0xFFFFu);
                tail_to_frontier(t, r);
                T.truss_by_rank[r] = L + 2;
            }
            __syncthreads();
            tick(4);
            alive -= ncur;
            ++rounds;
            ncur = nnext;
            sel ^= 1;
        }
        L += 1;
    }
    __syncthreads();
    for (uint32_t r = tid; r < E; r += 1024)
        truss[__hip_atomic_load(&T.gid_by_rank[r], __ATOMIC_RELAXED, __HIP_MEMORY_SCOPE_AGENT)] =
            __hip_atomic_load(&T.truss_by_rank[r], __ATOMIC_RELAXED, __HIP_MEMORY_SCOPE_AGENT);
    tick(5);
    if (tid == 0) {
#ifdef KOMB_TAIL_TIMERS
        for (int k = 0; k < 8; ++k) T.cnt[8 + k] = (uint32_t)tm[k];
#endif
        ctrl->remaining = alive;
        ctrl->n_levels += (int32_t)levels;
        ctrl->n_rounds += (int32_t)rounds;
        ctrl->n_scans += (int32_t)levels;
        ctrl->max_level = max_level;
        ctrl->level = L;
        ctrl->done = state;
    }
}

}
}
```

Measured before the change: 4.203 billion.

## Drop per-edge stamp array and freeze support as truss level in peel

Removes the 32-bit per-edge stamp and separate truss/rlevel arrays from the k-truss peel. Liveness now comes from the 8-bit state array, and a peeled edge's support slot is overwritten with its level, so the support array doubles as the result. Support now reuses the triangle count buffer, which saves allocations and per-edge memory traffic in init, scan and trigger paths. The cost is threading a new state pointer through the local-finish, tail and shard paths, plus an extra conversion kernel when sharding.

After: 4.249 billion, median of 6. No clear change (+1.1%).

```diff
diff --git a/komb_amd/csrc/common.h b/komb_amd/csrc/common.h
--- a/komb_amd/csrc/common.h
+++ b/komb_amd/csrc/common.h
@@ -49,7 +49,8 @@
     int32_t  done;
     uint32_t cur_light;
     uint32_t cur_heavy;
-    int32_t  cur_sel;
+    int16_t  cur_sel;
+    int16_t  cur_src;
     uint32_t remaining;
     int32_t  n_levels;
     int32_t  n_rounds;
diff --git a/komb_amd/csrc/kcore.hip b/komb_amd/csrc/kcore.hip
--- a/komb_amd/csrc/kcore.hip
+++ b/komb_amd/csrc/kcore.hip
@@ -288,7 +288,7 @@
         (void)hipEventRecord(ev[0], s);
         KOMB_HIP(ctx, hipMemsetAsync(d_livebits, 0, live_words * sizeof(unsigned long long), s));
         LocalStats ls;
-        const int rc = local_finish(ctx, bufs, hc, d_ctrl, (uint32_t)nv, ctx->d_core, d_degw, Q.live[hc.live_sel],
+        const int rc = local_finish(ctx, bufs, hc, d_ctrl, (uint32_t)nv, ctx->d_core, nullptr, d_degw, Q.live[hc.live_sel],
             (uint32_t)kWave * CoreLocal::kU, sizeof(uint32_t), local_item_limit(ctx, std::max<uint64_t>(kCoreLocalItems, (uint64_t)ctx->ne / 3)), 0u, false, 0, ctx->d_core,
             [&](const LocalGraph &lg, const int32_t *num, void *items, PeelCtrl *d_cctrl, int32_t launch) {
                 CoreCollect C{(uint32_t)nv, ctx->d_o_rowptr, ctx->d_o_col, ctx->d_core, d_livebits, num, lg.off, lg.cur, (uint32_t *)items};
diff --git a/komb_amd/csrc/ktruss.hip b/komb_amd/csrc/ktruss.hip
--- a/komb_amd/csrc/ktruss.hip
+++ b/komb_amd/csrc/ktruss.hip
@@ -24,8 +24,8 @@
     const uint2 *off2;
     const int2 *inc;
     int32_t *sup;
-    int32_t *stamp;
     uint8_t *st8;
+    static constexpr bool kFreezeKey = true;
     static constexpr int32_t kRetireEvery = komb::kRetireEvery;
     int32_t retire_every;
 #ifdef KOMB_DEBUG_SWITCHES
@@ -55,10 +55,11 @@
         }
     }
 
-    __device__ __forceinline__ const int32_t *scan_marker() const { return stamp; }
     __device__ __forceinline__ const uint8_t *scan_state() const { return st8; }
     __device__ __forceinline__ const int32_t *scan_key() const { return sup; }
-    __device__ __forceinline__ void mark_scanned(uint32_t e, const CtrlView &cv) const { stamp[e] = cv.round; st8[e] = state_of_round(cv.round); }
+    __device__ __forceinline__ void mark_scanned(uint32_t e, const CtrlView &cv) const { st8[e] = state_of_round(cv.round); }
+    __device__ __forceinline__ void freeze_key(int32_t e, const CtrlView &cv) const { sup[e] = cv.level; }
+    __device__ __forceinline__ uint32_t chunks_of(int32_t e) const { return (off2[e].y + (uint32_t)kChunk - 1u) / (uint32_t)kChunk; }
     __device__ __forceinline__ void slice(uint32_t e, uint32_t &b, uint32_t &len) const
     {
         const uint2 o = off2[e];
@@ -96,12 +97,12 @@
         if (ablate & 1) { decx = false; decy = false; }
 #endif
         if (decx && atomicSub(&sup[ld.x], 1) == L + 1) {
-            c0 = ld.cx == ST_ALIVE_HEAVY ? marker_chunks(stamp[ld.x]) : 0u;
-            stamp[ld.x] = r + 1; st8[ld.x] = state_of_round(r + 1); t0 = ld.x;
+            c0 = ld.cx == ST_ALIVE_HEAVY ? chunks_of(ld.x) : 0u;
+            st8[ld.x] = state_of_round(r + 1); t0 = ld.x;
         }
         if (decy && atomicSub(&sup[ld.y], 1) == L + 1) {
-            c1 = ld.cy == ST_ALIVE_HEAVY ? marker_chunks(stamp[ld.y]) : 0u;
-            stamp[ld.y] = r + 1; st8[ld.y] = state_of_round(r + 1); t1 = ld.y;
+            c1 = ld.cy == ST_ALIVE_HEAVY ? chunks_of(ld.y) : 0u;
+            st8[ld.y] = state_of_round(r + 1); t1 = ld.y;
         }
     }
 };
@@ -114,11 +115,12 @@
     const int2 *inc;
     int32_t *sup;
     int32_t *stamp;
+    uint8_t *st8;
     uint32_t lo, hi;
 
     __device__ __forceinline__ const int32_t *scan_marker() const { return stamp; }
     __device__ __forceinline__ const int32_t *scan_key() const { return sup; }
-    __device__ __forceinline__ void mark_scanned(uint32_t e, const CtrlView &cv) const { stamp[e] = cv.round; }
+    __device__ __forceinline__ void mark_scanned(uint32_t e, const CtrlView &cv) const { stamp[e] = cv.round; st8[e] = (uint8_t)ST_GONE; sup[e] = cv.level; }
     __device__ __forceinline__ void slice(uint32_t e, uint32_t &b, uint32_t &len) const
     {
         const uint2 o = off2[e];
@@ -147,19 +149,25 @@
     }
 };
 
+__global__ __launch_bounds__(kBlock) void k_shard_stamps(const uint8_t *__restrict__ st8, int64_t m, int32_t *__restrict__ stamp)
+{
+    for (int64_t e = (int64_t)blockIdx.x * kBlock + threadIdx.x; e < m; e += (int64_t)gridDim.x * kBlock)
+        stamp[e] = state_alive(st8[e]) ? kAlive : 0;
+}
+
 struct TrussCollect {
     static constexpr bool kChain = false;
     static constexpr bool kSingleStep = false;
     uint32_t units;
     const uint2 *off2;
     const int2 *inc;
-    const int32_t *stamp;
+    const uint8_t *st8;
     const int32_t *num;
     const uint32_t *coff;
     uint32_t *cur;
     uint2 *cpair;
 
-    __device__ __forceinline__ const int32_t *scan_marker() const { return stamp; }
+    __device__ __forceinline__ const uint8_t *scan_state() const { return st8; }
     __device__ __forceinline__ const int32_t *scan_key() const { return nullptr; }
     __device__ __forceinline__ void mark_scanned(uint32_t, const CtrlView &) const {}
     __device__ __forceinline__ void slice(uint32_t e, uint32_t &b, uint32_t &len) const
@@ -168,18 +176,18 @@
         b = o.x;
         len = o.y;
     }
-    struct Loaded { int32_t me, x, y, sx, sy; };
+    struct Loaded { int32_t me, x, y; uint32_t cx, cy; };
     __device__ __forceinline__ Loaded item_load(int32_t me, uint32_t pos, const CtrlView &) const
     {
         Loaded ld;
         const int2 p = inc[pos];
         ld.me = me; ld.x = p.x; ld.y = p.y;
-        ld.sx = stamp[p.x]; ld.sy = stamp[p.y];
+        ld.cx = st8[p.x]; ld.cy = st8[p.y];
         return ld;
     }
     __device__ __forceinline__ void item_apply(const Loaded &ld, const CtrlView &, int32_t &, int32_t &, uint32_t &, uint32_t &) const
     {
-        if (!marker_alive(ld.sx) || !marker_alive(ld.sy)) return;
+        if (!state_alive(ld.cx) || !state_alive(ld.cy)) return;
         const uint32_t id = (uint32_t)num[ld.me];
         const uint32_t b0 = coff[id], k = local_slot(id, cur);
         if (k < coff[id + 1] - b0) cpair[b0 + k] = make_uint2((uint32_t)num[ld.x], (uint32_t)num[ld.y]);
@@ -522,20 +530,18 @@
     uint32_t total = 0;
     const uint32_t sum_supports = (uint32_t)st.triangles * 3u;
     int2 *d_inc = nullptr;
-    int32_t *d_sup = nullptr, *d_stamp = nullptr, *d_truss = nullptr;
+    int32_t *d_sup = reinterpret_cast<int32_t *>(d_cnt);
+    int32_t *d_stamp = nullptr;
     uint8_t *d_st8 = nullptr;
     bool peel_inited = false;
     if (layout == IDX_STREAM) {
         KOMB_TRY(prim_exclusive_sum_u32(ctx, d_bintot, d_bintot, n_bins + 1));
         total = sum_supports;
         KOMB_HIP(ctx, bufs.alloc(&d_inc, (size_t)total));
-        KOMB_HIP(ctx, bufs.alloc(&d_sup, (size_t)m));
-        KOMB_HIP(ctx, bufs.alloc(&d_stamp, (size_t)m));
         KOMB_HIP(ctx, bufs.alloc(&d_st8, (size_t)m + 16));
-        KOMB_HIP(ctx, bufs.alloc(&d_truss, (size_t)m));
         ctx->timer.start(s);
         k_bin_finish<<<grid_for(n_bins, 1, 256 * kFinPerCu), kFinBlock, 0, s>>>(d_reckey, d_recval, d_toff, geom, d_own, d_cnt, d_bintot, d_owndense, d_ownoff, d_inc, m,
-                                                                      d_off2, d_sup, d_stamp, d_st8, d_grp + kInitOff, d_light0);
+                                                                      d_off2, d_st8, d_grp + kInitOff, d_light0);
         st.ms_compact += ctx->timer.stop(s);
         peel_inited = true;
         bufs.release(d_toff); bufs.release(d_bintot); bufs.release((void *)d_recval); bufs.release(d_reckey);
@@ -552,17 +558,14 @@
         st.ms_tri_fill = ctx->timer.stop(s);
     }
     st.ms_support = st.ms_tri_count + st.ms_tri_fill + st.ms_sort + st.ms_compact;
-    bufs.release(d_cnt); bufs.release(d_own);
+    bufs.release(d_own);
 
     phase.next("truss: peel");
     PeelCtrl *d_ctrl = nullptr;
     PeelQueues Q{nullptr, {nullptr, nullptr}, {nullptr, nullptr}, {nullptr, nullptr}, 0};
     const size_t heavy_cap = (size_t)total / 32 + 64;
     if (!peel_inited) {
-        KOMB_HIP(ctx, bufs.alloc(&d_sup, (size_t)m));
-        KOMB_HIP(ctx, bufs.alloc(&d_stamp, (size_t)m));
         KOMB_HIP(ctx, bufs.alloc(&d_st8, (size_t)m + 16));
-        KOMB_HIP(ctx, bufs.alloc(&d_truss, (size_t)m));
         KOMB_HIP(ctx, bufs.alloc(&d_grp, (size_t)kInitOff + 4));
     }
     for (int i = 0; i < 2; ++i) {
@@ -573,14 +576,13 @@
     }
     KOMB_HIP(ctx, bufs.alloc(&d_ctrl, 1));
     KOMB_HIP(ctx, bufs.alloc(&Q.code, (size_t)m));
-    KOMB_HIP(ctx, bufs.alloc(&Q.rlevel, (size_t)m + 2));
-    KOMB_HIP(ctx, hipMemsetAsync(Q.rlevel, 0, 2 * sizeof(int32_t), s));
+    if (shard_peel_on) KOMB_HIP(ctx, bufs.alloc(&d_stamp, (size_t)m));
     int32_t retire_every = kRetireEvery;
     if (const char *e = ctx_opt(ctx, "RETIRE_EVERY")) retire_every = std::max(1, std::min((int)kRetireEvery, atoi(e)));
 #ifdef KOMB_DEBUG_SWITCHES
-    TrussProblem P{(uint32_t)m, d_off2, d_inc, d_sup, d_stamp, d_st8, retire_every, getenv("KOMB_PEEL_ABLATE") ? atoi(getenv("KOMB_PEEL_ABLATE")) : 0};
+    TrussProblem P{(uint32_t)m, d_off2, d_inc, d_sup, d_st8, retire_every, getenv("KOMB_PEEL_ABLATE") ? atoi(getenv("KOMB_PEEL_ABLATE")) : 0};
 #else
-    TrussProblem P{(uint32_t)m, d_off2, d_inc, d_sup, d_stamp, d_st8, retire_every};
+    TrussProblem P{(uint32_t)m, d_off2, d_inc, d_sup, d_st8, retire_every};
 #endif
     TailBufs T{};
     if (fin == FIN_LDS && tail_limit) {
@@ -593,7 +595,7 @@
         KOMB_HIP(ctx, bufs.alloc(&T.gid, (size_t)tail_limit));
         KOMB_HIP(ctx, bufs.alloc(&T.gid_by_rank, (size_t)tail_limit));
         KOMB_HIP(ctx, bufs.alloc(&T.pair_by_rank, (size_t)tail_limit));
-        KOMB_HIP(ctx, bufs.alloc(&T.truss_by_rank, (size_t)tail_limit));
+        KOMB_HIP(ctx, bufs.alloc(&T.level_by_rank, (size_t)tail_limit));
         KOMB_HIP(ctx, bufs.alloc(&T.spill[0], (size_t)tail_limit));
         KOMB_HIP(ctx, bufs.alloc(&T.spill[1], (size_t)tail_limit));
         T.max_edges = tail_limit;
@@ -607,11 +609,11 @@
         hipEvent_t ev[3] = {nullptr, nullptr, nullptr};
         for (auto &e : ev) (void)hipEventCreate(&e);
         (void)hipEventRecord(ev[0], s);
-        k_tail_mark<<<g, kBlock, 0, s>>>(list, n_in, d_sup, d_stamp, d_osrc, d_ocol, T);
+        k_tail_mark<<<g, kBlock, 0, s>>>(list, n_in, d_sup, d_st8, d_osrc, d_ocol, T);
         k_tail_number<<<1, kTailMaxV, 0, s>>>(T);
-        k_tail_rows<<<g, kBlock, 0, s>>>(list, n_in, d_sup, d_stamp, d_osrc, d_ocol, T);
+        k_tail_rows<<<g, kBlock, 0, s>>>(list, n_in, d_sup, d_st8, d_osrc, d_ocol, T);
         (void)hipEventRecord(ev[1], s);
-        k_truss_tail<<<1, 1024, 0, s>>>(d_ctrl, T, d_truss);
+        k_truss_tail<<<1, 1024, 0, s>>>(d_ctrl, T, d_sup);
         (void)hipEventRecord(ev[2], s);
         KOMB_HIP(ctx, d2h(ctx, &ctx->h_ctrl[0], d_ctrl, sizeof(PeelCtrl)));
         ++st.truss_tail_runs;
@@ -639,13 +641,11 @@
         for (auto &e : ev) KOMB_HIP(ctx, evs.make(&e));
         (void)hipEventRecord(ev[0], s);
         LocalStats ls;
-        const int lrc = local_finish(ctx, bufs, hc, d_ctrl, (uint32_t)m, d_stamp, d_sup, Q.live[hc.live_sel],
-            (uint32_t)kWave * TrussLocal::kU, sizeof(uint2), local_item_limit(ctx, kTrussLocalItems), local_density_limit(ctx, kTrussLocalDensity), true, 2, d_truss,
+        const int lrc = local_finish(ctx, bufs, hc, d_ctrl, (uint32_t)m, nullptr, d_st8, d_sup, Q.live[hc.live_sel],
+            (uint32_t)kWave * TrussLocal::kU, sizeof(uint2), local_item_limit(ctx, kTrussLocalItems), local_density_limit(ctx, kTrussLocalDensity), true, 0, d_sup,
             [&](const LocalGraph &lg, const int32_t *num, void *items, PeelCtrl *d_cctrl, int32_t launch) {
-                TrussCollect C{(uint32_t)m, d_off2, d_inc, d_stamp, num, lg.off, lg.cur, (uint2 *)items};
-                PeelQueues Qc = Q;
-                Qc.rlevel = nullptr;
-                k_peel_step<TrussCollect><<<gp, kPeelBlock, 0, s>>>(d_cctrl, d_grp, Qc, C, launch);
+                TrussCollect C{(uint32_t)m, d_off2, d_inc, d_st8, num, lg.off, lg.cur, (uint2 *)items};
+                k_peel_step<TrussCollect><<<gp, kPeelBlock, 0, s>>>(d_cctrl, d_grp, Q, C, launch);
             },
             [&](const LocalGraph &lg, void *items, uint64_t total_items, LocalCtrl *d_lctrl, uint32_t *d_cnt, int *nl) -> int {
                 return local_fixpoint(ctx, d_lctrl, d_cnt, lg, TrussLocal{(const uint2 *)items}, total_items, nl);
@@ -669,7 +669,7 @@
     ctx->timer.start(s);
     if (!peel_inited) {
         peel_ctrl_pre(s, d_grp);
-        k_peel_init<<<grid_for(m, kBlock, 1024), kBlock, 0, s>>>(m, d_off, d_off2, d_sup, d_stamp, d_st8, d_grp + kInitOff);
+        k_peel_init<<<grid_for(m, kBlock, 1024), kBlock, 0, s>>>(m, d_off, d_off2, d_st8, d_grp + kInitOff);
     }
     peel_ctrl_init(s, d_ctrl, d_grp, (uint32_t)m, tail_limit);
     int launches = 0, rc = KOMB_OK;
@@ -679,7 +679,8 @@
     if (shard_peel_on) {
         uint32_t iw[2] = {0u, 0u};
         KOMB_HIP(ctx, d2h(ctx, iw, d_grp + kInitOff, sizeof(iw)));
-        ShardTruss SP{(uint32_t)m, d_off2, d_inc, d_sup, d_stamp, 0u, 0u};
+        k_shard_stamps<<<grid_for(m), kBlock, 0, s>>>(d_st8, m, d_stamp);
+        ShardTruss SP{(uint32_t)m, d_off2, d_inc, d_sup, d_stamp, d_st8, 0u, 0u};
         shard_bounds((uint64_t)m, rank, world, &SP.lo, &SP.hi);
         ShardStats ss;
         rc = shard_peel(ctx, bufs, SP, d_sup, (uint32_t)m, iw[0], (int32_t)iw[1], rank, world, fn, user, Q, d_ctrl,
@@ -732,7 +733,7 @@
     st.max_trussness = ctx->h_ctrl[0].max_level + 2;
     for (int i = 0; i < 2; ++i) { bufs.release(Q.light[i]); bufs.release(Q.heavy[i]); bufs.release(Q.live[i]); }
     bufs.release(Q.code);
-    bufs.release(d_sup); bufs.release(d_inc);
+    bufs.release(d_inc);
 
     phase.next("truss: canonical gather");
     ctx->timer.start(s);
@@ -755,7 +756,8 @@
         KOMB_TRY(edge_list(ctx, sub.rowptr, sub.col, sub.nv, sub.vold, ctx->d_t_eu, ctx->d_t_ev));
     }
     ctx->t_k_lo = k_lo; ctx->t_k_hi = k_hi;
-    k_truss_results<<<grid_for(m), kBlock, 0, s>>>(d_stamp, Q.rlevel, d_truss, tp->e2k, m, k_lo, k_hi, ctx->d_t_truss);
+    k_truss_results<<<grid_for(m), kBlock, 0, s>>>(d_sup, tp->e2k, m, k_lo, k_hi, ctx->d_t_truss);
+    bufs.release(d_sup);
     ctx->d_t_slice = d_off2;
     bufs.detach(d_off2);
     ctx->t_sup_ready = false;
diff --git a/komb_amd/csrc/local_dev.h b/komb_amd/csrc/local_dev.h
--- a/komb_amd/csrc/local_dev.h
+++ b/komb_amd/csrc/local_dev.h
@@ -43,7 +43,7 @@
 
 constexpr int kNumBlock = 1024;
 static __global__ __launch_bounds__(kNumBlock) void k_local_number(const int32_t *__restrict__ list, uint32_t n_in, uint32_t n_live,
-                                                         const int32_t *__restrict__ marker, const int32_t *__restrict__ key,
+                                                         const int32_t *__restrict__ marker, const uint8_t *__restrict__ state, const int32_t *__restrict__ key,
                                                          uint32_t light_max, int32_t *__restrict__ num, LocalGraph g, LocalCtrl *ctrl)
 {
     __shared__ uint32_t sh_cnt[kNumBlock / kWave][2];
@@ -59,7 +59,7 @@
         int32_t u = -1, k = 0;
         if (i < n_in) {
             u = list ? list[i] : (int32_t)i;
-            if (!marker_alive(marker[u])) u = -1; else k = key[u];
+            if (!(state ? state_alive(state[u]) : marker_alive(marker[u]))) u = -1; else k = key[u];
         }
         const bool heavy = u >= 0 && (uint32_t)k > light_max, light = u >= 0 && !heavy;
         const uint64_t mh = __ballot(heavy), ml = __ballot(light);
@@ -756,7 +756,7 @@
 };
 
 template <class LaunchCollect, class RunFix, class AfterNumber>
-int local_finish(komb_ctx *ctx, DevBufs &bufs, const PeelCtrl &hc, PeelCtrl *d_ctrl, uint32_t units, const int32_t *marker,
+int local_finish(komb_ctx *ctx, DevBufs &bufs, const PeelCtrl &hc, PeelCtrl *d_ctrl, uint32_t units, const int32_t *marker, const uint8_t *state,
                  const int32_t *key, const int32_t *live_list, uint32_t light_max, size_t item_bytes, uint64_t item_limit, uint32_t max_density, bool use_list, int32_t add, int32_t *out,
                  LaunchCollect &&launch_collect, RunFix &&run_fix, LocalStats *ls, AfterNumber &&after_number)
 {
@@ -805,7 +805,7 @@
     };
     g.n = n; g.nh = 0; g.ng = 0; g.nchunk = 0;
     int64_t gb = ((int64_t)n_in + kNumBlock - 1) / kNumBlock;
-    k_local_number<<<(int)(gb < 1 ? 1 : (gb > 1024 ? 1024 : gb)), kNumBlock, 0, s>>>(list, n_in, n, marker, key, light_max, d_num, g, d_lctrl);
+    k_local_number<<<(int)(gb < 1 ? 1 : (gb > 1024 ? 1024 : gb)), kNumBlock, 0, s>>>(list, n_in, n, marker, state, key, light_max, d_num, g, d_lctrl);
     LocalCtrl hl{};
     std::vector<uint32_t> kh(kKeyBins);
     if (ctx->h_stage && sizeof(LocalCtrl) + kKeyBins * sizeof(uint32_t) <= kStageBytes) {
diff --git a/komb_amd/csrc/peel_dev.h b/komb_amd/csrc/peel_dev.h
--- a/komb_amd/csrc/peel_dev.h
+++ b/komb_amd/csrc/peel_dev.h
@@ -5,6 +5,7 @@
 namespace komb {
 
 enum : int32_t { MODE_SCAN = 0, MODE_PROCESS = 1, MODE_RETIRE = 2 };
+enum : int32_t { SRC_SCAN = 0, SRC_TRIGGER = 1 };
 
 #ifndef KOMB_PEEL_BLOCK
 #define KOMB_PEEL_BLOCK 1024
@@ -26,7 +27,7 @@
 constexpr int kInitOff = 2 * (kMaxGroups + 1);
 
 struct CtrlView {
-    int32_t mode, level, round, done, cur_sel;
+    int32_t mode, level, round, done, cur_sel, cur_src;
     uint32_t cur_light, cur_heavy, remaining;
     uint32_t live_count;
     int32_t live_sel, live_mode;
@@ -46,11 +47,11 @@
 constexpr int32_t kRetireEvery = 120;
 static_assert(2 * kRetireEvery + 2 < (int32_t)kStateWindow, "state codes must not wrap between two RETIRE steps, even if one were late by a whole period");
 __device__ __forceinline__ uint8_t state_of_round(int32_t q) { return (uint8_t)(ST_ROUND0 + (uint32_t)q % kStateWindow); }
-__device__ __forceinline__ uint8_t state_of_stamp(int32_t stamp)
-{
-    if (stamp >= kAliveMin) return (uint8_t)(stamp == kAlive ? ST_ALIVE_LIGHT : ST_ALIVE_HEAVY);
-    return stamp == 0 ? (uint8_t)ST_GONE : state_of_round(stamp);
-}
+__device__ __forceinline__ uint8_t state_of_len(uint32_t len)
+{
+    return (uint8_t)(len == 0 ? ST_GONE : (len <= (uint32_t)kLight ? ST_ALIVE_LIGHT : ST_ALIVE_HEAVY));
+}
+__device__ __forceinline__ bool state_alive(uint32_t c) { return c < ST_GONE; }
 __device__ __forceinline__ int32_t marker_of_state(uint32_t c)
 {
     return c == ST_ALIVE_LIGHT ? kAlive : (c == ST_ALIVE_HEAVY ? kAlive - 1 : 0);
@@ -121,7 +122,6 @@
     int2 *heavy[2];
     int32_t *live[2];
     int scalar_scan;
-    int32_t *rlevel = nullptr;
 };
 
 
@@ -216,13 +216,13 @@
 }
 
 __device__ __forceinline__ void finalize_step(PeelCtrl *ctrl, const CtrlView &cv, uint32_t units, CtrlView *out, uint32_t acc, int32_t launch,
-                                              int32_t *rlevel, int32_t retire_every)
+                                              int32_t retire_every)
 {
     const int lane = lane_id();
     if (lane == 0) { (void)atomicExch(&ctrl->seq, launch + 1); asm volatile("s_waitcnt vmcnt(0)" ::: "memory"); }
     __builtin_amdgcn_wave_barrier();
     if (cv.mode & MODE_RETIRE) {
-        if (lane == 0) { ctrl->mode = cv.mode & ~MODE_RETIRE; ctrl->last_retire = cv.round; *out = cv; out->mode = cv.mode & ~MODE_RETIRE; }
+        if (lane == 0) { ctrl->mode = cv.mode & ~MODE_RETIRE; ctrl->last_retire = cv.round; out->mode = cv.mode & ~MODE_RETIRE; }
         return;
     }
     const bool scan = cv.mode == MODE_SCAN;
@@ -241,7 +241,7 @@
     const int32_t nmin = __shfl((int)v, 3);
     const uint32_t live_n = (uint32_t)__shfl((int)v, 4);
     if (lane != 0) return;
-    if (!scan && rlevel) rlevel[cv.round] = cv.level;
+    const int32_t src = scan ? SRC_SCAN : SRC_TRIGGER;
     int32_t mode = cv.mode, level = cv.level, round = cv.round, done = 0, nsel = sel;
     int32_t live_sel = cv.live_sel, live_mode = cv.live_mode;
     uint32_t live_count = cv.live_count;
@@ -275,10 +275,10 @@
         }
     }
     ctrl->mode = mode; ctrl->level = level; ctrl->round = round; ctrl->done = done;
-    ctrl->cur_sel = nsel; ctrl->cur_light = cur_l; ctrl->cur_heavy = cur_h; ctrl->remaining = remaining;
+    ctrl->cur_sel = (int16_t)nsel; ctrl->cur_src = (int16_t)src; ctrl->cur_light = cur_l; ctrl->cur_heavy = cur_h; ctrl->remaining = remaining;
     ctrl->live_count = live_count; ctrl->live_sel = live_sel; ctrl->live_mode = live_mode;
     out->mode = mode; out->level = level; out->round = round; out->done = done;
-    out->cur_sel = nsel; out->cur_light = cur_l; out->cur_heavy = cur_h; out->remaining = remaining;
+    out->cur_sel = nsel; out->cur_src = src; out->cur_light = cur_l; out->cur_heavy = cur_h; out->remaining = remaining;
     out->live_count = live_count; out->live_sel = live_sel; out->live_mode = live_mode;
     out->tail_limit = cv.tail_limit;
 }
@@ -286,6 +286,10 @@
 template <class P, class = void> struct PeelRetire { static constexpr int32_t every = 0; };
 template <class P> struct PeelRetire<P, decltype((void)P::kRetireEvery)> { static constexpr int32_t every = P::kRetireEvery; };
 template <class P> __host__ __device__ constexpr int32_t peel_retire_every() { return PeelRetire<P>::every; }
+template <class P, class = void> struct PeelByteScan { static constexpr bool value = false; };
+template <class P> struct PeelByteScan<P, decltype((void)&P::scan_state)> { static constexpr bool value = true; };
+template <class P, class = void> struct PeelFreeze { static constexpr bool value = false; };
+template <class P> struct PeelFreeze<P, decltype((void)P::kFreezeKey)> { static constexpr bool value = P::kFreezeKey; };
 
 template <class P>
 __global__ __launch_bounds__(kPeelBlock, (kPeelBlock / 64) * kPeelPerCu / 4) void k_peel_step(PeelCtrl *ctrl, uint32_t *grp_done, PeelQueues Q, P p, int32_t launch)
@@ -315,7 +319,7 @@
     if (threadIdx.x == 0) {
         const PeelCtrl *c = reinterpret_cast<const PeelCtrl *>(sh_raw);
         sh_cv.mode = c->mode; sh_cv.level = c->level; sh_cv.round = c->round; sh_cv.done = c->done;
-        sh_cv.cur_sel = c->cur_sel; sh_cv.cur_light = c->cur_light; sh_cv.cur_heavy = c->cur_heavy;
+        sh_cv.cur_sel = c->cur_sel; sh_cv.cur_src = c->cur_src; sh_cv.cur_light = c->cur_light; sh_cv.cur_heavy = c->cur_heavy;
         sh_cv.remaining = c->remaining; sh_cv.live_count = c->live_count;
         sh_cv.live_sel = c->live_sel; sh_cv.live_mode = c->live_mode;
         sh_cv.tail_limit = ctrl->tail_limit;
@@ -345,10 +349,10 @@
         const int32_t *live_in = Q.live[cv.live_sel];
         int32_t *live_out = Q.live[cv.live_sel ^ 1];
         const bool vec = !from_list && !Q.scalar_scan;
-        const int32_t *s_marker = p.scan_marker(), *s_key = p.scan_key();
-        constexpr bool byte_marker = peel_retire_every<P>() > 0;
+        constexpr bool byte_marker = PeelByteScan<P>::value;
+        const int32_t *s_marker = nullptr, *s_key = p.scan_key();
         const uint8_t *s_state = nullptr;
-        if constexpr (byte_marker) s_state = p.scan_state();
+        if constexpr (byte_marker) s_state = p.scan_state(); else s_marker = p.scan_marker();
         uint32_t n_light = 0, n_chunks = 0, n_hits = 0, n_surv = 0;
         int32_t lmin = 0x7FFFFFFF;
         const uint64_t tile = (uint64_t)kPeelBlock * kScanU;
@@ -536,7 +540,10 @@
                 const uint64_t idx = job * bsz + (uint64_t)lane;
                 int32_t unit = -1;
                 uint32_t beg = 0, len = 0;
-                if ((uint32_t)lane < bsz && idx < cv.cur_light) { unit = Q.light[sel][idx]; p.slice((uint32_t)unit, beg, len); }
+                if ((uint32_t)lane < bsz && idx < cv.cur_light) {
+                    unit = Q.light[sel][idx]; p.slice((uint32_t)unit, beg, len);
+                    if constexpr (PeelFreeze<P>::value) if (cv.cur_src == SRC_TRIGGER) p.freeze_key(unit, cv);
+                }
 #ifdef KOMB_STEP_TIMERS
                 if (blockIdx.x == 0 && threadIdx.x == 0 && tk[2] == 0) { asm volatile("s_waitcnt vmcnt(0)" ::: "memory"); tk[2] = wall_clock64(); }
 #endif
@@ -546,6 +553,7 @@
             const int2 ent = Q.heavy[sel][job - n_batches];
             uint32_t beg, len;
             p.slice((uint32_t)ent.x, beg, len);
+            if constexpr (PeelFreeze<P>::value) if (cv.cur_src == SRC_TRIGGER && ent.y == 0 && lane == 0) p.freeze_key(ent.x, cv);
 #ifdef KOMB_STEP_TIMERS
             if (blockIdx.x == 0 && threadIdx.x == 0 && tk[2] == 0) { asm volatile("s_waitcnt vmcnt(0)" ::: "memory"); tk[2] = wall_clock64(); }
 #endif
@@ -625,10 +633,10 @@
 #endif
         last = __shfl(last, 0);
         total = (uint32_t)__shfl((int)total, 0);
-        if (last) finalize_step(ctrl, cv, p.units, &sh_cv, total, launch, Q.rlevel, retire_every);
+        if (last) finalize_step(ctrl, cv, p.units, &sh_cv, total, launch, retire_every);
         return;
     }
-    if (threadIdx.x < kWave) finalize_step(ctrl, cv, p.units, &sh_cv, sh_acc, launch, Q.rlevel, retire_every);
+    if (threadIdx.x < kWave) finalize_step(ctrl, cv, p.units, &sh_cv, sh_acc, launch, retire_every);
     if (P::kSingleStep) return;
     __syncthreads();
     cv = sh_cv;
diff --git a/komb_amd/csrc/truss_gather.h b/komb_amd/csrc/truss_gather.h
--- a/komb_amd/csrc/truss_gather.h
+++ b/komb_amd/csrc/truss_gather.h
@@ -6,14 +6,12 @@
 
 namespace {
 
-__global__ __launch_bounds__(kBlock) void k_truss_results(const int32_t *__restrict__ stamp, const int32_t *__restrict__ rlevel,
-                                                         const int32_t *__restrict__ truss,
+__global__ __launch_bounds__(kBlock) void k_truss_results(const int32_t *__restrict__ sup,
                                                          const uint32_t *__restrict__ e2k, int64_t m, uint32_t k_lo, uint32_t k_hi,
                                                          int32_t *__restrict__ tr_out)
 {
     for (int64_t e = (int64_t)blockIdx.x * kBlock + threadIdx.x; e < m; e += (int64_t)gridDim.x * kBlock) {
-        const int32_t s = stamp[e];
-        const int32_t t = marker_alive(s) ? truss[e] : rlevel[s] + 2;
+        const int32_t t = sup[e] + 2;
         const uint32_t k = e2k[e];
         if (k - k_lo < k_hi - k_lo) tr_out[k] = t;
     }
diff --git a/komb_amd/csrc/truss_index.h b/komb_amd/csrc/truss_index.h
--- a/komb_amd/csrc/truss_index.h
+++ b/komb_amd/csrc/truss_index.h
@@ -157,7 +157,7 @@
                                                          const uint32_t *__restrict__ bin_base,
                                                          const int2 *__restrict__ own_dense, const unsigned long long *__restrict__ ownoff,
                                                          int2 *__restrict__ dense, int64_t m,
-                                                         uint2 *__restrict__ off2, int32_t *__restrict__ sup, int32_t *__restrict__ stamp, uint8_t *__restrict__ st8,
+                                                         uint2 *__restrict__ off2, uint8_t *__restrict__ st8,
                                                          uint32_t *__restrict__ init, int32_t *__restrict__ light0)
 {
     __shared__ uint32_t sh_off[kBinEdges + 4];
@@ -211,27 +211,21 @@
         if (nin == (uint32_t)kFinE) {
             reinterpret_cast<uint4 *>(off2 + e0)[0] = make_uint4(base + o[0], c[0], base + o[1], c[1]);
             reinterpret_cast<uint4 *>(off2 + e0)[1] = make_uint4(base + o[2], c[2], base + o[3], c[3]);
-            int4 sv, mv;
-            int32_t *svp = &sv.x, *mvp = &mv.x;
+            uint8_t cd[kFinE];
 #pragma unroll
             for (int u = 0; u < kFinE; ++u) {
                 const bool first = queue_first && (int32_t)c[u] == L1;
-                svp[u] = (int32_t)c[u];
-                mvp[u] = first ? 1 : (c[u] ? alive_marker(c[u]) : 0);
+                cd[u] = first ? state_of_round(1) : state_of_len(c[u]);
                 if (!c[u]) ++zeros;
             }
-            *reinterpret_cast<int4 *>(sup + e0) = sv;
-            *reinterpret_cast<int4 *>(stamp + e0) = mv;
-            *reinterpret_cast<uchar4 *>(st8 + e0) = make_uchar4(state_of_stamp(mv.x), state_of_stamp(mv.y), state_of_stamp(mv.z), state_of_stamp(mv.w));
+            *reinterpret_cast<uchar4 *>(st8 + e0) = make_uchar4(cd[0], cd[1], cd[2], cd[3]);
         } else {
 #pragma unroll
             for (int u = 0; u < kFinE; ++u) if ((uint32_t)u < nin) {
                 const uint64_t e = e0 + u;
                 const bool first = queue_first && (int32_t)c[u] == L1;
                 off2[e] = make_uint2(base + o[u], c[u]);
-                sup[e] = (int32_t)c[u];
-                stamp[e] = first ? 1 : (c[u] ? alive_marker(c[u]) : 0);
-                st8[e] = state_of_stamp(stamp[e]);
+                st8[e] = first ? state_of_round(1) : state_of_len(c[u]);
                 if (!c[u]) ++zeros;
             }
         }
@@ -306,7 +300,7 @@
 }
 
 __global__ __launch_bounds__(kBlock) void k_peel_init(int64_t m, const uint32_t *__restrict__ off, uint2 *__restrict__ off2,
-                                                      int32_t *__restrict__ sup, int32_t *__restrict__ stamp, uint8_t *__restrict__ st8,
+                                                      uint8_t *__restrict__ st8,
                                                       uint32_t *__restrict__ init)
 {
     uint32_t zeros = 0;
@@ -315,9 +309,9 @@
         const uint32_t b0 = off[e];
         const int32_t s0 = (int32_t)(off[e + 1] - b0);
         off2[e] = make_uint2(b0, (uint32_t)s0);
-        sup[e] = s0;
-        if (s0 == 0) { stamp[e] = 0; st8[e] = (uint8_t)ST_GONE; ++zeros; }
-        else { const int32_t a = alive_marker((uint32_t)s0); stamp[e] = a; st8[e] = state_of_stamp(a); lmin = min(lmin, s0); }
+        st8[e] = state_of_len((uint32_t)s0);
+        if (s0 == 0) ++zeros;
+        else lmin = min(lmin, s0);
     }
     block_add_min(zeros, lmin, &init[0], (int32_t *)&init[1]);
 }
diff --git a/komb_amd/csrc/truss_tail.h b/komb_amd/csrc/truss_tail.h
--- a/komb_amd/csrc/truss_tail.h
+++ b/komb_amd/csrc/truss_tail.h
@@ -24,13 +24,13 @@
     int32_t *gid;
     int32_t *gid_by_rank;
     uint32_t *pair_by_rank;
-    int32_t *truss_by_rank;
+    int32_t *level_by_rank;
     uint32_t *spill[2];
     uint32_t max_edges;
 };
 
 __global__ __launch_bounds__(kBlock) void k_tail_mark(const int32_t *__restrict__ list, uint32_t n_in, const int32_t *__restrict__ sup,
-                                                      const int32_t *__restrict__ stamp,
+                                                      const uint8_t *__restrict__ st8,
                                                       const int32_t *__restrict__ osrc, const int32_t *__restrict__ ocol, TailBufs T)
 {
     __shared__ uint32_t seen[32];
@@ -40,7 +40,7 @@
     unsigned long long work = 0;
     for (uint32_t i = blockIdx.x * kBlock + threadIdx.x; i < n_in; i += gridDim.x * kBlock) {
         const int32_t e = list ? list[i] : (int32_t)i;
-        if (!marker_alive(stamp[e])) continue;
+        if (!state_alive(st8[e])) continue;
         ++live;
         const uint32_t sv = (uint32_t)sup[e];
         work += sv;
@@ -90,16 +90,16 @@
 }
 
 __global__ __launch_bounds__(kBlock) void k_tail_rows(const int32_t *__restrict__ list, uint32_t n_in, const int32_t *__restrict__ sup,
-                                                      const int32_t *__restrict__ stamp,
+                                                      const uint8_t *__restrict__ st8,
                                                       const int32_t *__restrict__ osrc, const int32_t *__restrict__ ocol, TailBufs T)
 {
     if (T.cnt[2]) return;
     for (uint32_t i0 = blockIdx.x * kBlock; i0 < n_in; i0 += gridDim.x * kBlock) {
         const uint32_t i = i0 + threadIdx.x;
         int32_t e = -1;
-        int32_t st = 0;
-        if (i < n_in) { e = list ? list[i] : (int32_t)i; st = stamp[e]; }
-        const bool live = e >= 0 && marker_alive(st);
+        uint32_t st = ST_GONE;
+        if (i < n_in) { e = list ? list[i] : (int32_t)i; st = st8[e]; }
+        const bool live = e >= 0 && state_alive(st);
         const uint64_t m = __ballot(live);
         uint32_t base = 0;
         if (lane_id() == 0 && m) base = atomicAdd(&T.cnt[3], (uint32_t)__popcll(m));
@@ -148,7 +148,7 @@
 __device__ __forceinline__ void tail_to_frontier(const TailLds &t, uint32_t r) { atomicOr(&t.S[r >> 1], 0xFFFFu << (16 * (r & 1))); }
 __device__ __forceinline__ void tail_to_dead(const TailLds &t, uint32_t r) { atomicAnd(&t.S[r >> 1], ~(1u << (16 * (r & 1)))); }
 
-__global__ __launch_bounds__(1024) void k_truss_tail(PeelCtrl *ctrl, TailBufs T, int32_t *__restrict__ truss)
+__global__ __launch_bounds__(1024) void k_truss_tail(PeelCtrl *ctrl, TailBufs T, int32_t *__restrict__ level_out)
 {
     __shared__ __attribute__((aligned(16))) uint32_t pool[kTailPoolWords];
     __shared__ uint32_t sh_cnt[2];
@@ -272,7 +272,7 @@
                 if (s < kTDead && r < E && (int32_t)s <= L) {
                     q_push(sel, __hip_atomic_load(&T.pair_by_rank[r], __ATOMIC_RELAXED, __HIP_MEMORY_SCOPE_AGENT));
                     tail_to_frontier(t, r);
-                    T.truss_by_rank[r] = L + 2;
+                    T.level_by_rank[r] = L;
                 }
             }
         }
@@ -349,7 +349,7 @@
                 const uint32_t code = q_get(sel ^ 1, i);
                 const uint32_t r = tail_rank(t, code >> 16, code & 0xFFFFu);
                 tail_to_frontier(t, r);
-                T.truss_by_rank[r] = L + 2;
+                T.level_by_rank[r] = L;
             }
             __syncthreads();
             tick(4);
@@ -362,8 +362,8 @@
     }
     __syncthreads();
     for (uint32_t r = tid; r < E; r += 1024)
-        truss[__hip_atomic_load(&T.gid_by_rank[r], __ATOMIC_RELAXED, __HIP_MEMORY_SCOPE_AGENT)] =
-            __hip_atomic_load(&T.truss_by_rank[r], __ATOMIC_RELAXED, __HIP_MEMORY_SCOPE_AGENT);
+        level_out[__hip_atomic_load(&T.gid_by_rank[r], __ATOMIC_RELAXED, __HIP_MEMORY_SCOPE_AGENT)] =
+            __hip_atomic_load(&T.level_by_rank[r], __ATOMIC_RELAXED, __HIP_MEMORY_SCOPE_AGENT);
     tick(5);
     if (tid == 0) {
 #ifdef KOMB_TAIL_TIMERS
```
